# EnricoMiccoli/nodal

Hardware: AMD Instinct MI355X
Metric: circuits_per_sec (higher is better)
Workload: dtype f64; 1 GPU; cfg3: grid(1000) 1e6 nodes, sparse CSR path; n=999999, nnz=4995995, parallelism=one GPU

## Files before the change

include/nodal_hip.h:

```cpp
#ifndef NODAL_HIP_H
#define NODAL_HIP_H

#include <stddef.h>
#include <stdint.h>

#ifdef __cplusplus
extern "C" {
#endif

typedef struct nodal_ctx *nodal_handle;

typedef enum {
    NODAL_OK = 0,
    NODAL_E_INVALID = 1,
    NODAL_E_HIP = 2,
    NODAL_E_ZERO_RESISTANCE = 3,
    NODAL_E_STAMP_COLLISION = 4,
    NODAL_E_SINGULAR = 5,
    NODAL_E_NOMEM = 6,
    NODAL_E_UNSUPPORTED = 7
} nodal_status;

enum { NODAL_T_R = 0, NODAL_T_A = 1, NODAL_T_E = 2, NODAL_T_VCVS = 3,
       NODAL_T_CCVS = 4, NODAL_T_CCCS = 5,
// ... 11 lines not shown
const char *nodal_version(void);

int nodal_upload_components(nodal_handle h, int64_t ncomp,
                            const uint8_t *type, const double *value,
                            const int32_t *a, const int32_t *b,
                            const int32_t *c, const int32_t *d,
                            const int32_t *drv, const int32_t *k,
                            int32_t K, int32_t B);
int nodal_host_alloc(size_t bytes, void **out);
int nodal_host_free(void *p);

int nodal_upload_values(nodal_handle h, int32_t batch, const double *values);

int nodal_assemble_symbolic(nodal_handle h);
int nodal_assemble_numeric(nodal_handle h, int32_t member, int64_t *bad_component);

int nodal_get_sizes(nodal_handle h, int64_t *n, int64_t *nnz, int64_t *ncontrib);

int nodal_export_csr(nodal_handle h, int32_t *indptr, int32_t *indices,
                     double *data, double *rhs);
int nodal_export_dense(nodal_handle h, double *G, double *rhs);

int nodal_solve_dense(nodal_handle h, double *x, int32_t *info);
int nodal_solve_sparse(nodal_handle h, int32_t method, double *x, int32_t *info,
                       int32_t *iters, double *resid);
int nodal_download_x(nodal_handle h, double *x);

int nodal_solve_pairs(nodal_handle h, int32_t dense, int32_t npairs, const int32_t *ia,
                      const int32_t *ib, double *resistance, int32_t *info);

int nodal_solve_sources(nodal_handle h, int32_t dense, int32_t count, int32_t nsrc, const int64_t *rows,
                        const double *values, double *x_out, double *resid_out, int32_t *info_out);

int nodal_branches(nodal_handle h, double *voltage, double *current, double *power, double *totals2);

int nodal_solve_sources_branches(nodal_handle h, int32_t dense, int32_t count, int32_t nsrc, const int64_t *rows,
                                 const double *values, double *x_out, double *resid_out, int32_t *info_out,
                                 double *current_absmax, int32_t *current_member, double *potential_min,
                                 int32_t *potential_min_member, double *potential_max, int32_t *potential_max_member,
                                 double *power_out);

int nodal_sensitivities(nodal_handle h, int32_t dense, int32_t count, const int32_t *kind, const int32_t *p,
                        const int32_t *q2, double *sens_out, double *value_out, double *adjoint_out,
                        double *resid_out, int32_t *info_out);

int nodal_gradient(nodal_handle h, int32_t dense, int32_t count, const double *x, const double *cotangent, int32_t nsrc,
                   const int64_t *rows, double *grad_out, double *grad_sources_out, double *adjoint_out,
                   double *resid_out, int32_t *info_out);

int nodal_transient(nodal_handle h, int32_t dense, int32_t steps, int32_t method, int64_t ncap, const int64_t *cap_rows,
                    int32_t nsrc, const int64_t *src_rows, const double *src_values, const double *x0, int32_t nprobe,
                    const int32_t *probe_a, const int32_t *probe_b, double *wave_out, int32_t keep_every, double *x_out,
                    double *pot_min, int32_t *pot_min_step, double *pot_max, int32_t *pot_max_step, double *resid_out,
                    int32_t *info_out, int32_t *iters_out);

int nodal_transient_rlc(nodal_handle h, int32_t dense, int32_t steps, int32_t method, int64_t ncap, const int64_t *cap_rows,
                        int32_t nsrc, const int64_t *src_rows, const double *src_values, const double *x0, int32_t nprobe,
                        const int32_t *probe_a, const int32_t *probe_b, double *wave_out, int32_t keep_every, double *x_out,
                        double *pot_min, int32_t *pot_min_step, double *pot_max, int32_t *pot_max_step, double *resid_out,
                        int32_t *info_out, int32_t *iters_out, int64_t nind, const int64_t *ind_rows, const double *i0,
                        int32_t ncur, const int32_t *cur_index, double *cur_out, double *i_final_out);

int nodal_transient_gradient(nodal_handle h, int32_t dense, int32_t nprobe, const int32_t *probe_a, const int32_t *probe_b,
                             const double *wave_cot ,
                             double *grad_out ,
                             double *grad_sources_out ,
                             double *grad_x0_out ,
                             double *adjoint_out ,
                             double *resid_out , int32_t *info_out );

int nodal_ac_sweep(nodal_handle h, int32_t dense, int32_t nfreq, const double *omega ,
                   int64_t nreact, const uint8_t *kind , const double *value ,
                   const int32_t *lead_a, const int32_t *lead_b ,
                   int32_t nsrc, const int64_t *src_rows, const double *src_re, const double *src_im,
                   int32_t nprobe, const int32_t *probe_a, const int32_t *probe_b, double *wave_out ,
                   int32_t ncur, const int32_t *cur_index , double *cur_out ,
                   int32_t keep_every, double *x_out ,
                   double *peak_out , int32_t *peak_freq_out ,
                   double *resid_out , int32_t *info_out );

int nodal_ac_noise(nodal_handle h, int32_t dense, int32_t nfreq, const double *omega ,
                   int64_t nreact, const uint8_t *kind , const double *value ,
                   const int32_t *lead_a, const int32_t *lead_b ,
                   double temperature ,
                   int32_t nout, const int32_t *out_a, const int32_t *out_b ,
                   int64_t input_row , const double *weight ,
                   double *density_out , double *gain_out ,
                   double *contrib_out , double *resid_out ,
                   int32_t *info_out );

int nodal_ac_ports(nodal_handle h, int32_t dense, int32_t nfreq, const double *omega ,
                   int64_t nreact, const uint8_t *kind , const double *value ,
                   const int32_t *lead_a, const int32_t *lead_b ,
                   int32_t nports, const int32_t *ia, const int32_t *ib ,
                   double *z_out ,
                   double *node_peak_out , int32_t *node_peak_port_out ,
                   int32_t *node_peak_freq_out ,
                   double *resid_out , int32_t *info_out ,
                   int64_t *work_out );

int nodal_ac_gradient(nodal_handle h, int32_t dense, int32_t nfreq, const double *omega ,
                      int64_t nreact, const uint8_t *kind , const double *value ,
                      const int32_t *lead_a, const int32_t *lead_b ,
                      int32_t nsrc, const int64_t *src_rows, const double *src_re, const double *src_im,
                      int32_t nprobe, const int32_t *probe_a, const int32_t *probe_b ,
                      const double *wave_cot , double *wave_out ,
                      double *grad_out , double *grad_react_out ,
                      double *grad_sources_out , int32_t keep_every,
                      double *adjoint_out ,
                      double *resid_out , int32_t *info_out ,
                      int64_t *work_out );

int nodal_port_matrix(nodal_handle h, int32_t dense, int32_t nports, const int32_t *ia, const int32_t *ib,
                      double *z_out , double *voc_out ,
                      double *resid_out , int32_t *info_out );

int nodal_residual(nodal_handle h, double *scaled_residual);

int nodal_run(nodal_handle h, int32_t dense, int32_t member, int32_t reuse_symbolic,
              int32_t *info);

int nodal_run_batch(nodal_handle h, int32_t first, int32_t count, int32_t reuse_symbolic,
                    double *x_out, int32_t *info_out);
int nodal_batch_x_device(nodal_handle h, void *device_dst, int64_t capacity_bytes);
int nodal_x_device(nodal_handle h, void *device_dst, int64_t capacity_bytes);

int nodal_last_timings(nodal_handle h, double *ms3);
int nodal_last_kernel_stats(nodal_handle h, double *ms_total, int64_t *launches,
                            double *alg_bytes_or_flops);

int nodal_last_solve_info(nodal_handle h, int32_t *iterations, int32_t *amg_levels,
                          double *relative_residual);

int nodal_synchronize(nodal_handle h);

enum {
    NODAL_OPT_FORCE_PIVOTING = 1, NODAL_OPT_GEPP_PANEL = 2, NODAL_OPT_EXTRA_STREAMS = 3, NODAL_OPT_BORROW_TABLE = 4,
    NODAL_OPT_TRANSIENT_TAPE = 5
};
int nodal_set_option(nodal_handle h, int32_t option, int32_t value);

int nodal_debug_gemm(nodal_handle h, int32_t M, int32_t N, int32_t K, const double *A,
                     const double *B, double *C);
int nodal_debug_sources_rhs(nodal_handle h, int32_t count, int32_t nsrc, const int64_t *rows,
                            const double *values, double *rhs_out);
int nodal_debug_residual(nodal_handle h, int32_t transposed, int32_t cols, int32_t layout, const double *x,
                         const double *b, double *scaled_out, double *norms_out);
int nodal_debug_direct_apply(nodal_handle h, int32_t transposed, int32_t cols, const double *r, double *z,
                             int64_t *perturbed_out, int32_t *info_out);
enum {
    NODAL_HA_ACOL = 0, NODAL_HA_AVAL = 1, NODAL_HA_AVALF = 2, NODAL_HA_ALEN = 3, NODAL_HA_DINV = 4, NODAL_HA_ADCOL = 5,
    NODAL_HA_AGG = 6, NODAL_HA_PCOL = 7, NODAL_HA_PVAL = 8, NODAL_HA_PVALF = 9, NODAL_HA_RCOL = 10, NODAL_HA_RVAL = 11,
    NODAL_HA_RVALF = 12, NODAL_HA_RLEN = 13, NODAL_HA_WCOL = 14, NODAL_HA_WVAL = 15, NODAL_HA_WLEN = 16,
    NODAL_HA_P2COL = 17, NODAL_HA_P2VAL = 18, NODAL_HA_P2LEN = 19, NODAL_HA_D2 = 20
};
int nodal_debug_hierarchy_info(nodal_handle h, int32_t *nlev, int64_t *ints , double *reals );
int nodal_debug_hierarchy_array(nodal_handle h, int32_t level, int32_t which, void *dst, int64_t capacity_bytes,
                                int64_t *bytes_out);

#ifdef __cplusplus
}
#endif
#endif
```

nodal_amd/_ffi.py:

```python

import atexit
import ctypes as C
import os
import weakref

import numpy as np

_HERE = os.path.dirname(os.path.abspath(__file__))
LIB_PATH = os.path.join(_HERE, "libnodal_hip.so")

OK, E_INVALID, E_HIP, E_ZERO_RESISTANCE, E_STAMP_COLLISION, E_SINGULAR, E_NOMEM, \
    E_UNSUPPORTED = range(8)
SPARSE_AUTO, SPARSE_PCG, SPARSE_DENSIFY, SPARSE_LU, SPARSE_DIRECT = range(5)
OPT_FORCE_PIVOTING = 1
OPT_GEPP_PANEL = 2
OPT_EXTRA_STREAMS = 3
OPT_BORROW_TABLE = 4
OPT_TRANSIENT_TAPE = 5

_p = C.POINTER
_i32p, _i64p, _f64p, _u8p = _p(C.c_int32), _p(C.c_int64), _p(C.c_double), _p(C.c_uint8)

SIGNATURES = {
    "nodal_version": (C.c_char_p, []),
    "nodal_create": (C.c_int, [C.c_int, _p(C.c_void_p)]),
    "nodal_destroy": (C.c_int, [C.c_void_p]),
    "nodal_last_error": (C.c_char_p, [C.c_void_p]),
    "nodal_upload_components": (C.c_int, [C.c_void_p, C.c_int64, _u8p, _f64p, _i32p, _i32p,
                                          _i32p, _i32p, _i32p, _i32p, C.c_int32, C.c_int32]),
    "nodal_host_alloc": (C.c_int, [C.c_size_t, _p(C.c_void_p)]),
    "nodal_host_free": (C.c_int, [C.c_void_p]),
    "nodal_upload_values": (C.c_int, [C.c_void_p, C.c_int32, _f64p]),
    "nodal_assemble_symbolic": (C.c_int, [C.c_void_p]),
    "nodal_assemble_numeric": (C.c_int, [C.c_void_p, C.c_int32, _i64p]),
    "nodal_get_sizes": (C.c_int, [C.c_void_p, _i64p, _i64p, _i64p]),
    "nodal_export_csr": (C.c_int, [C.c_void_p, _i32p, _i32p, _f64p, _f64p]),
    "nodal_export_dense": (C.c_int, [C.c_void_p, _f64p, _f64p]),
    "nodal_solve_dense": (C.c_int, [C.c_void_p, _f64p, _i32p]),
    "nodal_solve_sparse": (C.c_int, [C.c_void_p, C.c_int32, _f64p, _i32p, _i32p, _f64p]),
    "nodal_download_x": (C.c_int, [C.c_void_p, _f64p]),
    "nodal_solve_pairs": (C.c_int, [C.c_void_p, C.c_int32, C.c_int32, _i32p, _i32p, _f64p, _i32p]),
    "nodal_solve_sources": (C.c_int, [C.c_void_p, C.c_int32, C.c_int32, C.c_int32, _i64p, _f64p, _f64p, _f64p,
                                      _i32p]),
    "nodal_branches": (C.c_int, [C.c_void_p, _f64p, _f64p, _f64p, _f64p]),
    "nodal_solve_sources_branches": (C.c_int, [C.c_void_p, C.c_int32, C.c_int32, C.c_int32, _i64p, _f64p, _f64p, _f64p,
                                               _i32p, _f64p, _i32p, _f64p, _i32p, _f64p, _i32p, _f64p]),
    "nodal_sensitivities": (C.c_int, [C.c_void_p, C.c_int32, C.c_int32, _i32p, _i32p, _i32p, _f64p, _f64p, _f64p, _f64p,
                                      _i32p]),
    "nodal_gradient": (C.c_int, [C.c_void_p, C.c_int32, C.c_int32, _f64p, _f64p, C.c_int32, _i64p, _f64p, _f64p, _f64p,
                                 _f64p, _i32p]),
    "nodal_transient": (C.c_int, [C.c_void_p, C.c_int32, C.c_int32, C.c_int32, C.c_int64, _i64p, C.c_int32, _i64p, _f64p,
                                  _f64p, C.c_int32, _i32p, _i32p, _f64p, C.c_int32, _f64p, _f64p, _i32p, _f64p, _i32p,
                                  _f64p, _i32p, _i32p]),
    "nodal_transient_rlc": (C.c_int, [C.c_void_p, C.c_int32, C.c_int32, C.c_int32, C.c_int64, _i64p, C.c_int32, _i64p, _f64p,
                                      _f64p, C.c_int32, _i32p, _i32p, _f64p, C.c_int32, _f64p, _f64p, _i32p, _f64p, _i32p,
                                      _f64p, _i32p, _i32p, C.c_int64, _i64p, _f64p, C.c_int32, _i32p, _f64p, _f64p]),
    "nodal_transient_gradient": (C.c_int, [C.c_void_p, C.c_int32, C.c_int32, _i32p, _i32p, _f64p, _f64p, _f64p, _f64p, _f64p,
                                           _f64p, _i32p]),
    "nodal_ac_sweep": (C.c_int, [C.c_void_p, C.c_int32, C.c_int32, _f64p, C.c_int64, _u8p, _f64p, _i32p, _i32p, C.c_int32,
                                 _i64p, _f64p, _f64p, C.c_int32, _i32p, _i32p, _f64p, C.c_int32, _i32p, _f64p, C.c_int32,
                                 _f64p, _f64p, _i32p, _f64p, _i32p]),
    "nodal_ac_noise": (C.c_int, [C.c_void_p, C.c_int32, C.c_int32, _f64p, C.c_int64, _u8p, _f64p, _i32p, _i32p, C.c_double,
                                 C.c_int32, _i32p, _i32p, C.c_int64, _f64p, _f64p, _f64p, _f64p, _f64p, _i32p]),
    "nodal_ac_ports": (C.c_int, [C.c_void_p, C.c_int32, C.c_int32, _f64p, C.c_int64, _u8p, _f64p, _i32p, _i32p, C.c_int32,
                                 _i32p, _i32p, _f64p, _f64p, _i32p, _i32p, _f64p, _i32p, _i64p]),
    "nodal_ac_gradient": (C.c_int, [C.c_void_p, C.c_int32, C.c_int32, _f64p, C.c_int64, _u8p, _f64p, _i32p, _i32p, C.c_int32,
                                    _i64p, _f64p, _f64p, C.c_int32, _i32p, _i32p, _f64p, _f64p, _f64p, _f64p, _f64p,
                                    C.c_int32, _f64p, _f64p, _i32p, _i64p]),
    "nodal_port_matrix": (C.c_int, [C.c_void_p, C.c_int32, C.c_int32, _i32p, _i32p, _f64p, _f64p, _f64p, _i32p]),
    "nodal_residual": (C.c_int, [C.c_void_p, _f64p]),
    "nodal_run": (C.c_int, [C.c_void_p, C.c_int32, C.c_int32, C.c_int32, _i32p]),
    "nodal_run_batch": (C.c_int, [C.c_void_p, C.c_int32, C.c_int32, C.c_int32, _f64p, _i32p]),
    "nodal_batch_x_device": (C.c_int, [C.c_void_p, C.c_void_p, C.c_int64]),
    "nodal_x_device": (C.c_int, [C.c_void_p, C.c_void_p, C.c_int64]),
    "nodal_last_timings": (C.c_int, [C.c_void_p, _f64p]),
    "nodal_last_kernel_stats": (C.c_int, [C.c_void_p, _f64p, _i64p, _f64p]),
    "nodal_last_solve_info": (C.c_int, [C.c_void_p, _i32p, _i32p, _f64p]),
    "nodal_synchronize": (C.c_int, [C.c_void_p]),
    "nodal_set_option": (C.c_int, [C.c_void_p, C.c_int32, C.c_int32]),
    "nodal_debug_gemm": (C.c_int, [C.c_void_p, C.c_int32, C.c_int32, C.c_int32, _f64p, _f64p, _f64p]),
    "nodal_debug_sources_rhs": (C.c_int, [C.c_void_p, C.c_int32, C.c_int32, _i64p, _f64p, _f64p]),
    "nodal_debug_residual": (C.c_int, [C.c_void_p, C.c_int32, C.c_int32, C.c_int32, _f64p, _f64p, _f64p, _f64p]),
    "nodal_debug_direct_apply": (C.c_int, [C.c_void_p, C.c_int32, C.c_int32, _f64p, _f64p, _i64p, _i32p]),
    "nodal_debug_hierarchy_info": (C.c_int, [C.c_void_p, _i32p, _i64p, _f64p]),
    "nodal_debug_hierarchy_array": (C.c_int, [C.c_void_p, C.c_int32, C.c_int32, C.c_void_p, C.c_int64, _i64p]),
}

HIERARCHY_ARRAYS = (("acol", np.int32), ("aval", np.float64), ("avalf", np.float32), ("alen", np.int32),
                    ("dinv", np.float64), ("adcol", np.int16), ("agg", np.int32), ("pcol", np.int32),
                    ("pval", np.float64), ("pvalf", np.float32), ("rcol", np.int32), ("rval", np.float64),
                    ("rvalf", np.float32), ("rlen", np.int32), ("wcol", np.int32), ("wval", np.float32),
                    ("wlen", np.int32), ("p2col", np.int32), ("p2val", np.float32), ("p2len", np.int32),
                    ("d2", np.float32))
HIERARCHY_INFO = ("n", "ld", "nc", "width", "maxlen", "wfix", "nnz", "rld", "rcap", "wslots", "fold_want", "fold", "d16",
                  "in_tail", "refreshed", "dense_coarsest")

_lib = None
_live = weakref.WeakSet()


@atexit.register
def _close_all():
    _closing[0] = True
    for h in list(_live):
        h.close()


class NodalHipError(RuntimeError):
    def __init__(self, status, message):
        super().__init__(f"libnodal_hip status {status}: {message}")
        self.status = status


def load():
    global _lib
    if _lib is None:
        if not os.path.exists(LIB_PATH):
            raise OSError(
                f"{LIB_PATH} not found: build it with `make` (or "
                "`python -c 'import __graft_entry__ as g; g.build()'`) -- "
                "nodal_amd has no CPU fallback")
        lib = C.CDLL(LIB_PATH)
        for name, (res, args) in SIGNATURES.items():
            fn = getattr(lib, name)
            fn.restype, fn.argtypes = res, args
        _lib = lib
    return _lib


def _ptr(arr, ctype):
    return arr.ctypes.data_as(_p(ctype))


PINNED_MIN_BYTES = 1 << 20
_PINNED_POOL = {}
_PINNED_POOL_BYTES = [0]
_PINNED_POOL_MAX = 1 << 30
_pinned_ok = [None]
_closing = [False]


def _pinned_release(addr, nbytes):
    if _lib is None or _closing[0]:
        return
    if _PINNED_POOL_BYTES[0] + nbytes <= _PINNED_POOL_MAX:
        _PINNED_POOL.setdefault(nbytes, []).append(addr)
        _PINNED_POOL_BYTES[0] += nbytes
    else:
        _lib.nodal_host_free(C.c_void_p(addr))


def host_empty(count, dtype):
    dtype = np.dtype(dtype)
    nbytes = int(count) * dtype.itemsize
    if nbytes < PINNED_MIN_BYTES or _pinned_ok[0] is False:
        return np.empty(count, dtype=dtype)
    try:
        lib = load()
    except OSError:
        _pinned_ok[0] = False
        return np.empty(count, dtype=dtype)
    size = (nbytes + 4095) & ~4095
    free = _PINNED_POOL.get(size)
    if free:
        addr = free.pop()
        _PINNED_POOL_BYTES[0] -= size
    else:
        out = C.c_void_p()
        if lib.nodal_host_alloc(size, C.byref(out)) != OK or not out.value:
            _pinned_ok[0] = False
            return np.empty(count, dtype=dtype)
        _pinned_ok[0] = True
        addr = out.value
    buf = (C.c_char * size).from_address(addr)
    weakref.finalize(buf, _pinned_release, addr, size)
    return np.frombuffer(buf, dtype=dtype, count=count)


class Handle:

    def __init__(self, device=0):
        self.lib = load()
        self._h = C.c_void_p()
        status = self.lib.nodal_create(device, C.byref(self._h))
        if status != OK:
            raise NodalHipError(
                status, f"nodal_create(device={device}) failed: no usable MI355X "
                "(HIP device) is visible; nodal_amd has no CPU fallback")
        self.n = self.nnz = self.ncontrib = 0
        self._ncomp = self._K = 0
        self.lib.nodal_set_option(self._h, OPT_BORROW_TABLE, 1)
        _live.add(self)

    def close(self):
        if getattr(self, "_h", None):
            self.lib.nodal_destroy(self._h)
            self._h = None

    __del__ = close

    @property
    def closed(self):
        return not getattr(self, "_h", None)

    def _check(self, status, allow=()):
        if status != OK and status not in allow:
            raise NodalHipError(status, self.lib.nodal_last_error(self._h).decode())
        return status

    def upload(self, table):
        names = ("type", "value", "a", "b") if table.B == 0 else ("type", "value", "a", "b", "c", "d", "drv", "k")
        cols = [np.ascontiguousarray(getattr(table, n)) for n in names]
        self._keep = cols
        t, v, a, b = cols[:4]
        rest = [_ptr(x, C.c_int32) for x in cols[4:]] or [None] * 4
        self.n_members = table.K + table.B
        self._ncomp, self._K = int(table.ncomp), int(table.K)
        self._check(self.lib.nodal_upload_components(
            self._h, table.ncomp, _ptr(t, C.c_uint8), _ptr(v, C.c_double),
            _ptr(a, C.c_int32), _ptr(b, C.c_int32), *rest, table.K, table.B))

    def upload_values(self, values):
        values = np.ascontiguousarray(values, dtype=np.float64)
        assert values.ndim == 2
        self._check(self.lib.nodal_upload_values(self._h, values.shape[0], _ptr(values, C.c_double)))

    def assemble_symbolic(self):
        self._check(self.lib.nodal_assemble_symbolic(self._h))
        self._refresh_sizes()

    def _refresh_sizes(self):
        n, nnz, nc = C.c_int64(), C.c_int64(), C.c_int64()
        self._check(self.lib.nodal_get_sizes(self._h, C.byref(n), C.byref(nnz), C.byref(nc)))
        self.n, self.nnz, self.ncontrib = n.value, nnz.value, nc.value

    def assemble_numeric(self, member=0):
        bad = C.c_int64(-1)
        status = self._check(self.lib.nodal_assemble_numeric(self._h, member, C.byref(bad)),
                             allow=(E_ZERO_RESISTANCE, E_STAMP_COLLISION))
        return status, bad.value

    def export_csr(self, values=True):
        indptr = np.empty(self.n + 1, dtype=np.int32)
        indices = np.empty(self.nnz, dtype=np.int32)
        data = np.empty(self.nnz, dtype=np.float64) if values else None
        rhs = np.empty(self.n, dtype=np.float64) if values else None
# ... 445 lines not shown
```

nodal_amd/csrc/knobs.h:

```cpp
#pragma once
#include <stdint.h>
#include <stdlib.h>

#include <optional>

namespace knob {

struct Present {
    const char *name;
    bool now() const { return getenv(name) != nullptr; }
};
struct OnUnless0 {
    const char *name;
    bool now() const { const char *e = getenv(name); return !(e && atoi(e) == 0); }
};
struct OffUnlessNon0 {
    const char *name;
    bool now() const { const char *e = getenv(name); return e && atoi(e) != 0; }
};
struct OnIfSet0 {
    const char *name;
    bool now() const { const char *e = getenv(name); return e != nullptr && atoi(e) == 0; }
};
struct Level {
    const char *name;
    int now() const {
        const char *e = getenv(name);
        if (!e) return 0;
        const int v = atoi(e);
        return v > 1 ? v : 1;
    }
};
struct Int {
    const char *name;
    int dflt;
    int now() const { const char *e = getenv(name); return e ? atoi(e) : dflt; }
};
struct Int64 {
    const char *name;
    int64_t dflt;
    int64_t now() const { const char *e = getenv(name); return e ? atoll(e) : dflt; }
};
struct Double {
    const char *name;
    double dflt;
    double now() const { const char *e = getenv(name); return e ? atof(e) : dflt; }
};
struct IntIfSet {
    const char *name;
    std::optional<int> now() const { const char *e = getenv(name); return e ? std::optional<int>(atoi(e)) : std::nullopt; }
};
struct Int64IfSet {
    const char *name;
    std::optional<int64_t> now() const { const char *e = getenv(name); return e ? std::optional<int64_t>(atoll(e)) : std::nullopt; }
};
struct DoubleIfSet {
    const char *name;
    std::optional<double> now() const { const char *e = getenv(name); return e ? std::optional<double>(atof(e)) : std::nullopt; }
};
struct Text {
    const char *name;
    const char *now() const { return getenv(name); }
};

inline constexpr Present TRACE{"NODAL_TRACE"};
inline constexpr Level POISON{"NODAL_POISON"};
inline constexpr Present NOFILL{"NODAL_NOFILL"};
inline constexpr Present NANCHECK{"NODAL_NANCHECK"};
inline constexpr Double WAIT_TIMEOUT_S{"NODAL_WAIT_TIMEOUT_S", 60.0};
inline constexpr Text STREAM_PRIORITY{"NODAL_STREAM_PRIORITY"};
inline constexpr IntIfSet EXTRA_STREAMS{"NODAL_EXTRA_STREAMS"};
inline constexpr IntIfSet HOST_THREADS{"NODAL_HOST_THREADS"};
inline constexpr IntIfSet CSV_CHUNKS{"NODAL_CSV_CHUNKS"};
inline constexpr OnUnless0 FOLD_STREAM{"NODAL_FOLD_STREAM"};
inline constexpr OffUnlessNon0 COUNT_LDS{"NODAL_COUNT_LDS"};
inline constexpr IntIfSet DENSE_BLOCKINV{"NODAL_DENSE_BLOCKINV"};
inline constexpr IntIfSet GJ_SCALAR{"NODAL_GJ_SCALAR"};
inline constexpr OnUnless0 GJ_DPP{"NODAL_GJ_DPP"};
inline constexpr OnUnless0 BI_SYM{"NODAL_BI_SYM"};
inline constexpr OnIfSet0 BI_MASKED{"NODAL_BI_MASKED"};
inline constexpr Int PANEL_CUS{"NODAL_PANEL_CUS", 32};
inline constexpr Int64 BI_UNMASK_ROWS{"NODAL_BI_UNMASK_ROWS", 0};
inline constexpr OnUnless0 BI_EARLY_COPY{"NODAL_BI_EARLY_COPY"};
inline constexpr Int BI_FIRST_BLOCKS{"NODAL_BI_FIRST_BLOCKS", 2};
inline constexpr Text BI_SWITCH{"NODAL_BI_SWITCH"};
inline constexpr Text BI_SWITCH2{"NODAL_BI_SWITCH2"};
inline constexpr Text BI_WIDTH{"NODAL_BI_WIDTH"};
inline constexpr IntIfSet GEPP_PANEL{"NODAL_GEPP_PANEL"};
inline constexpr Int GEPP_MAX{"NODAL_GEPP_MAX", 1280};
inline constexpr Present GEPP_PROBE{"NODAL_GEPP_PROBE"};
inline constexpr Int64IfSet FCG_MAXIT{"NODAL_FCG_MAXIT"};
inline constexpr OnUnless0 FCG_HOST_SUM{"NODAL_FCG_HOST_SUM"};
inline constexpr Double FCG_LOOK{"NODAL_FCG_LOOK", 0.75};
inline constexpr OnUnless0 LOWDEG{"NODAL_LOWDEG"};
inline constexpr IntIfSet LOWDEG_SHARE{"NODAL_LOWDEG_SHARE"};
inline constexpr Int64 LOWDEG_MIN{"NODAL_LOWDEG_MIN", 32};
inline constexpr Present SPARSE_FORCE_DIRECT{"NODAL_SPARSE_FORCE_DIRECT"};
inline constexpr Present SPARSE_CHILD_DIRECT{"NODAL_SPARSE_CHILD_DIRECT"};
inline constexpr OnUnless0 SAGG{"NODAL_SAGG"};
inline constexpr OnUnless0 SA_REUSE{"NODAL_SA_REUSE"};
inline constexpr OnUnless0 SA_FORK{"NODAL_SA_FORK"};
inline constexpr Double SA_SPREAD{"NODAL_SA_SPREAD", 16.0};
inline constexpr Double SA_SHARE{"NODAL_SA_SHARE", 0.9};
inline constexpr IntIfSet SA_MIS{"NODAL_SA_MIS"};
inline constexpr Text SA_OMEGA_P{"NODAL_SA_OMEGA_P"};
inline constexpr Double SA_PADSLACK{"NODAL_SA_PADSLACK", 1.3};
inline constexpr OnUnless0 SA_D16{"NODAL_SA_D16"};
inline constexpr Int SA_GG{"NODAL_SA_GG", 40};
inline constexpr Int64 SA_GCAP{"NODAL_SA_GCAP", 16384};
inline constexpr Int SA_GSEG{"NODAL_SA_GSEG", 4};
inline constexpr Text SA_NU{"NODAL_SA_NU"};
inline constexpr Int SA_KCYCLE{"NODAL_SA_KCYCLE", 1};
inline constexpr Int SA_KLEVELS{"NODAL_SA_KLEVELS", 1};
inline constexpr OnUnless0 SA_KFREEZE{"NODAL_SA_KFREEZE"};
inline constexpr OnUnless0 SA_FUSE_DIR{"NODAL_SA_FUSE_DIR"};
inline constexpr OffUnlessNon0 SA_GRAPH{"NODAL_SA_GRAPH"};
inline constexpr Text SA_FOLD_POST{"NODAL_SA_FOLD_POST"};
inline constexpr OffUnlessNon0 SA_FOLD_CHECK{"NODAL_SA_FOLD_CHECK"};
inline constexpr OnUnless0 SA_FOLD_VISIT{"NODAL_SA_FOLD_VISIT"};
inline constexpr Int64 SA_VISIT_CAP{"NODAL_SA_VISIT_CAP", 16777216};
inline constexpr OffUnlessNon0 SA_VISIT_CHECK{"NODAL_SA_VISIT_CHECK"};
inline constexpr OnUnless0 SA_TAIL_DENSE{"NODAL_SA_TAIL_DENSE"};
inline constexpr OffUnlessNon0 SA_TAIL_CHECK{"NODAL_SA_TAIL_CHECK"};
inline constexpr Int SA_TAIL_NU{"NODAL_SA_TAIL_NU", 3};
inline constexpr Present TAIL_PROBE{"NODAL_TAIL_PROBE"};
inline constexpr IntIfSet AMG_PASSES0{"NODAL_AMG_PASSES0"};
inline constexpr IntIfSet AMG_PASSES1{"NODAL_AMG_PASSES1"};
inline constexpr IntIfSet AMG_SWEEPS0{"NODAL_AMG_SWEEPS0"};
inline constexpr IntIfSet AMG_BLOCK{"NODAL_AMG_BLOCK"};
inline constexpr DoubleIfSet AMG_THETA{"NODAL_AMG_THETA"};
inline constexpr Present AMG_KEEP_DENSE{"NODAL_AMG_KEEP_DENSE"};
inline constexpr Present AMG_NOTAIL{"NODAL_AMG_NOTAIL"};
inline constexpr IntIfSet AMG_KMAX{"NODAL_AMG_KMAX"};
inline constexpr OnUnless0 PAIRS_BLOCK{"NODAL_PAIRS_BLOCK"};
inline constexpr OnUnless0 PAIRS_FUNCTIONAL{"NODAL_PAIRS_FUNCTIONAL"};
inline constexpr Int PAIRS_DIRECT{"NODAL_PAIRS_DIRECT", -1};
inline constexpr Int64 PAIRS_DIRECT_MIN{"NODAL_PAIRS_DIRECT_MIN", 256};
inline constexpr Double MULTI_BAR{"NODAL_MULTI_BAR", 1e-14};
inline constexpr IntIfSet PRESOLVE{"NODAL_PRESOLVE"};
inline constexpr OnUnless0 PRESOLVE_KEEP{"NODAL_PRESOLVE_KEEP"};
inline constexpr IntIfSet FGMRES_WINDOW{"NODAL_FGMRES_WINDOW"};
inline constexpr Text DIRECT_NB{"NODAL_DIRECT_NB"};
inline constexpr Int DIRECT_LANES{"NODAL_DIRECT_LANES", 4};
inline constexpr DoubleIfSet DIRECT_MAX_GB{"NODAL_DIRECT_MAX_GB"};
inline constexpr IntIfSet DIRECT_BIG_DIM{"NODAL_DIRECT_BIG_DIM"};
inline constexpr OnUnless0 DIRECT_FRONT_LDS{"NODAL_DIRECT_FRONT_LDS"};
inline constexpr Int DIRECT_LDS_BS{"NODAL_DIRECT_LDS_BS", 64};
inline constexpr OnUnless0 DIRECT_PANEL_REGS{"NODAL_DIRECT_PANEL_REGS"};
inline constexpr OnUnless0 DIRECT_BATCHED{"NODAL_DIRECT_BATCHED"};
inline constexpr OnUnless0 DIRECT_WAVE{"NODAL_DIRECT_WAVE"};
inline constexpr Present DIRECT_LEVELS{"NODAL_DIRECT_LEVELS"};
inline constexpr OnUnless0 DIRECT_SUPER{"NODAL_DIRECT_SUPER"};
inline constexpr OnUnless0 DIRECT_APPLY_STEPPED{"NODAL_DIRECT_APPLY_STEPPED"};
inline constexpr OnUnless0 DIRECT_PEEL{"NODAL_DIRECT_PEEL"};
inline constexpr Int ND_DEPTH{"NODAL_ND_DEPTH", 4};
inline constexpr Int64 ND_PAR{"NODAL_ND_PAR", 20000};
inline constexpr Present SLU_DEBUG{"SLU_DEBUG"};

}
```

nodal_amd/csrc/sagg.hip:

```cpp
#include <hip/hip_ext.h>

#include <atomic>
#include <type_traits>

#include "group.h"

int grounded_flags(nodal_ctx *h, uint8_t *flags_dev);

namespace {

using grp::TB;
constexpr int PW = 4;
constexpr int ACAP = 64;
constexpr int RCAP = 96;
constexpr int RCAP_SMALL = 512;
constexpr int RCAP_SMALL_ROWS = 16384;
inline int rcap_for(int64_t nc) { return nc <= RCAP_SMALL_ROWS ? RCAP_SMALL : RCAP; }
constexpr int W0_MAX = 32;
constexpr int COARSEST = 64;
constexpr int MAX_LEVELS = 12;
constexpr int MIS_ROUNDS = 6;
constexpr int TAIL_MAX_N = 1024;
constexpr int TAIL_LEVELS = 6;
constexpr int TAIL_LDS_BUDGET = 150 * 1024;
constexpr int APAD = 32;
constexpr int DOT_BLOCKS = 1024;
#ifndef NODAL_SA_OMEGA
#define NODAL_SA_OMEGA 0.85
#endif
constexpr double OMEGA = NODAL_SA_OMEGA;
constexpr double OMEGA_P = 0.70;
constexpr double OMEGA_P_COARSE = 0.85;
using cyc_t = nodal_cyc_t;

inline unsigned grid_for(int64_t n, unsigned cap = 8192) {
    int64_t g = (n + TB - 1) / TB;
    if (g < 1) g = 1;
    if (g >= 64) g = (g + 7) & ~(int64_t)7;
    return (unsigned)(g > cap ? cap : g);
}
inline int64_t pad64(int64_t n) { return (n + 63) & ~(int64_t)63; }
inline size_t align256(size_t x) { return (x + 255) & ~(size_t)255; }

__device__ __forceinline__ unsigned xcd_block() {
    const unsigned g = gridDim.x, b = blockIdx.x;
    return (g & 7u) ? b : (b & 7u) * (g >> 3) + (b >> 3);
}


struct Ell {
    int64_t n = 0, ld = 0;
    int32_t width = 0;
    const int32_t *col = nullptr;
    const int16_t *dcol = nullptr;
    const double *val = nullptr;
    const float *valf = nullptr;
    const int32_t *len = nullptr;
};

enum { ST_MAXLEN = 0, ST_GRADED = 1, ST_BADDIAG = 2, ST_OVERFLOW = 3, ST_NNZ = 4, ST_UNASSIGNED = 5,
       ST_MAXR = 6, ST_NC = 7 ,
       ST_FARCOL = 8 ,
       ST_FOLDMISS = 9 ,
       ST_VISITMISS = 10 ,
       ST_COUNT = 11 };

struct SLevel {
    int64_t n = 0, ld = 0, nc = 0;
    int32_t width = 0;
    int32_t maxlen = 0;
    int32_t wfix = 0;
    int64_t nnz = 0;
    DevBuf acol, aval, alen, dinv;
    DevBuf adcol;
    bool d16 = false;
    DevBuf agg, pcol, pval;
    DevBuf rcol, rval, rlen;
    int64_t rld = 0;
    DevBuf vec, part, gflag;
    DevBuf avalf, pvalf, rvalf;
    DevBuf wcol, wval, wlen;
    int32_t wslots = 0;
    bool fold_want = false, fold = false;
    DevBuf p2col, p2val, p2len, d2;
    bool visit_want = false, visit = false;
    Ell A() const {
        Ell e;
        e.n = n; e.ld = ld; e.width = width;
        e.col = acol.as<int32_t>(); e.val = aval.as<double>(); e.len = alen.as<int32_t>();
        e.valf = avalf.as<float>();
        e.dcol = d16 ? adcol.as<int16_t>() : nullptr;
        return e;
    }
    template <typename T = double> T *v(int which) const { return reinterpret_cast<T *>(vec.as<double>() + (int64_t)which * ld); }
};
enum { V_X = 0, V_R = 1, V_XP = 2, V_RC = 3, V_C1 = 4, V_C2 = 5, V_V1 = 6, V_V2 = 7, V_R2 = 8, V_X1 = 9, V_T = 10,
       V_COUNT = 11 };

struct TailLevelDesc {
    int n, nc, ld, rld, width, nq, lpr;
    const int32_t *acol, *pcol, *rcol, *rlen, *alen;
    const double *aval, *dinv, *pval, *rval;
    int o_aval, o_acol, o_dinv, o_pval, o_pcol, o_rval, o_rcol, o_B, o_X, o_Y, o_R;
};
struct TailDesc {
    int nlev;
    TailLevelDesc lv[TAIL_LEVELS];
    const double *inv;
    int nu;
    int image_bytes;
    int lds_bytes;
    int skip;
    int slots;
    long long *stamps;
};

struct SHierarchy {
    std::vector<SLevel *> pool;
    int nlev = 0;
    int tail = -1;
    bool ready = false;
    bool kcycle = true;
    bool kfrozen = false;
    int kslot = -1, kcount = 0, ksamples = 0;
    int klevels = 1;
    int nu[3] = {2, 1, 2};
    bool dense_coarsest = true;
    DevBuf tail_stamps, tail_image, apcol, apval, aplen, bstat;
    DevBuf tail_op;
    bool tail_dense = false;
    DevBuf mvec;
    hipEvent_t ev_copy = nullptr;
    hipStream_t aux = nullptr;
    hipEvent_t ev_fork = nullptr, ev_join = nullptr, ev_flags = nullptr;
    bool aux_pending = false;
    bool aux_tried = false;
    bool want_flags = false;
    int flags_levels = 0;
    DevBuf stats, coarse_inv, mis_t, mis_m, mis_flag, mis_id, agg1, keys, rstart, cursor, lists;
    TailDesc td;
    uint64_t *host_stats = nullptr;
    bool sym_valid = false;
    uint64_t sym_epoch = 0;
    int64_t sym_n = 0, sym_nnz = 0;
    bool sym_general = false, sym_check = false;
    int32_t sym_floating = 0;
    hipGraph_t it_graph = nullptr;
    hipGraphExec_t it_exec = nullptr;
    uint64_t it_key = 0;
    bool refreshed = false;
    int last_iters = 0;
    int hint_iters = 0;
    int64_t hint_n = 0, hint_nnz = 0;
    int mblock_iters = 0;
    int64_t mblock_n = 0;
    unsigned long long sym_stats[MAX_LEVELS * ST_COUNT] = {0};
    SLevel *level(int l) {
        while ((int)pool.size() <= l) pool.push_back(new SLevel());
        return pool[l];
    }
    void drop_graph() {
        if (it_exec) (void)hipGraphExecDestroy(it_exec);
        if (it_graph) (void)hipGraphDestroy(it_graph);
        it_exec = nullptr;
        it_graph = nullptr;
        it_key = 0;
    }
    ~SHierarchy() {
        drop_graph();
        if (ev_copy) (void)hipEventDestroy(ev_copy);
        if (ev_fork) (void)hipEventDestroy(ev_fork);
        if (ev_join) (void)hipEventDestroy(ev_join);
        if (ev_flags) (void)hipEventDestroy(ev_flags);
        if (aux) (void)hipStreamDestroy(aux);
        for (SLevel *l : pool) {
            DevBuf *b[] = {&l->acol, &l->aval, &l->alen, &l->dinv, &l->agg, &l->pcol, &l->pval, &l->rcol,
                           &l->rval, &l->rlen, &l->vec, &l->part, &l->gflag, &l->avalf, &l->pvalf, &l->rvalf, &l->adcol,
                           &l->wcol, &l->wval, &l->wlen, &l->p2col, &l->p2val, &l->p2len, &l->d2};
            for (DevBuf *x : b) x->release();
            delete l;
        }
        tail_image.release();
        tail_op.release();
        mvec.release();
        tail_stamps.release();
        bstat.release();
        apcol.release();
        apval.release();
        aplen.release();
        DevBuf *b[] = {&stats, &coarse_inv, &mis_t, &mis_m, &mis_flag, &mis_id, &agg1, &keys, &rstart, &cursor, &lists};
        for (DevBuf *x : b) x->release();
        if (host_stats) (void)hipHostFree(host_stats);
    }
};


constexpr int BSTAT_MAX = 65536;
__global__ __launch_bounds__(1024) void reduce_bstat(int nblocks, const uint32_t *__restrict__ bstat,
                                                     unsigned long long *__restrict__ stats, int slot_max,
                                                     int slot_sum) {
    __shared__ unsigned int s_max;
    __shared__ unsigned long long s_sum;
    if (threadIdx.x == 0) { s_max = 0; s_sum = 0; }
    __syncthreads();
    unsigned int m = 0;
    unsigned long long t = 0;
    for (int i = threadIdx.x; i < nblocks; i += 1024) {
        m = max(m, bstat[i]);
        t += bstat[BSTAT_MAX + i];
    }
    atomicMax(&s_max, m);
    atomicAdd(&s_sum, t);
    __syncthreads();
    if (threadIdx.x == 0) {
        if (slot_max >= 0) stats[slot_max] = s_max;
        if (slot_sum >= 0) stats[slot_sum] = s_sum;
    }
}

__global__ __launch_bounds__(TB) void row_stats(int64_t n, const int32_t *__restrict__ indptr,
                                                const int32_t *__restrict__ indices,
                                                const double *__restrict__ data, double share, double spread,
                                                bool general, unsigned long long *__restrict__ stats,
                                                uint32_t *__restrict__ bstat) {
    int32_t mlen = 0;
    uint32_t graded = 0, bad = 0, far = 0;
    for (int64_t i = (int64_t)xcd_block() * TB + threadIdx.x; i < n; i += (int64_t)gridDim.x * TB) {
        const int32_t e0 = indptr[i], e1 = indptr[i + 1];
        mlen = max(mlen, e1 - e0);
        double d = 0.0, mx = 0.0, mn = 1e300;
        for (int32_t e = e0; e < e1; ++e) {
            const double v = data[e];
            const int64_t dc = (int64_t)indices[e] - i;
            if (dc > 32767 || dc < -32767) far = 1;
            if (indices[e] == (int32_t)i) d = v;
            else if (v != 0.0) {
                mx = fmax(mx, fabs(v));
                mn = fmin(mn, fabs(v));
                if (v > 0.0 && !general) bad = 1;
            }
        }
        if (!(d > 0.0)) bad = 1;
        graded += (d > 0.0 && (mx > share * d || mx > spread * mn)) ? 1u : 0u;
    }
    __shared__ unsigned int s_len, s_graded, s_bad;
    if (threadIdx.x == 0) s_len = s_graded = s_bad = 0;
    __syncthreads();
    atomicMax(&s_len, (unsigned)mlen);
    if (graded) atomicAdd(&s_graded, graded);
    if (bad) atomicOr(&s_bad, 1u);
    if (far) atomicOr(&s_bad, 2u);
    __syncthreads();
    if (threadIdx.x == 0) {
        bstat[blockIdx.x] = s_len;
        bstat[BSTAT_MAX + blockIdx.x] = s_graded;
        if (s_bad & 1u) atomicOr(&stats[ST_BADDIAG], 1ull);
        if (s_bad & 2u) stats[ST_FARCOL] = 1ull;
    }
}

__global__ __launch_bounds__(TB) void csr_to_ell(int64_t n, int64_t ld, const int32_t *__restrict__ indptr,
                                                 const int32_t *__restrict__ indices,
                                                 const double *__restrict__ data, int32_t *__restrict__ col,
                                                 double *__restrict__ val, float *__restrict__ valf,
                                                 int32_t *__restrict__ len, double *__restrict__ dinv, int32_t wpad,
                                                 int16_t *__restrict__ dcol) {
    for (int64_t i = (int64_t)xcd_block() * TB + threadIdx.x; i < n; i += (int64_t)gridDim.x * TB) {
        const int32_t e0 = indptr[i], e1 = indptr[i + 1];
        double d = 1.0;
        for (int32_t e = e0; e < e1; ++e) {
            const int32_t c = indices[e];
            const double v = data[e];
            col[(int64_t)(e - e0) * ld + i] = c;
            if (dcol) dcol[(int64_t)(e - e0) * ld + i] = (int16_t)(c - (int32_t)i);
            val[(int64_t)(e - e0) * ld + i] = v;
            valf[(int64_t)(e - e0) * ld + i] = (float)v;
            if (c == (int32_t)i) d = v;
        }
        for (int32_t s = e1 - e0; s < wpad; ++s) {
            col[(int64_t)s * ld + i] = (int32_t)i;
            if (dcol) dcol[(int64_t)s * ld + i] = 0;
            val[(int64_t)s * ld + i] = 0.0;
            valf[(int64_t)s * ld + i] = 0.0f;
        }
        len[i] = e1 - e0;
        dinv[i] = 1.0 / d;
    }
}


__device__ __forceinline__ uint32_t hash30(uint32_t x) {
    x ^= x >> 16;
    x *= 0x7feb352du;
    x ^= x >> 15;
    x *= 0x846ca68bu;
    x ^= x >> 16;
    return x & 0x3fffffffu;
}

__global__ __launch_bounds__(TB) void mis_init(int64_t n, uint32_t *__restrict__ T) {
    for (int64_t i = (int64_t)xcd_block() * TB + threadIdx.x; i < n; i += (int64_t)gridDim.x * TB)
        T[i] = (1u << 30) | hash30((uint32_t)i);
}

template <int NB>
__device__ __forceinline__ uint32_t nbr_max_batch(const Ell &A, const uint32_t *__restrict__ v, int64_t i, int32_t l, int32_t s0,
                                                  uint32_t best) {
    int32_t c[NB];
#pragma unroll
    for (int u = 0; u < NB; ++u) c[u] = A.col[(int64_t)(s0 + u < l ? s0 + u : 0) * A.ld + i];
    uint32_t t[NB];
#pragma unroll
    for (int u = 0; u < NB; ++u) t[u] = v[c[u]];
#pragma unroll
    for (int u = 0; u < NB; ++u) best = t[u] > best ? t[u] : best;
    return best;
}
__device__ __forceinline__ uint32_t nbr_max(const Ell &A, const uint32_t *__restrict__ v, int64_t i, int32_t l, uint32_t best) {
    if (l <= 5) return nbr_max_batch<5>(A, v, i, l, 0, best);
    for (int32_t s0 = 0; s0 < l; s0 += 8) best = nbr_max_batch<8>(A, v, i, l, s0, best);
    return best;
}

__global__ __launch_bounds__(TB) void mis_max(Ell A, const uint32_t *__restrict__ v, uint32_t *__restrict__ m) {
    for (int64_t i = (int64_t)xcd_block() * TB + threadIdx.x; i < A.n; i += (int64_t)gridDim.x * TB)
        m[i] = nbr_max(A, v, i, A.len[i], v[i]);
}

__global__ __launch_bounds__(TB) void mis_update(Ell A, uint32_t *__restrict__ T, const uint32_t *__restrict__ m1) {
    for (int64_t i = (int64_t)xcd_block() * TB + threadIdx.x; i < A.n; i += (int64_t)gridDim.x * TB) {
        const uint32_t own = T[i];
        if ((own >> 30) != 1) continue;
        const uint32_t best = nbr_max(A, m1, i, A.len[i], m1[i]);
        if (best == own) T[i] = own | (2u << 30);
        else if ((best >> 30) == 3) T[i] = 0;
    }
}

__global__ __launch_bounds__(TB) void mis_count(int64_t n, const uint32_t *__restrict__ T,
                                                unsigned long long *__restrict__ out) {
    uint32_t left = 0;
    for (int64_t i = (int64_t)xcd_block() * TB + threadIdx.x; i < n; i += (int64_t)gridDim.x * TB)
        left += (T[i] >> 30) == 1 ? 1u : 0u;
// ... 22 lines not shown

constexpr int64_t MIS_SMALL_MAX = 1024;
__global__ __launch_bounds__(1024) void mis_small(Ell A, uint32_t *__restrict__ T, uint32_t *__restrict__ M,
                                                  uint32_t *__restrict__ flag, int rounds) {
    const int64_t n = A.n;
    for (int64_t i = threadIdx.x; i < n; i += 1024) T[i] = (1u << 30) | hash30((uint32_t)i);
    __syncthreads();
    for (int r = 0; r < rounds; ++r) {
        for (int64_t i = threadIdx.x; i < n; i += 1024) {
            uint32_t best = T[i];
            const int32_t l = A.len[i];
            for (int32_t s = 0; s < l; ++s) {
                const uint32_t t = T[A.col[(int64_t)s * A.ld + i]];
                best = t > best ? t : best;
            }
            M[i] = best;
        }
        __syncthreads();
        for (int64_t i = threadIdx.x; i < n; i += 1024) {
            const uint32_t own = T[i];
            if ((own >> 30) != 1) continue;
            uint32_t best = M[i];
            const int32_t l = A.len[i];
            for (int32_t s = 0; s < l; ++s) {
                const uint32_t t = M[A.col[(int64_t)s * A.ld + i]];
                best = t > best ? t : best;
            }
            if (best == own) T[i] = own | (2u << 30);
            else if ((best >> 30) == 3) T[i] = 0;
        }
        __syncthreads();
    }
    for (int64_t i = threadIdx.x; i <= n; i += 1024) {
        uint32_t f = 0;
        if (i < n) {
            const uint32_t own = T[i];
            if ((own >> 30) == 3) f = 1;
            else if ((own >> 30) == 1) {
                bool near = false;
                const int32_t l = A.len[i];
                for (int32_t s = 0; s < l; ++s) near = near || (T[A.col[(int64_t)s * A.ld + i]] >> 30) == 3;
                f = near ? 0u : 1u;
            }
        }
        flag[i] = f;
    }
}

__global__ __launch_bounds__(TB) void assign_near(Ell A, const uint32_t *__restrict__ T,
                                                  const uint32_t *__restrict__ flag,
                                                  const uint32_t *__restrict__ id, int32_t *__restrict__ agg1) {
    for (int64_t i = (int64_t)xcd_block() * TB + threadIdx.x; i < A.n; i += (int64_t)gridDim.x * TB) {
        int32_t a = -1;
        if (flag[i]) a = (int32_t)id[i];
        else {
            uint32_t best = 0;
            const int32_t l = A.len[i];
            auto batch = [&](auto NBc, int32_t s0) {
                constexpr int NB = decltype(NBc)::value;
                int32_t c[NB];
#pragma unroll
                for (int u = 0; u < NB; ++u) c[u] = A.col[(int64_t)(s0 + u < l ? s0 + u : 0) * A.ld + i];
                uint32_t fl[NB], tt[NB], idd[NB];
#pragma unroll
                for (int u = 0; u < NB; ++u) {
                    fl[u] = flag[c[u]];
                    tt[u] = T[c[u]];
                    idd[u] = id[c[u]];
                }
#pragma unroll
                for (int u = 0; u < NB; ++u) {
                    if (s0 + u >= l || c[u] == (int32_t)i || !fl[u]) continue;
                    const uint32_t t = tt[u] | (3u << 30);
                    if (t > best) { best = t; a = (int32_t)idd[u]; }
                }
            };
            if (l <= 5) batch(std::integral_constant<int, 5>{}, 0);
            else for (int32_t s0 = 0; s0 < l; s0 += 8) batch(std::integral_constant<int, 8>{}, s0);
        }
        agg1[i] = a;
    }
}

__global__ __launch_bounds__(TB) void assign_far(Ell A, const int32_t *__restrict__ agg1, int32_t *__restrict__ agg,
                                                 unsigned long long *__restrict__ stats) {
    for (int64_t i = (int64_t)xcd_block() * TB + threadIdx.x; i < A.n; i += (int64_t)gridDim.x * TB) {
        int32_t a = agg1[i];
        if (a < 0) {
            double bw = -1.0;
            const int32_t l = A.len[i];
            auto batch = [&](auto NBc, int32_t s0) {
                constexpr int NB = decltype(NBc)::value;
                int32_t c[NB];
                double w[NB];
#pragma unroll
                for (int u = 0; u < NB; ++u) {
                    const int64_t at = (int64_t)(s0 + u < l ? s0 + u : 0) * A.ld + i;
                    c[u] = A.col[at];
                    w[u] = fabs(A.val[at]);
                }
                int32_t aj[NB];
#pragma unroll
                for (int u = 0; u < NB; ++u) aj[u] = agg1[c[u]];
#pragma unroll
                for (int u = 0; u < NB; ++u) {
                    if (s0 + u >= l || c[u] == (int32_t)i || aj[u] < 0) continue;
                    if (w[u] > bw) { bw = w[u]; a = aj[u]; }
                }
            };
            if (l <= 5) batch(std::integral_constant<int, 5>{}, 0);
            else for (int32_t s0 = 0; s0 < l; s0 += 8) batch(std::integral_constant<int, 8>{}, s0);
            if (a < 0) stats[ST_UNASSIGNED] = 1;
        }
        agg[i] = a;
    }
}

__global__ __launch_bounds__(TB) void build_P(Ell A, const double *__restrict__ dinv,
                                              const int32_t *__restrict__ agg, int32_t *__restrict__ pcol,
                                              double *__restrict__ pval, float *__restrict__ pvalf, double omega_p) {
    for (int64_t i = (int64_t)xcd_block() * TB + threadIdx.x; i < A.n; i += (int64_t)gridDim.x * TB) {
        int32_t c[PW];
        double v[PW];
#pragma unroll
        for (int k = 0; k < PW; ++k) { c[k] = -1; v[k] = 0.0; }
        const int32_t own = agg[i];
        c[0] = own;
        v[0] = 1.0;
        const double wd = omega_p * dinv[i];
        const int32_t l = A.len[i];
        for (int32_t s = 0; s < l; ++s) {
            const int32_t J = agg[A.col[(int64_t)s * A.ld + i]];
            const double t = -wd * A.val[(int64_t)s * A.ld + i];
            bool placed = false;
#pragma unroll
            for (int k = 0; k < PW; ++k) {
                if (!placed && c[k] == J) { v[k] += t; placed = true; }
            }
#pragma unroll
            for (int k = 1; k < PW; ++k) {
                if (!placed && c[k] < 0) { c[k] = J; v[k] = t; placed = true; }
            }
            if (!placed) v[0] += t;
        }
#pragma unroll
        for (int k = 0; k < PW; ++k) {
            pcol[(int64_t)k * A.ld + i] = c[k];
            pval[(int64_t)k * A.ld + i] = v[k];
            pvalf[(int64_t)k * A.ld + i] = (float)v[k];
        }
    }
}

__global__ __launch_bounds__(TB) void r_count(int64_t n, int64_t ld, const int32_t *__restrict__ pcol,
                                              uint32_t *__restrict__ cnt, uint32_t *__restrict__ place) {
    for (int64_t i = (int64_t)xcd_block() * TB + threadIdx.x; i < n; i += (int64_t)gridDim.x * TB) {
#pragma unroll
        for (int k = 0; k < PW; ++k) {
            const int32_t J = pcol[(int64_t)k * ld + i];
            if (J >= 0) place[(int64_t)k * ld + i] = atomicAdd(&cnt[J], 1u);
        }
    }
}
__global__ __launch_bounds__(TB) void r_fill(int64_t n, int64_t ld, const int32_t *__restrict__ pcol,
                                             const uint32_t *__restrict__ rstart, const uint32_t *__restrict__ place,
                                             uint64_t *__restrict__ keys) {
    for (int64_t i = (int64_t)xcd_block() * TB + threadIdx.x; i < n; i += (int64_t)gridDim.x * TB) {
#pragma unroll
        for (int k = 0; k < PW; ++k) {
            const int32_t J = pcol[(int64_t)k * ld + i];
            if (J >= 0) keys[rstart[J] + place[(int64_t)k * ld + i]] = ((uint64_t)i << 2) | (uint64_t)k;
        }
    }
}
__global__ __launch_bounds__(TB) void r_to_ell(int64_t nc, int64_t rld, const uint32_t *__restrict__ rstart,
                                               const uint64_t *__restrict__ keys, int64_t ld,
                                               const double *__restrict__ pval, int32_t *__restrict__ rcol,
                                               double *__restrict__ rval, float *__restrict__ rvalf,
                                               int32_t *__restrict__ rlen,
                                               unsigned long long *__restrict__ stats, uint32_t *__restrict__ bstat,
                                               uint32_t rcap) {
    uint32_t mlen = 0;
    const int sub = threadIdx.x & 7;
    const int64_t rows_per_pass = (int64_t)gridDim.x * (TB / 8);
    for (int64_t I = (int64_t)xcd_block() * (TB / 8) + threadIdx.x / 8; I < nc; I += rows_per_pass) {
        const uint32_t s0 = rstart[I];
        uint32_t l = rstart[I + 1] - s0;
        mlen = l > mlen ? l : mlen;
        if (l > rcap) l = rcap;
        const uint32_t upto = nc <= 4096 ? rcap : ((l + 7u) & ~7u);
        for (uint32_t t = sub; t < upto; t += 8) {
            const int64_t at = ((int64_t)(t >> 3) * rld + I) * 8 + (t & 7);
            if (t < l) {
                const uint64_t key = keys[s0 + t];
                const int64_t i = (int64_t)(key >> 2);
                const double v = pval[(int64_t)(key & 3) * ld + i];
                rcol[at] = (int32_t)i;
                rval[at] = v;
                rvalf[at] = (float)v;
            } else {
                rcol[at] = 0;
                rval[at] = 0.0;
                rvalf[at] = 0.0f;
            }
        }
        if (sub == 0) rlen[I] = (int32_t)l;
    }
    if (mlen > rcap) atomicOr(&stats[ST_OVERFLOW], 2ull);
    __shared__ unsigned int s_max;
    if (threadIdx.x == 0) s_max = 0;
    __syncthreads();
#pragma unroll
    for (int off = 32; off > 0; off >>= 1) {
        const uint32_t o = __shfl_down(mlen, off, 64);
        mlen = o > mlen ? o : mlen;
    }
    if ((threadIdx.x & 63) == 0) atomicMax(&s_max, mlen);
    __syncthreads();
    if (threadIdx.x == 0) {
        bstat[blockIdx.x] = s_max;
        bstat[BSTAT_MAX + blockIdx.x] = 0;
    }
}

__global__ __launch_bounds__(TB) void r_refresh(int64_t nc, int64_t rld, const int32_t *__restrict__ rlen,
                                                const int32_t *__restrict__ rcol, int64_t ld,
                                                const int32_t *__restrict__ pcol, const double *__restrict__ pval,
                                                double *__restrict__ rval, float *__restrict__ rvalf) {
    const int sub = threadIdx.x & 7;
    const int64_t rows_per_pass = (int64_t)gridDim.x * (TB / 8);
    for (int64_t I = (int64_t)xcd_block() * (TB / 8) + threadIdx.x / 8; I < nc; I += rows_per_pass) {
        const int32_t l = rlen[I];
        for (int32_t t = sub; t < l; t += 8) {
            const int64_t at = ((int64_t)(t >> 3) * rld + I) * 8 + (t & 7);
            const int64_t i = rcol[at];
            double v = 0.0;
#pragma unroll
            for (int k = 0; k < PW; ++k) {
                const double pv = pval[(int64_t)k * ld + i];
                v = pcol[(int64_t)k * ld + i] == (int32_t)I ? pv : v;
            }
            rval[at] = v;
            rvalf[at] = (float)v;
        }
    }
}

__global__ __launch_bounds__(TB) void r_sort_short(const uint32_t *__restrict__ rstart, uint64_t *__restrict__ keys,
                                                   int64_t nc) {
    for (int64_t I = (int64_t)xcd_block() * TB + threadIdx.x; I < nc; I += (int64_t)gridDim.x * TB) {
        const uint32_t s0 = rstart[I];
        const int len = (int)(rstart[I + 1] - s0);
        if (len < 2) continue;
        if (len <= 4) grp::sort_short_row<4>(keys + s0, len);
        else if (len <= 8) grp::sort_short_row<8>(keys + s0, len);
        else if (len <= 16) grp::sort_short_row<16>(keys + s0, len);
        else if (len <= 32) grp::sort_short_row<32>(keys + s0, len);
    }
}
__global__ __launch_bounds__(64) void r_sort_medium(const uint32_t *__restrict__ rstart, uint64_t *__restrict__ keys,
                                                    int64_t nc) {
    __shared__ uint64_t buf[RCAP_SMALL];
    const int lane = threadIdx.x;
    for (int64_t I = blockIdx.x; I < nc; I += gridDim.x) {
        const uint32_t s0 = rstart[I];
        const int len = (int)(rstart[I + 1] - s0);
        if (len <= 32 || len > RCAP_SMALL) continue;
        const int P = len <= 64 ? 64 : (len <= 128 ? 128 : (len <= 256 ? 256 : 512));
        for (int e = lane; e < P; e += 64) buf[e] = e < len ? keys[s0 + e] : ~0ull;
        __syncthreads();
        for (int size = 2; size <= P; size <<= 1)
            for (int stride = size >> 1; stride > 0; stride >>= 1) {
                for (int p = lane; p < P / 2; p += 64) {
                    const int i = ((p & ~(stride - 1)) << 1) | (p & (stride - 1));
                    const int j = i | stride;
                    const bool up = (i & size) == 0;
                    const uint64_t a = buf[i], b = buf[j];
                    if ((a > b) == up) { buf[i] = b; buf[j] = a; }
                }
                __syncthreads();
            }
        for (int e = lane; e < len; e += 64) keys[s0 + e] = buf[e];
        __syncthreads();
    }
}

__device__ __forceinline__ int wave_excl_scan(int v, int *total) {
    const int lane = threadIdx.x & 63;
    int incl = v;
#pragma unroll
    for (int off = 1; off < 64; off <<= 1) {
        const int t = __shfl_up(incl, off, 64);
        if (lane >= off) incl += t;
    }
    *total = __shfl(incl, 63, 64);
    return incl - v;
}

template <int APW, bool EMIT>
__global__ __launch_bounds__(TB) void ap_rows(Ell A, const int32_t *__restrict__ pcol, const double *__restrict__ pval,
                                              int32_t *__restrict__ apcol, double *__restrict__ apval,
                                              int32_t *__restrict__ aplen, unsigned long long *__restrict__ stats,
                                              const double *__restrict__ dinv, int32_t *__restrict__ wcol,
                                              float *__restrict__ wval, int32_t *__restrict__ wlen) {
    bool overflow = false, miss = false;
    for (int64_t i = (int64_t)xcd_block() * TB + threadIdx.x; i < A.n; i += (int64_t)gridDim.x * TB) {
        int32_t c[APW];
        double v[APW];
        [[maybe_unused]] int32_t Jo[PW];
        [[maybe_unused]] double po[PW], wd = 0.0;
        if constexpr (EMIT) {
#pragma unroll
            for (int sp = 0; sp < PW; ++sp) {
                Jo[sp] = pcol[(int64_t)sp * A.ld + i];
                po[sp] = pval[(int64_t)sp * A.ld + i];
            }
            wd = OMEGA * dinv[i];
        }
#pragma unroll
        for (int q = 0; q < APW; ++q) { c[q] = -1; v[q] = 0.0; }
        int cnt = 0;
        const int32_t l = A.len[i];
        for (int32_t s = 0; s < l; ++s) {
            const int32_t k = A.col[(int64_t)s * A.ld + i];
            const double a = A.val[(int64_t)s * A.ld + i];
            int32_t J[PW];
            double pp[PW];
#pragma unroll
            for (int sp = 0; sp < PW; ++sp) {
                J[sp] = pcol[(int64_t)sp * A.ld + k];
                pp[sp] = pval[(int64_t)sp * A.ld + k];
            }
#pragma unroll
            for (int sp = 0; sp < PW; ++sp) {
                if (J[sp] < 0) continue;
                const double t = a * pp[sp];
                bool placed = false;
#pragma unroll
                for (int q = 0; q < APW; ++q)
                    if (!placed && c[q] == J[sp]) { v[q] += t; placed = true; }
#pragma unroll
                for (int q = 0; q < APW; ++q)
                    if (!placed && c[q] < 0) { c[q] = J[sp]; v[q] = t; placed = true; cnt = q + 1; }
                if (!placed) overflow = true;
            }
        }
#pragma unroll
        for (int q = 0; q < APW; ++q)
            if (q < cnt) {
                apcol[(int64_t)q * A.ld + i] = c[q];
                apval[(int64_t)q * A.ld + i] = v[q];
            }
        aplen[i] = cnt;
        if constexpr (EMIT) {
            int have = 0, found = 0;
#pragma unroll
            for (int sp = 0; sp < PW; ++sp) have += Jo[sp] >= 0 ? 1 : 0;
#pragma unroll
            for (int q = 0; q < APW; ++q)
                if (q < cnt) {
                    double pv = 0.0;
#pragma unroll
                    for (int sp = 0; sp < PW; ++sp)
                        if (Jo[sp] == c[q]) { pv += po[sp]; ++found; }
                    wcol[(int64_t)q * A.ld + i] = c[q];
                    wval[(int64_t)q * A.ld + i] = (float)(pv - wd * v[q]);
                }
            wlen[i] = cnt;
            if (found != have) miss = true;
        }
    }
    if (overflow) atomicOr(&stats[ST_OVERFLOW], 4ull);
    if (miss) stats[ST_FOLDMISS] = 1ull;
}

template <int APW, bool EMIT>
__global__ __launch_bounds__(64) void ap_rows_lds(Ell A, const int32_t *__restrict__ pcol,
                                                  const double *__restrict__ pval, int32_t *__restrict__ apcol,
                                                  double *__restrict__ apval, int32_t *__restrict__ aplen,
                                                  unsigned long long *__restrict__ stats,
                                                  const double *__restrict__ dinv, int32_t *__restrict__ wcol,
                                                  float *__restrict__ wval, int32_t *__restrict__ wlen) {
    __shared__ int32_t tc[APW * 64];
    __shared__ double tv[APW * 64];
    const int lane = threadIdx.x;
    bool overflow = false, miss = false;
    for (int64_t i0 = (int64_t)xcd_block() * 64; i0 < A.n; i0 += (int64_t)gridDim.x * 64) {
        const int64_t i = i0 + lane;
#pragma unroll 8
        for (int q = 0; q < APW; ++q) tc[q * 64 + lane] = -1;
        int cnt = 0;
        if (i < A.n) {
            const int32_t l = A.len[i];
            [[maybe_unused]] int32_t Jo[PW];
            [[maybe_unused]] double po[PW], wd = 0.0;
            if constexpr (EMIT) {
#pragma unroll
                for (int sp = 0; sp < PW; ++sp) {
                    Jo[sp] = pcol[(int64_t)sp * A.ld + i];
                    po[sp] = pval[(int64_t)sp * A.ld + i];
                }
                wd = OMEGA * dinv[i];
            }
            constexpr int AB = 4;
            for (int32_t s0 = 0; s0 < l; s0 += AB) {
                int32_t kk[AB];
                double aa[AB];
#pragma unroll
                for (int u = 0; u < AB; ++u) {
                    const int32_t su = s0 + u < l ? s0 + u : 0;
                    kk[u] = A.col[(int64_t)su * A.ld + i];
                    aa[u] = A.val[(int64_t)su * A.ld + i];
                }
                int32_t J[AB][PW];
                double pp[AB][PW];
#pragma unroll
                for (int u = 0; u < AB; ++u)
#pragma unroll
                    for (int sp = 0; sp < PW; ++sp) {
                        J[u][sp] = pcol[(int64_t)sp * A.ld + kk[u]];
                        pp[u][sp] = pval[(int64_t)sp * A.ld + kk[u]];
                    }
#pragma unroll
                for (int u = 0; u < AB; ++u) {
                    if (s0 + u >= l) continue;
#pragma unroll
                    for (int sp = 0; sp < PW; ++sp) {
                        if (J[u][sp] < 0) continue;
                        const double t = aa[u] * pp[u][sp];
                        uint32_t slot = ((uint32_t)J[u][sp] * 2654435761u) >> 16 & (APW - 1);
                        bool placed = false;
                        for (int probe = 0; probe < APW && !placed; ++probe) {
                            const int32_t c = tc[slot * 64 + lane];
                            if (c == J[u][sp]) {
                                tv[slot * 64 + lane] += t;
                                placed = true;
                            } else if (c < 0) {
// ... 282 lines not shown
}

__global__ __launch_bounds__(TB) void any_unflagged(int64_t n, const uint8_t *__restrict__ grounded,
                                                    uint32_t *__restrict__ floating) {
    for (int64_t i = (int64_t)xcd_block() * TB + threadIdx.x; i < n; i += (int64_t)gridDim.x * TB)
        if (!grounded[i]) *floating = 1;
}

}

#include "sagg_cycle.h"

namespace {

constexpr int SAGG_DECLINED = -3;

int width_class(int maxlen) {
    static const int classes[] = {4, 5, 6, 8, 12, 16, 20, 24, 32};
    for (int c : classes)
        if (maxlen <= c) return c;
    return 0;
}
int choose_wfix(int maxlen, int64_t n, int64_t nnz, int pad_limit) {
    const int c = width_class(maxlen);
    if (c == 0 || c > pad_limit) return 0;
    static const double slack = knob::SA_PADSLACK.now();
    if ((double)c * (double)n <= slack * (double)nnz || n <= 32768) return c;
    return 0;
}

SHierarchy *hierarchy_of(nodal_ctx *h) {
    if (!h->sagg) h->sagg = new SHierarchy();
    return static_cast<SHierarchy *>(h->sagg);
}

struct SolveBufs {
    double *r, *p, *p2, *Ap, *part_rz, *part_zap, *part_rr, *part_pap, *sc;
    cyc_t *z, *x0;
    int g0;
};

template <bool NUMERIC>
int galerkin_product(nodal_ctx *h, SHierarchy *H, int l, hipEvent_t r_ready = nullptr, int phase = 0) {
    hipStream_t st = h->stream;
    SLevel *L = H->level(l), *C = H->level(l + 1);
    const int64_t n = L->n, ld = L->ld, nc = C->n;
    Ell A = L->A();
    A.width = L->maxlen;
    unsigned long long *dstats = H->stats.as<unsigned long long>();
    const int apw = A.width <= 6 ? 16 : 64;
    NODAL_HIP_TRY(h, H->apcol.reserve((size_t)apw * ld * 4 + 64));
    NODAL_HIP_TRY(h, H->apval.reserve((size_t)apw * ld * 8 + 64));
    NODAL_HIP_TRY(h, H->aplen.reserve((size_t)ld * 4 + 64));
    int32_t *apcol = H->apcol.as<int32_t>(), *aplen = H->aplen.as<int32_t>();
    double *apval = H->apval.as<double>();
    unsigned long long *lst = dstats + (size_t)l * ST_COUNT;
    const unsigned g = grid_for(n);
    if (phase != 2) {
        const bool w = L->fold_want && L->wslots == apw;
        int32_t *wcol = w ? L->wcol.as<int32_t>() : nullptr, *wlen = w ? L->wlen.as<int32_t>() : nullptr;
        float *wval = w ? L->wval.as<float>() : nullptr;
        const double *dinv = L->dinv.as<double>();
        const int32_t *pc = L->pcol.as<int32_t>();
        const double *pv = L->pval.as<double>();
        const unsigned gl = (unsigned)((n + 63) / 64 < 4096 ? (n + 63) / 64 : 4096);
        if (apw == 16 && w) ap_rows<16, true><<<g, TB, 0, st>>>(A, pc, pv, apcol, apval, aplen, lst, dinv, wcol, wval, wlen);
        else if (apw == 16) ap_rows<16, false><<<g, TB, 0, st>>>(A, pc, pv, apcol, apval, aplen, lst, dinv, wcol, wval, wlen);
        else if (w) ap_rows_lds<64, true><<<gl, 64, 0, st>>>(A, pc, pv, apcol, apval, aplen, lst, dinv, wcol, wval, wlen);
        else ap_rows_lds<64, false><<<gl, 64, 0, st>>>(A, pc, pv, apcol, apval, aplen, lst, dinv, wcol, wval, wlen);
        NODAL_HIP_TRY(h, hipGetLastError());
    }
    if (phase == 1) return NODAL_OK;
    int G = 1024 / apw;
    G = (G < 8 ? 8 : (G > 64 ? 64 : G));
    static const int g_env = knob::SA_GG.now();
    if (g_env >= 8 && g_env <= 64 && apw == 16) G = g_env & ~7;
    const int pcap = G * apw + 72;
    const size_t lds = 1024 + (size_t)pcap * 12;
    static const int64_t gcap = knob::SA_GCAP.now();
    static const int maxseg = knob::SA_GSEG.now();
    const unsigned gg = (unsigned)(nc < gcap ? nc : (gcap < BSTAT_MAX ? gcap : BSTAT_MAX));
    if (r_ready) NODAL_HIP_TRY(h, hipStreamWaitEvent(st, r_ready, 0));
    galerkin<NUMERIC><<<gg, 64, lds, st>>>(
        ld, apcol, apval, aplen, nc, L->rld, L->rcol.as<int32_t>(), L->rval.as<double>(), L->rlen.as<int32_t>(),
        C->ld, C->acol.as<int32_t>(), C->aval.as<double>(), C->avalf.as<float>(), C->alen.as<int32_t>(),
        C->dinv.as<double>(), dstats + (size_t)(l + 1) * ST_COUNT, H->bstat.as<uint32_t>(), G, pcap, maxseg);
    if (!NUMERIC)
        reduce_bstat<<<1, 1024, 0, st>>>((int)gg, H->bstat.as<uint32_t>(), dstats + (size_t)(l + 1) * ST_COUNT,
                                         ST_MAXLEN, ST_NNZ);
    NODAL_HIP_TRY(h, hipGetLastError());
    return NODAL_OK;
}

double omega_p(int level) {
    static double w[2] = {-1.0, -1.0};
    if (w[0] < 0.0) {
        double a = OMEGA_P, b = OMEGA_P_COARSE;
        if (const char *e = knob::SA_OMEGA_P.now()) {
            a = atof(e);
            const char *c = strchr(e, ',');
            b = c ? atof(c + 1) : a;
        }
        w[1] = b > 0.0 && b < 1.2 ? b : OMEGA_P_COARSE;
        w[0] = a > 0.0 && a < 1.0 ? a : OMEGA_P;
    }
    return w[level > 0 ? 1 : 0];
}

constexpr int64_t FOLD_MAX_ROWS = 1 << 19;
struct FoldSetting { int mode = 0; unsigned mask = 0; };
const FoldSetting &fold_setting() {
    static const FoldSetting s = [] {
        FoldSetting f;
        const char *e = knob::SA_FOLD_POST.now();
        if (!e || !*e) return f;
        if (strchr(e, 'l')) {
            f.mode = 3;
            for (const char *q = e; (q = strchr(q, 'l')) != nullptr; ++q) {
                const int k = atoi(q + 1);
                if (q[1] >= '0' && q[1] <= '9' && k < MAX_LEVELS) f.mask |= 1u << k;
            }
        } else {
            f.mode = atoi(e) == 0 ? 1 : 2;
        }
        return f;
    }();
    return s;
}
bool fold_wanted(int level, int64_t n) {
    if (level > 0 && n <= TAIL_MAX_N) return false;
    const FoldSetting &f = fold_setting();
    switch (f.mode) {
    case 1: return false;
    case 2: return true;
    case 3: return (f.mask >> level & 1u) != 0;
    default: return n <= FOLD_MAX_ROWS;
    }
}
void decide_folds(SHierarchy *H, const unsigned long long *hs, bool trace) {
    for (int k = 0; k < H->nlev; ++k) {
        SLevel *L = H->pool[k];
        const bool runs_cycle = k + 1 < H->nlev && (H->tail < 0 || k < H->tail);
        const bool miss = hs[(size_t)k * ST_COUNT + ST_FOLDMISS] != 0;
        L->fold = L->fold_want && runs_cycle && !miss;
        if (trace && L->fold_want && runs_cycle)
            fprintf(stderr, "[sagg] level %d (%lld rows): first post-smoothing sweep %s\n", k, (long long)L->n,
                    miss ? "NOT folded: a row of A P lacks a column of its P row (no stored diagonal)"
                         : "folded into the prolongation");
        const bool wide = hs[(size_t)k * ST_COUNT + ST_VISITMISS] != 0;
        L->visit = L->visit_want && L->fold && !wide;
        if (trace && L->visit_want)
            fprintf(stderr, "[sagg] level %d (%lld rows): visit %s\n", k, (long long)L->n,
                    L->visit ? "in three launches" : "NOT in three launches: W missing, or a row of P2 beyond its slots");
    }
}

int build_level(nodal_ctx *h, SHierarchy *H, int l, unsigned long long *hs, bool *declined, bool *stop) {
    hipStream_t st = h->stream;
    SLevel *L = H->level(l);
    const int64_t n = L->n, ld = L->ld;
    Ell A = L->A();
    A.width = L->maxlen;
    unsigned long long *dstats = H->stats.as<unsigned long long>();

    NODAL_HIP_TRY(h, H->mis_t.reserve((size_t)n * 8 + 64));
    NODAL_HIP_TRY(h, H->mis_m.reserve((size_t)n * 8 + 64));
    NODAL_HIP_TRY(h, H->mis_flag.reserve((size_t)(n + 1) * 4 + 64));
    NODAL_HIP_TRY(h, H->mis_id.reserve((size_t)(n + 1) * 4 + 64 + scan_tmp_bytes(n + 1)));
    NODAL_HIP_TRY(h, H->agg1.reserve((size_t)n * 4 + 64));
    NODAL_HIP_TRY(h, L->agg.reserve((size_t)n * 4 + 64));
    NODAL_HIP_TRY(h, H->cursor.reserve((MIS_ROUNDS + 2) * 8 + 64));
    uint32_t *T = H->mis_t.as<uint32_t>(), *M = H->mis_m.as<uint32_t>();
    uint32_t *flag = H->mis_flag.as<uint32_t>(), *id = H->mis_id.as<uint32_t>();
    unsigned long long *cnt = H->cursor.as<unsigned long long>();
    void *scan_tmp = H->mis_id.as<char>() + (((size_t)(n + 1) * 4 + 63) & ~(size_t)63);

    const unsigned g = grid_for(n);
    static const bool trace_mis = knob::TRACE.now();
    if (trace_mis) NODAL_HIP_TRY(h, hipMemsetAsync(cnt, 0, (MIS_ROUNDS + 2) * 8, st));
    static const int mis_rounds = std::min(MIS_ROUNDS, std::max(1, knob::SA_MIS.now().value_or(MIS_ROUNDS)));
    if (n <= MIS_SMALL_MAX && !trace_mis) {
        mis_small<<<1, 1024, 0, st>>>(A, T, M, flag, mis_rounds);
    } else {
        mis_init<<<g, TB, 0, st>>>(n, T);
        for (int r = 0; r < mis_rounds; ++r) {
            mis_max<<<g, TB, 0, st>>>(A, T, M);
            mis_update<<<g, TB, 0, st>>>(A, T, M);
            if (trace_mis) mis_count<<<g, TB, 0, st>>>(n, T, cnt + r + 1);
        }
        mis_flag_roots<<<grid_for(n + 1), TB, 0, st>>>(A, T, flag);
    }
    NODAL_HIP_TRY(h, hipGetLastError());
    NODAL_TRY(scan_exclusive_u32(h, flag, id, n + 1, reinterpret_cast<uint32_t *>(dstats + (size_t)l * ST_COUNT + ST_NC),
                                 scan_tmp));
    NODAL_HIP_TRY(h, hipMemcpyAsync(hs, dstats, (size_t)MAX_LEVELS * ST_COUNT * 8, hipMemcpyDeviceToHost, st));
    unsigned long long hcnt[MIS_ROUNDS + 1] = {0};
    if (trace_mis) NODAL_HIP_TRY(h, hipMemcpyAsync(hcnt, cnt, sizeof hcnt, hipMemcpyDeviceToHost, st));
    if (!H->ev_copy) NODAL_HIP_TRY(h, hipEventCreateWithFlags(&H->ev_copy, hipEventDisableTiming));
    NODAL_HIP_TRY(h, hipEventRecord(H->ev_copy, st));
    NODAL_HIP_TRY(h, L->pcol.reserve((size_t)PW * ld * 4 + 64));
    NODAL_HIP_TRY(h, L->pval.reserve((size_t)PW * ld * 8 + 64));
    NODAL_HIP_TRY(h, L->pvalf.reserve((size_t)PW * ld * 4 + 64));
    assign_near<<<g, TB, 0, st>>>(A, T, flag, id, H->agg1.as<int32_t>());
    assign_far<<<g, TB, 0, st>>>(A, H->agg1.as<int32_t>(), L->agg.as<int32_t>(), dstats + (size_t)l * ST_COUNT);
    build_P<<<g, TB, 0, st>>>(A, L->dinv.as<double>(), L->agg.as<int32_t>(), L->pcol.as<int32_t>(),
                             L->pval.as<double>(), L->pvalf.as<float>(), omega_p(l));
    NODAL_HIP_TRY(h, hipGetLastError());
    NODAL_WAIT_EVENT(h, H->ev_copy, st);
    if (trace_mis) {
        fprintf(stderr, "[sagg] level %d: undecided after each MIS round:", l);
        for (int r = 1; r <= MIS_ROUNDS; ++r) fprintf(stderr, " %llu", hcnt[r]);
        fprintf(stderr, "\n");
    }
    const int64_t nc = (int64_t)(hs[(size_t)l * ST_COUNT + ST_NC] & 0xffffffffull);
    if (l > 0) {
        const unsigned long long *s = hs + (size_t)l * ST_COUNT;
        L->maxlen = (int32_t)s[ST_MAXLEN];
        L->nnz = (int64_t)s[ST_NNZ];
        A.width = L->maxlen;
        if (s[ST_OVERFLOW] || s[ST_BADDIAG] || hs[(size_t)(l - 1) * ST_COUNT + ST_OVERFLOW] ||
            hs[(size_t)(l - 1) * ST_COUNT + ST_UNASSIGNED]) {
            *declined = true;
            return NODAL_OK;
        }
    }
    if (nc >= n || L->maxlen <= 1) {
        *stop = true;
        return NODAL_OK;
    }
    if ((nc * 2 > n && n > 4096) || nc < 1) {
        *declined = true;
        return NODAL_OK;
    }
    L->nc = nc;

    static const bool fork_allowed = knob::SA_FORK.now();
    if (H->aux && !nodal_extra_streams_ok(h) && nodal_calls_in_flight() <= 1) {
        NODAL_WAIT_STREAM(h, H->aux);
        (void)hipStreamDestroy(H->aux);
        H->aux = nullptr;
        H->aux_tried = false;
    }
    if (fork_allowed && !H->aux_tried && nodal_extra_streams_ok(h)) {
        H->aux_tried = true;
        if (hipStreamCreateWithFlags(&H->aux, hipStreamNonBlocking) != hipSuccess) H->aux = nullptr;
        if (H->aux && ((!H->ev_fork && hipEventCreateWithFlags(&H->ev_fork, hipEventDisableTiming) != hipSuccess) ||
                       (!H->ev_join && hipEventCreateWithFlags(&H->ev_join, hipEventDisableTiming) != hipSuccess) ||
                       (!H->ev_flags && hipEventCreateWithFlags(&H->ev_flags, hipEventDisableTiming) != hipSuccess))) {
            (void)hipStreamDestroy(H->aux);
            H->aux = nullptr;
        }
        (void)hipGetLastError();
    }
    const bool forked = fork_allowed && H->aux != nullptr && nodal_extra_streams_ok(h);
    const size_t a4 = (((size_t)(nc + 1) * 4) + 255) & ~(size_t)255;
    const size_t scan2 = (scan_tmp_bytes(nc + 1) + 255) & ~(size_t)255;
    NODAL_HIP_TRY(h, H->rstart.reserve(a4 + 256 + scan2 + (size_t)PW * ld * 4 + 64));
    NODAL_HIP_TRY(h, H->keys.reserve((size_t)PW * n * 8 + 64));
    SLevel *C = H->level(l + 1);
    C->n = nc;
    C->ld = pad64(nc);
    C->width = ACAP;
    C->nc = 0;
    L->rld = C->ld;
    const int rcap = rcap_for(nc);
    NODAL_HIP_TRY(h, L->rcol.reserve((size_t)rcap * C->ld * 4 + 64));
    NODAL_HIP_TRY(h, L->rval.reserve((size_t)rcap * C->ld * 8 + 64));
    NODAL_HIP_TRY(h, L->rvalf.reserve((size_t)rcap * C->ld * 4 + 64));
    NODAL_HIP_TRY(h, L->rlen.reserve((size_t)C->ld * 4 + 64));
    NODAL_HIP_TRY(h, C->acol.reserve((size_t)ACAP * C->ld * 4 + 64));
    NODAL_HIP_TRY(h, C->aval.reserve((size_t)ACAP * C->ld * 8 + 64));
    NODAL_HIP_TRY(h, C->avalf.reserve((size_t)ACAP * C->ld * 4 + 64));
    NODAL_HIP_TRY(h, C->alen.reserve((size_t)C->ld * 4 + 64));
    NODAL_HIP_TRY(h, C->dinv.reserve((size_t)C->ld * 8 + 64));
    if (forked && H->want_flags) {
        if (l == 0) NODAL_HIP_TRY(h, L->gflag.reserve((size_t)n + 64));
        NODAL_HIP_TRY(h, C->gflag.reserve((size_t)C->n + 64));
    }
    {
        const int apw = L->maxlen <= 6 ? 16 : 64;
        NODAL_HIP_TRY(h, H->apcol.reserve((size_t)apw * ld * 4 + 64));
        NODAL_HIP_TRY(h, H->apval.reserve((size_t)apw * ld * 8 + 64));
        NODAL_HIP_TRY(h, H->aplen.reserve((size_t)ld * 4 + 64));
        L->fold = false;
        L->fold_want = fold_wanted(l, n);
        L->wslots = apw;
        if (L->fold_want) {
            NODAL_HIP_TRY(h, L->wcol.reserve((size_t)apw * ld * 4 + 64));
            NODAL_HIP_TRY(h, L->wval.reserve((size_t)apw * ld * 4 + 64));
            NODAL_HIP_TRY(h, L->wlen.reserve((size_t)ld * 4 + 64));
        }
    }
    hipStream_t main_st = h->stream;
    struct StreamGuard {
        nodal_ctx *h;
        hipStream_t keep;
        ~StreamGuard() { h->stream = keep; }
    } guard{h, main_st};
    if (forked) {
        NODAL_HIP_TRY(h, hipEventRecord(H->ev_fork, main_st));
        NODAL_HIP_TRY(h, hipStreamWaitEvent(H->aux, H->ev_fork, 0));
        H->aux_pending = true;
        NODAL_TRY(galerkin_product<false>(h, H, l, nullptr, 1));
        h->stream = H->aux;
        st = H->aux;
    }
    char *rs = H->rstart.as<char>();
    uint32_t *rstart = reinterpret_cast<uint32_t *>(rs);
    void *scan_tmp2 = rs + a4 + 256;
    uint32_t *place = reinterpret_cast<uint32_t *>(rs + a4 + 256 + scan2);
    NODAL_HIP_TRY(h, hipMemsetAsync(rs, 0, a4 + 256, st));
    r_count<<<g, TB, 0, st>>>(n, ld, L->pcol.as<int32_t>(), rstart, place);
    NODAL_HIP_TRY(h, hipGetLastError());
    NODAL_TRY(scan_exclusive_u32(h, rstart, rstart, nc + 1, nullptr, scan_tmp2));
    uint64_t *keys = H->keys.as<uint64_t>();
    r_fill<<<g, TB, 0, st>>>(n, ld, L->pcol.as<int32_t>(), rstart, place, keys);
    r_sort_short<<<grid_for(nc), TB, 0, st>>>(rstart, keys, nc);
    r_sort_medium<<<(unsigned)(nc < 8192 ? nc : 8192), 64, 0, st>>>(rstart, keys, nc);
    NODAL_HIP_TRY(h, hipGetLastError());

    {
        const unsigned gr = grid_for(nc * 8);
        r_to_ell<<<gr, TB, 0, st>>>(nc, L->rld, rstart, keys, ld, L->pval.as<double>(), L->rcol.as<int32_t>(),
                                   L->rval.as<double>(), L->rvalf.as<float>(), L->rlen.as<int32_t>(),
                                   dstats + (size_t)l * ST_COUNT, H->bstat.as<uint32_t>(), (uint32_t)rcap);
        reduce_bstat<<<1, 1024, 0, st>>>((int)gr, H->bstat.as<uint32_t>(), dstats + (size_t)l * ST_COUNT, ST_MAXR, -1);
    }
    if (forked) {
        NODAL_HIP_TRY(h, hipGetLastError());
        NODAL_HIP_TRY(h, hipEventRecord(H->ev_join, H->aux));
        if (H->want_flags && H->flags_levels == l) {
            if (l == 0) NODAL_TRY(grounded_flags(h, L->gflag.as<uint8_t>()));
            NODAL_HIP_TRY(h, hipMemsetAsync(C->gflag.p, 0, ((size_t)C->n + 63) & ~(size_t)63, st));
            flags_up<<<grid_for(n), TB, 0, st>>>(n, L->agg.as<int32_t>(), L->gflag.as<uint8_t>(), C->gflag.as<uint8_t>());
            NODAL_HIP_TRY(h, hipGetLastError());
            NODAL_HIP_TRY(h, hipEventRecord(H->ev_flags, H->aux));
            H->flags_levels = l + 1;
        }
        h->stream = main_st;
        st = main_st;
    }
    NODAL_TRY(galerkin_product<false>(h, H, l, forked ? H->ev_join : nullptr, forked ? 2 : 0));
    if (forked && H->flags_levels != l + 1) H->aux_pending = false;
    return NODAL_OK;
}

const void *tail_kernel(int slots) {
    return slots <= 8 ? reinterpret_cast<const void *>(k_tail<8>)
                      : slots <= 16 ? reinterpret_cast<const void *>(k_tail<16>)
                                    : reinterpret_cast<const void *>(k_tail<32>);
}

const void *tail_op_kernel(int slots) {
    return slots <= 8 ? reinterpret_cast<const void *>(k_tail_pack_op<8>)
                      : slots <= 16 ? reinterpret_cast<const void *>(k_tail_pack_op<16>)
                                    : reinterpret_cast<const void *>(k_tail_pack_op<32>);
}

int tail_walk(nodal_ctx *h, SHierarchy *H, const double *b, double *out, int nv) {
    const TailDesc &d = H->td;
    const char *img = H->tail_image.as<char>();
    if (d.slots <= 8) k_tail<8><<<nv, 1024, (size_t)d.lds_bytes, h->stream>>>(d, img, b, out, nv);
    else if (d.slots <= 16) k_tail<16><<<nv, 1024, (size_t)d.lds_bytes, h->stream>>>(d, img, b, out, nv);
    else k_tail<32><<<nv, 1024, (size_t)d.lds_bytes, h->stream>>>(d, img, b, out, nv);
    NODAL_HIP_TRY(h, hipGetLastError());
    return NODAL_OK;
}

template <int NV>
int tail_apply(nodal_ctx *h, SHierarchy *H, const double *b, double *out) {
    const int n = H->td.lv[0].n;
    const double *T = H->tail_op.as<double>();
    const unsigned gr = (unsigned)((n + 3) / 4);
    if (n <= 256) k_tail_apply<4, NV><<<gr, 256, 0, h->stream>>>(n, T, b, out);
    else if (n <= 512) k_tail_apply<8, NV><<<gr, 256, 0, h->stream>>>(n, T, b, out);
    else k_tail_apply<16, NV><<<gr, 256, 0, h->stream>>>(n, T, b, out);
    NODAL_HIP_TRY(h, hipGetLastError());
    return NODAL_OK;
}

int tail_self_check(nodal_ctx *h, SHierarchy *H) {
    const int n = H->td.lv[0].n;
    std::vector<double> b((size_t)n), yc((size_t)n), yd((size_t)n), T((size_t)n * n);
    uint64_t seed = 0x9e3779b97f4a7c15ull;
    for (int i = 0; i < n; ++i) {
        uint64_t z = (seed += 0x9e3779b97f4a7c15ull);
        z = (z ^ (z >> 30)) * 0xbf58476d1ce4e5b9ull;
        z = (z ^ (z >> 27)) * 0x94d049bb133111ebull;
        z ^= z >> 31;
        b[i] = (double)(z >> 11) * (1.0 / 4503599627370496.0) - 1.0;
    }
    DevBuf v;
    hipError_t e = v.reserve((size_t)3 * n * 8);
    double *db = v.as<double>(), *dc = db + n, *dd = dc + n;
    int rc = NODAL_OK;
    if (e == hipSuccess) e = hipMemcpyAsync(db, b.data(), (size_t)n * 8, hipMemcpyHostToDevice, h->stream);
    if (e == hipSuccess) rc = tail_walk(h, H, db, dc, 1);
    if (e == hipSuccess && rc == NODAL_OK) rc = tail_apply<1>(h, H, db, dd);
    if (e == hipSuccess && rc == NODAL_OK) e = hipStreamSynchronize(h->stream);
    if (e == hipSuccess) e = hipMemcpy(yc.data(), dc, (size_t)n * 8, hipMemcpyDeviceToHost);
    if (e == hipSuccess) e = hipMemcpy(yd.data(), dd, (size_t)n * 8, hipMemcpyDeviceToHost);
    if (e == hipSuccess) e = hipMemcpy(T.data(), H->tail_op.p, (size_t)n * n * 8, hipMemcpyDeviceToHost);
    v.release();
    if (rc != NODAL_OK) return rc;
    NODAL_HIP_TRY(h, e);
    double d = 0.0, dp = 0.0;
    for (int i = 0; i < n; ++i) {
        long double y = 0.0L, a = 0.0L;
        for (int j = 0; j < n; ++j) {
            y += (long double)T[(size_t)i * n + j] * b[j];
            a += fabsl((long double)T[(size_t)i * n + j] * b[j]);
        }
        const double den = (double)a;
        const double q = fabs(yd[i] - yc[i]) / den, qp = (double)(fabsl((long double)yd[i] - y) / a);
        d = !(q <= d) ? q : d;
        dp = !(qp <= dp) ? qp : dp;
    }
    fprintf(stderr, "[sagg] tail check: n_t %d, dense operator against the cycle d = %.3e (product alone %.3e)\n", n, d, dp);
    return NODAL_OK;
}

int form_tail_op(nodal_ctx *h, SHierarchy *H) {
    static const bool on = knob::SA_TAIL_DENSE.now();
    H->tail_dense = false;
    if (!on || H->tail < 0) return NODAL_OK;
    const TailDesc &d = H->td;
    const int n = d.lv[0].n;
    static std::atomic<int> cus[64];
    const int dev = h->device >= 0 && h->device < 64 ? h->device : 0;
    int ncu = cus[dev].load(std::memory_order_acquire);
    if (ncu == 0) {
        NODAL_HIP_TRY(h, hipDeviceGetAttribute(&ncu, hipDeviceAttributeMultiprocessorCount, h->device >= 0 ? h->device : 0));
        if (ncu < 1) ncu = 1;
        cus[dev].store(ncu, std::memory_order_release);
    }
    NODAL_HIP_TRY(h, H->tail_op.reserve((size_t)n * n * 8 + 64));
    const unsigned gr = (unsigned)(n < ncu ? n : ncu);
    double *T = H->tail_op.as<double>();
    const char *img = H->tail_image.as<char>();
    if (d.slots <= 8) k_tail_pack_op<8><<<gr, 1024, (size_t)d.lds_bytes, h->stream>>>(d, img, T);
    else if (d.slots <= 16) k_tail_pack_op<16><<<gr, 1024, (size_t)d.lds_bytes, h->stream>>>(d, img, T);
    else k_tail_pack_op<32><<<gr, 1024, (size_t)d.lds_bytes, h->stream>>>(d, img, T);
    NODAL_HIP_TRY(h, hipGetLastError());
    H->tail_dense = true;
    static const bool check = knob::TRACE.now() && knob::SA_TAIL_CHECK.now();
    if (check) NODAL_TRY(tail_self_check(h, H));
    return NODAL_OK;
}

constexpr int P2LIST = 1024;
__global__ __launch_bounds__(64) void p2_rows_wave(Ell A, const double *__restrict__ dinv, const int32_t *__restrict__ wcol,
                                                   const float *__restrict__ wval, const int32_t *__restrict__ wlen,
                                                   int32_t *__restrict__ p2col, float *__restrict__ p2val,
                                                   int32_t *__restrict__ p2len, unsigned long long *__restrict__ stats) {
    __shared__ int32_t lJ[P2LIST];
    __shared__ double lV[P2LIST];
    __shared__ uint32_t mask[TAIL_MAX_N / 32];
    __shared__ int32_t cols[P2CAP];
    static_assert(TAIL_MAX_N / 32 <= 64, "one lane per word of the column mask");
    const int lane = threadIdx.x;
    bool overflow = false;
    for (int64_t i = blockIdx.x; i < A.n; i += gridDim.x) {
        if (lane < TAIL_MAX_N / 32) mask[lane] = 0u;
        const int32_t total = A.len[i] + 1;
        const double wd = -OMEGA * dinv[i];
        int np = 0;
        bool fits = true;
        for (int32_t g0 = 0; g0 < total; g0 += 64) {
            const int32_t src = g0 + lane;
            const bool has = src < total;
            const int32_t su = has && src >= 1 ? src - 1 : 0;
            const int32_t ka = A.col[(int64_t)su * A.ld + i];
            const double a = A.val[(int64_t)su * A.ld + i];
            const int32_t k = src == 0 ? (int32_t)i : ka;
            const double cf = src == 0 ? 1.0 : wd * a;
            const int32_t lk = wlen[k];
            const int32_t len = has ? lk : 0;
            int tot = 0;
            int o = np + wave_excl_scan(len, &tot);
            if (np + tot > P2LIST) {
                fits = false;
                break;
            }
            constexpr int SQ = 8;
            for (int32_t s0 = 0; s0 < len; s0 += SQ) {
                int32_t cj[SQ];
                float cv[SQ];
#pragma unroll
                for (int q = 0; q < SQ; ++q) {
                    const int32_t s = s0 + q < len ? s0 + q : s0;
                    cj[q] = wcol[(int64_t)s * A.ld + k];
                    cv[q] = wval[(int64_t)s * A.ld + k];
                }
#pragma unroll
                for (int q = 0; q < SQ; ++q)
                    if (s0 + q < len) {
// ... 3 lines not shown
                    }
            }
            np += tot;
        }
        __syncthreads();
        if (fits)
            for (int p = lane; p < np; p += 64) atomicOr(&mask[lJ[p] >> 5], 1u << (lJ[p] & 31));
        __syncthreads();
        uint32_t m = lane < TAIL_MAX_N / 32 ? mask[lane] : 0u;
        int distinct = 0;
        int at = wave_excl_scan(__popc(m), &distinct);
        if (!fits || distinct > P2CAP) {
            overflow = true;
            if (lane == 0) p2len[i] = 0;
            __syncthreads();
            continue;
        }
        while (m) {
            cols[at++] = lane * 32 + (__ffs(m) - 1);
            m &= m - 1u;
        }
        __syncthreads();
        if (lane < distinct) {
            const int32_t c = cols[lane];
            double acc = 0.0;
#pragma unroll 8
            for (int p = 0; p < np; ++p) {
                const int32_t j = lJ[p];
                const double v = lV[p];
                if (j == c) acc += v;
            }
            p2col[(int64_t)lane * A.ld + i] = c;
            p2val[(int64_t)lane * A.ld + i] = (float)acc;
        }
        if (lane == 0) p2len[i] = distinct;
        __syncthreads();
    }
    if (overflow) stats[ST_VISITMISS] = 1ull;
}

__global__ __launch_bounds__(TB) void d2_zero(float4 *__restrict__ d, int64_t pieces) {
    for (int64_t e = (int64_t)blockIdx.x * TB + threadIdx.x; e < pieces; e += (int64_t)gridDim.x * TB)
        d[e] = make_float4(0.0f, 0.0f, 0.0f, 0.0f);
}

__global__ __launch_bounds__(TB) void d2_scatter(int64_t n, int64_t ld, const int32_t *__restrict__ p2col,
                                                 const float *__restrict__ p2val, const int32_t *__restrict__ p2len,
                                                 float *__restrict__ d2) {
    for (int64_t e = (int64_t)blockIdx.x * TB + threadIdx.x; e < (int64_t)P2CAP * ld; e += (int64_t)gridDim.x * TB) {
        const int64_t s = e / ld, i = e - s * ld;
        if (i >= n || s >= p2len[i]) continue;
        d2[(int64_t)p2col[e] * ld + i] = p2val[e];
    }
}

void apply_nu_knob(SHierarchy *H) {
    if (const char *e = knob::SA_NU.now()) {
        for (int k = 0; k < 3 && e[k] >= '1' && e[k] <= '3'; ++k) H->nu[k] = e[k] - '0';
    }
}

int build_visit(nodal_ctx *h, SHierarchy *H, bool general) {
    static const bool on = knob::SA_FOLD_VISIT.now();
    static const int64_t cap = knob::SA_VISIT_CAP.now();
    for (int k = 0; k < H->nlev; ++k) H->pool[k]->visit_want = H->pool[k]->visit = false;
    if (!on || general || H->tail < 2 || !H->tail_dense) return NODAL_OK;
    const int l = H->tail - 1;
    SLevel *L = H->pool[l];
    apply_nu_knob(H);
    const int64_t nt = H->pool[H->tail]->n;
    if (H->nu[l < 2 ? l : 2] != 2 || !L->fold_want || nt > TAIL_MAX_N || nt * L->ld * 4 > cap) return NODAL_OK;
    hipStream_t st = h->stream;
    NODAL_HIP_TRY(h, L->p2col.reserve((size_t)P2CAP * L->ld * 4 + 64));
    NODAL_HIP_TRY(h, L->p2val.reserve((size_t)P2CAP * L->ld * 4 + 64));
    NODAL_HIP_TRY(h, L->p2len.reserve((size_t)L->ld * 4 + 64));
    NODAL_HIP_TRY(h, L->d2.reserve((size_t)nt * L->ld * 4 + 64));
    Ell A = L->A();
    const unsigned gl = (unsigned)(L->n < 8192 ? L->n : 8192);
    p2_rows_wave<<<gl, 64, 0, st>>>(A, L->dinv.as<double>(), L->wcol.as<int32_t>(), L->wval.as<float>(), L->wlen.as<int32_t>(),
                                  L->p2col.as<int32_t>(), L->p2val.as<float>(), L->p2len.as<int32_t>(),
                                  H->stats.as<unsigned long long>() + (size_t)l * ST_COUNT);
    NODAL_HIP_TRY(h, hipGetLastError());
    d2_zero<<<grid_for(nt * L->ld / 4), TB, 0, st>>>(L->d2.as<float4>(), nt * L->ld / 4);
    d2_scatter<<<grid_for((int64_t)P2CAP * L->ld), TB, 0, st>>>(L->n, L->ld, L->p2col.as<int32_t>(), L->p2val.as<float>(),
                                                                 L->p2len.as<int32_t>(), L->d2.as<float>());
    NODAL_HIP_TRY(h, hipGetLastError());
    L->visit_want = true;
    return NODAL_OK;
}

template <typename TC>
int fold_check_level(nodal_ctx *h, SHierarchy *H, int l, bool two) {
    hipStream_t st = h->stream;
    const SLevel *L = H->pool[l];
    const int64_t n = L->n, nc = H->pool[l + 1]->n;
    const Ell A = L->A();
    uint64_t seed = 0x9e3779b97f4a7c15ull + (uint64_t)l;
    auto unit = [&]() {
        uint64_t z = (seed += 0x9e3779b97f4a7c15ull);
        z = (z ^ (z >> 30)) * 0xbf58476d1ce4e5b9ull;
        z = (z ^ (z >> 27)) * 0x94d049bb133111ebull;
        z ^= z >> 31;
        return (double)(z >> 11) * (1.0 / 4503599627370496.0) - 1.0;
    };
    std::vector<cyc_t> hx((size_t)n), hb((size_t)n);
    std::vector<TC> he((size_t)2 * nc);
    for (auto &v : hx) v = (cyc_t)unit();
    for (auto &v : hb) v = (cyc_t)unit();
    for (auto &v : he) v = (TC)unit();
    const double hcoef[2] = {0.9, 0.4};
    const size_t vb = align256((size_t)n * sizeof(cyc_t)), eb = align256((size_t)nc * sizeof(TC)), db = align256((size_t)n * 8);
    DevBuf buf;
    hipError_t e = buf.reserve(6 * vb + 2 * eb + 2 * db + 256);
    char *p = buf.as<char>();
    cyc_t *x = reinterpret_cast<cyc_t *>(p), *b = reinterpret_cast<cyc_t *>(p + vb), *r = reinterpret_cast<cyc_t *>(p + 2 * vb),
          *xp = reinterpret_cast<cyc_t *>(p + 3 * vb), *mt = reinterpret_cast<cyc_t *>(p + 4 * vb),
          *mf = reinterpret_cast<cyc_t *>(p + 5 * vb);
    TC *c1 = reinterpret_cast<TC *>(p + 6 * vb), *c2 = reinterpret_cast<TC *>(p + 6 * vb + eb);
    double *d = reinterpret_cast<double *>(p + 6 * vb + 2 * eb), *q = reinterpret_cast<double *>(p + 6 * vb + 2 * eb + db);
    double *coef = reinterpret_cast<double *>(p + 6 * vb + 2 * eb + 2 * db);
    std::vector<double> hd((size_t)n), hq((size_t)n);
    if (e == hipSuccess) e = hipMemcpyAsync(x, hx.data(), (size_t)n * sizeof(cyc_t), hipMemcpyHostToDevice, st);
    if (e == hipSuccess) e = hipMemcpyAsync(b, hb.data(), (size_t)n * sizeof(cyc_t), hipMemcpyHostToDevice, st);
    if (e == hipSuccess) e = hipMemcpyAsync(c1, he.data(), (size_t)nc * sizeof(TC), hipMemcpyHostToDevice, st);
    if (e == hipSuccess) e = hipMemcpyAsync(c2, he.data() + nc, (size_t)nc * sizeof(TC), hipMemcpyHostToDevice, st);
    if (e == hipSuccess) e = hipMemcpyAsync(coef, hcoef, sizeof hcoef, hipMemcpyHostToDevice, st);
    if (e == hipSuccess) {
        const unsigned g = grid_for(n), tb = L->wfix ? TB : TB * LPR_RAGGED;
        const double *dinv = L->dinv.as<double>(), *cf = two ? coef : nullptr;
        const int32_t *wcol = L->wcol.as<int32_t>(), *wlen = L->wlen.as<int32_t>();
        const float *wval = L->wval.as<float>();
        SAGG_DISPATCH_W(L->wfix, (k_smooth_residual<W, cyc_t><<<g, tb, 0, st>>>(A, b, x, r)));
        k_prolong<TC><<<g, TB, 0, st>>>(n, L->ld, L->pcol.as<int32_t>(), L->pvalf.as<float>(), x, c1, two ? c2 : nullptr, cf, xp);
        SAGG_DISPATCH_W(L->wfix, (k_post<W, false, cyc_t, cyc_t><<<g, tb, 0, st>>>(A, dinv, b, xp, mt, nullptr, nullptr, nullptr)));
        k_prolong_post<TC, cyc_t><<<g, TB, 0, st>>>(n, L->ld, wcol, wval, wlen, x, r, dinv, c1, two ? c2 : nullptr, cf, mf);
        k_fold_check<TC><<<g, TB, 0, st>>>(A, dinv, b, x, xp, wcol, wval, wlen, c1, two ? c2 : nullptr, cf, mt, mf, d, q);
        e = hipGetLastError();
    }
    if (e == hipSuccess) e = hipStreamSynchronize(st);
    if (e == hipSuccess) e = hipMemcpy(hd.data(), d, (size_t)n * 8, hipMemcpyDeviceToHost);
    if (e == hipSuccess) e = hipMemcpy(hq.data(), q, (size_t)n * 8, hipMemcpyDeviceToHost);
    buf.release();
    NODAL_HIP_TRY(h, e);
    double dm = 0.0, qm = 0.0;
    for (int64_t i = 0; i < n; ++i) {
        dm = !(hd[i] <= dm) ? hd[i] : dm;
        qm = !(hq[i] <= qm) ? hq[i] : qm;
    }
    fprintf(stderr, "[sagg] fold check: level %d, rows %lld, slots %d, width %d, fused launch against the two d = %.3e "
                    "(worst row against its own bound: %.3e)\n", l, (long long)n, (int)L->wslots, (int)L->maxlen, dm, qm);
    return NODAL_OK;
}
int visit_self_check(nodal_ctx *h, SHierarchy *H);
int fold_self_check(nodal_ctx *h, SHierarchy *H) {
    static const bool check = knob::TRACE.now() && knob::SA_FOLD_CHECK.now();
    if (!check) return NODAL_OK;
    for (int l = 0; l + 1 < H->nlev; ++l) {
        if (!H->pool[l]->fold) continue;
        const bool last = l + 1 == H->tail || l + 1 == H->nlev - 1;
        if (last) NODAL_TRY(fold_check_level<double>(h, H, l, false));
        else NODAL_TRY(fold_check_level<cyc_t>(h, H, l, true));
    }
    return NODAL_OK;
}

int build_tail(nodal_ctx *h, SHierarchy *H, const unsigned long long *hs) {
    H->tail = -1;
    H->tail_dense = false;
    const int last = H->nlev - 1;
    auto up16 = [](int x) { return (x + 15) & ~15; };
    for (int t = 1; t <= last; ++t) {
        if (H->pool[t]->n > TAIL_MAX_N || last - t + 1 > TAIL_LEVELS) continue;
        TailDesc d;
        memset(&d, 0, sizeof d);
        d.nlev = last - t + 1;
        d.nu = knob::SA_TAIL_NU.now();
        if (d.nu < 1) d.nu = 1;
        int off = 0;
        for (int k = 0; k < d.nlev; ++k) {
            const SLevel *L = H->pool[t + k];
            TailLevelDesc &q = d.lv[k];
            q.n = (int)L->n; q.nc = (int)L->nc; q.ld = (int)L->ld; q.rld = (int)L->rld; q.width = L->maxlen;
            q.acol = L->acol.as<int32_t>(); q.aval = L->aval.as<double>();
            q.dinv = L->dinv.as<double>(); q.alen = L->alen.as<int32_t>();
            q.pcol = L->pcol.as<int32_t>(); q.pval = L->pval.as<double>();
            q.rcol = L->rcol.as<int32_t>(); q.rval = L->rval.as<double>(); q.rlen = L->rlen.as<int32_t>();
            if (k == d.nlev - 1) {
                q.o_aval = off; off = up16(off + (H->dense_coarsest ? q.n * q.n : q.n) * 8);
                continue;
            }
            const int maxr = (int)hs[(size_t)(t + k) * ST_COUNT + ST_MAXR];
            q.nq = (maxr + 7) / 8;
            q.lpr = 1;
            while (q.lpr < 8 && q.n * q.lpr * 2 <= 1024) q.lpr *= 2;
            q.o_aval = off; off = up16(off + q.n * q.width * 8);
            q.o_acol = off; off = up16(off + q.n * q.width * 2);
            q.o_dinv = off; off = up16(off + q.n * 8);
            q.o_pval = off; off = up16(off + q.n * PW * 8);
            q.o_pcol = off; off = up16(off + q.n * PW * 2);
            q.o_rval = off; off = up16(off + q.nq * q.nc * 8 * 8);
            q.o_rcol = off; off = up16(off + q.nq * q.nc * 8 * 2);
        }
        d.image_bytes = off;
        for (int k = 0; k < d.nlev; ++k) {
            TailLevelDesc &q = d.lv[k];
            q.o_B = off; off = up16(off + q.n * 8);
            q.o_X = off; off = up16(off + q.n * 8);
            if (k == d.nlev - 1) continue;
            q.o_Y = off; off = up16(off + q.n * 8);
            q.o_R = off; off = up16(off + q.n * 8);
        }
        d.inv = H->dense_coarsest ? H->coarse_inv.as<double>() : nullptr;
        d.skip = d.nlev > 1 ? d.lv[0].o_dinv : 0;
        d.lds_bytes = off - d.skip;
        if (knob::TAIL_PROBE.now()) {
            NODAL_HIP_TRY(h, H->tail_stamps.reserve(64 * sizeof(long long)));
            d.stamps = H->tail_stamps.as<long long>();
        }
        if (d.lds_bytes > TAIL_LDS_BUDGET) continue;
        d.slots = d.nlev > 1 ? (d.lv[0].width + d.lv[0].lpr - 1) / d.lv[0].lpr : 1;
        if (d.slots > 32) continue;
        {
            static std::atomic<bool> lds_allowed[64][3];
            const int dev = h->device >= 0 && h->device < 64 ? h->device : 0;
            const int which = d.slots <= 8 ? 0 : (d.slots <= 16 ? 1 : 2);
            if (!lds_allowed[dev][which].load(std::memory_order_acquire)) {
                NODAL_HIP_TRY(h, hipFuncSetAttribute(tail_kernel(d.slots), hipFuncAttributeMaxDynamicSharedMemorySize,
                                                     TAIL_LDS_BUDGET));
                NODAL_HIP_TRY(h, hipFuncSetAttribute(tail_op_kernel(d.slots), hipFuncAttributeMaxDynamicSharedMemorySize,
                                                     TAIL_LDS_BUDGET));
                lds_allowed[dev][which].store(true, std::memory_order_release);
            }
        }
        NODAL_HIP_TRY(h, H->tail_image.reserve((size_t)d.image_bytes + 256));
        k_tail_pack<<<1, 1024, 0, h->stream>>>(d, H->tail_image.as<char>());
        NODAL_HIP_TRY(h, hipGetLastError());
        H->td = d;
        H->tail = t;
        NODAL_TRY(form_tail_op(h, H));
        break;
    }
    return NODAL_OK;
}

int sagg_refresh(nodal_ctx *h, SHierarchy *H, const int32_t *indptr0, const int32_t *indices0, const double *data0,
                 bool general, bool *ok) {
    *ok = false;
    hipStream_t st = h->stream;
    unsigned long long *dstats = H->stats.as<unsigned long long>();
    unsigned long long *hs = reinterpret_cast<unsigned long long *>(H->host_stats);
    NODAL_HIP_TRY(h, hipMemsetAsync(dstats, 0, (size_t)MAX_LEVELS * ST_COUNT * 8, st));
    SLevel *L0 = H->pool[0];
    const int64_t n0 = L0->n;
    {
        const unsigned gr = grid_for(n0);
        static const double spread = knob::SA_SPREAD.now();
        static const double share = knob::SA_SHARE.now();
        row_stats<<<gr, TB, 0, st>>>(n0, indptr0, indices0, data0, share, spread, general, dstats, H->bstat.as<uint32_t>());
        reduce_bstat<<<1, 1024, 0, st>>>((int)gr, H->bstat.as<uint32_t>(), dstats, ST_MAXLEN, ST_GRADED);
    }
    csr_to_ell<<<grid_for(n0), TB, 0, st>>>(n0, L0->ld, indptr0, indices0, data0, L0->acol.as<int32_t>(),
                                           L0->aval.as<double>(), L0->avalf.as<float>(),
                                           L0->alen.as<int32_t>(), L0->dinv.as<double>(), L0->wfix,
                                           L0->d16 ? L0->adcol.as<int16_t>() : nullptr);
    NODAL_HIP_TRY(h, hipGetLastError());
    for (int l = 0; l + 1 < H->nlev; ++l) {
        SLevel *L = H->pool[l], *C = H->pool[l + 1];
        Ell A = L->A();
        A.width = L->maxlen;
        build_P<<<grid_for(L->n), TB, 0, st>>>(A, L->dinv.as<double>(), L->agg.as<int32_t>(), L->pcol.as<int32_t>(),
                                              L->pval.as<double>(), L->pvalf.as<float>(), omega_p(l));
        const bool forked = H->aux != nullptr && nodal_extra_streams_ok(h) &&
                            knob::SA_FORK.now();
        hipStream_t rst = st;
        if (forked) {
            NODAL_HIP_TRY(h, hipEventRecord(H->ev_fork, st));
            NODAL_HIP_TRY(h, hipStreamWaitEvent(H->aux, H->ev_fork, 0));
            H->aux_pending = true;
            NODAL_TRY(galerkin_product<true>(h, H, l, nullptr, 1));
            rst = H->aux;
        }
        r_refresh<<<grid_for(C->n * 8), TB, 0, rst>>>(C->n, L->rld, L->rlen.as<int32_t>(), L->rcol.as<int32_t>(), L->ld,
                                                     L->pcol.as<int32_t>(), L->pval.as<double>(), L->rval.as<double>(),
                                                     L->rvalf.as<float>());
        NODAL_HIP_TRY(h, hipGetLastError());
        if (forked) NODAL_HIP_TRY(h, hipEventRecord(H->ev_join, H->aux));
        NODAL_TRY(galerkin_product<true>(h, H, l, forked ? H->ev_join : nullptr, forked ? 2 : 0));
        if (forked) H->aux_pending = false;
    }
    const int last = H->nlev - 1;
    if (H->dense_coarsest)
        coarsest_inverse<<<1, 256, 0, st>>>(H->pool[last]->A(), H->coarse_inv.as<double>(), dstats + (size_t)last * ST_COUNT);
    if (H->tail >= 0) k_tail_pack<<<1, 1024, 0, st>>>(H->td, H->tail_image.as<char>());
    NODAL_HIP_TRY(h, hipGetLastError());
    NODAL_TRY(form_tail_op(h, H));
    NODAL_TRY(build_visit(h, H, general));
    NODAL_HIP_TRY(h, hipMemcpyAsync(hs, dstats, (size_t)MAX_LEVELS * ST_COUNT * 8, hipMemcpyDeviceToHost, st));
    NODAL_WAIT_STREAM(h, st);
    const int64_t bar = n0 / 100 < 32 ? (n0 / 100 > 0 ? n0 / 100 : 1) : 32;
    if (hs[ST_BADDIAG] || (int64_t)hs[ST_GRADED] >= bar) return NODAL_OK;
    for (int k = 1; k < H->nlev; ++k)
        if (hs[(size_t)k * ST_COUNT + ST_BADDIAG] || hs[(size_t)k * ST_COUNT + ST_OVERFLOW]) return NODAL_OK;
    decide_folds(H, hs, false);
    NODAL_TRY(fold_self_check(h, H));
    NODAL_TRY(visit_self_check(h, H));
    *ok = true;
    return NODAL_OK;
}

}

void sagg_destroy(nodal_ctx *h) {
    delete static_cast<SHierarchy *>(h->sagg);
    h->sagg = nullptr;
}

static int sagg_setup_csr_body(nodal_ctx *h, int64_t n0, int64_t nnz0, const int32_t *indptr0, const int32_t *indices0,
                               const double *data0, bool general, bool check_floating, bool *accepted, int32_t *floating);

int sagg_setup_csr(nodal_ctx *h, int64_t n0, int64_t nnz0, const int32_t *indptr0, const int32_t *indices0,
                   const double *data0, bool general, bool check_floating, bool *accepted, int32_t *floating) {
    const int s = sagg_setup_csr_body(h, n0, nnz0, indptr0, indices0, data0, general, check_floating, accepted, floating);
    SHierarchy *H = static_cast<SHierarchy *>(h->sagg);
    if (H && H->aux && H->aux_pending && H->ev_flags) {
        if (hipEventRecord(H->ev_flags, H->aux) == hipSuccess) (void)hipStreamWaitEvent(h->stream, H->ev_flags, 0);
        H->aux_pending = false;
        (void)hipGetLastError();
    }
    return s;
}

static int sagg_setup_csr_body(nodal_ctx *h, int64_t n0, int64_t nnz0, const int32_t *indptr0, const int32_t *indices0,
                               const double *data0, bool general, bool check_floating, bool *accepted, int32_t *floating) {
    *accepted = false;
    *floating = 0;
    static const bool enabled = knob::SAGG.now();
    static const bool trace = knob::TRACE.now();
    if (!enabled) return NODAL_OK;
    SHierarchy *H = hierarchy_of(h);
    H->ready = false;
    hipStream_t st = h->stream;
    if (n0 >= (1ll << 30)) return NODAL_OK;
    static const bool reuse = knob::SA_REUSE.now();
    if (reuse && H->sym_valid && H->sym_epoch == h->struct_epoch && H->sym_n == n0 && H->sym_nnz == nnz0 &&
        H->sym_general == general && H->sym_check == check_floating) {
        bool ok = false;
        NODAL_TRY(sagg_refresh(h, H, indptr0, indices0, data0, general, &ok));
        if (ok) {
            *floating = H->sym_floating;
            H->refreshed = true;
            H->ready = true;
            *accepted = true;
            if (trace) fprintf(stderr, "[sagg] symbolic setup kept (struct epoch %llu): values refreshed\n",
                               (unsigned long long)h->struct_epoch);
            return NODAL_OK;
        }
        if (trace) fprintf(stderr, "[sagg] the kept hierarchy does not take the new values: full setup\n");
    }
    H->sym_valid = false;
    H->refreshed = false;
    H->want_flags = check_floating;
    H->flags_levels = 0;
    H->last_iters = 0;
    H->drop_graph();
    NODAL_HIP_TRY(h, H->stats.reserve((size_t)MAX_LEVELS * ST_COUNT * 8 + 64));
    if (!H->host_stats)
        NODAL_HIP_TRY(h, hipHostMalloc(reinterpret_cast<void **>(&H->host_stats), (size_t)MAX_LEVELS * ST_COUNT * 8 + 64));
    unsigned long long *dstats = H->stats.as<unsigned long long>();
    unsigned long long *hs = reinterpret_cast<unsigned long long *>(H->host_stats);
    NODAL_HIP_TRY(h, hipMemsetAsync(dstats, 0, (size_t)MAX_LEVELS * ST_COUNT * 8, st));
    NODAL_HIP_TRY(h, H->bstat.reserve((size_t)2 * BSTAT_MAX * 4 + 64));
    {
        const unsigned gr = grid_for(n0);
        static const double spread = knob::SA_SPREAD.now();
        static const double share = knob::SA_SHARE.now();
        row_stats<<<gr, TB, 0, st>>>(n0, indptr0, indices0, data0, share, spread, general, dstats, H->bstat.as<uint32_t>());
        reduce_bstat<<<1, 1024, 0, st>>>((int)gr, H->bstat.as<uint32_t>(), dstats, ST_MAXLEN, ST_GRADED);
    }
    NODAL_HIP_TRY(h, hipGetLastError());
    NODAL_HIP_TRY(h, hipMemcpyAsync(hs, dstats, ST_COUNT * 8, hipMemcpyDeviceToHost, st));
    NODAL_WAIT_STREAM(h, st);
    const int64_t bar = n0 / 100 < 32 ? (n0 / 100 > 0 ? n0 / 100 : 1) : 32;
    if (hs[ST_MAXLEN] > (unsigned long long)W0_MAX || hs[ST_MAXLEN] == 0 || hs[ST_BADDIAG] ||
        (int64_t)hs[ST_GRADED] >= bar) {
        if (trace)
            fprintf(stderr, "[sagg] declined: longest row %llu, graded nodes %llu (bar %lld), M-matrix %s\n",
                    hs[ST_MAXLEN], hs[ST_GRADED], (long long)bar, hs[ST_BADDIAG] ? "no" : "yes");
        return NODAL_OK;
    }
    SLevel *L0 = H->level(0);
    L0->n = n0;
    L0->ld = pad64(n0);
    L0->maxlen = (int32_t)hs[ST_MAXLEN];
    L0->nnz = nnz0;
    L0->wfix = choose_wfix(L0->maxlen, n0, nnz0, 8);
    L0->width = L0->wfix ? L0->wfix : L0->maxlen;
    NODAL_HIP_TRY(h, L0->acol.reserve((size_t)L0->width * L0->ld * 4 + 64));
    NODAL_HIP_TRY(h, L0->aval.reserve((size_t)L0->width * L0->ld * 8 + 64));
    NODAL_HIP_TRY(h, L0->avalf.reserve((size_t)L0->width * L0->ld * 4 + 64));
    NODAL_HIP_TRY(h, L0->alen.reserve((size_t)L0->ld * 4 + 64));
    NODAL_HIP_TRY(h, L0->dinv.reserve((size_t)L0->ld * 8 + 64));
    static const bool d16_env = knob::SA_D16.now();
    L0->d16 = d16_env && hs[ST_FARCOL] == 0;
    if (L0->d16) NODAL_HIP_TRY(h, L0->adcol.reserve((size_t)L0->width * L0->ld * 2 + 64));
    csr_to_ell<<<grid_for(n0), TB, 0, st>>>(n0, L0->ld, indptr0, indices0, data0, L0->acol.as<int32_t>(),
                                           L0->aval.as<double>(), L0->avalf.as<float>(),
                                           L0->alen.as<int32_t>(), L0->dinv.as<double>(), L0->wfix,
                                           L0->d16 ? L0->adcol.as<int16_t>() : nullptr);
    NODAL_HIP_TRY(h, hipGetLastError());

    int l = 0;
    bool diag_last = false;
    for (;; ++l) {
        SLevel *L = H->level(l);
        if (L->n <= COARSEST && l > 0) break;
        if (l + 1 >= MAX_LEVELS) {
            if (trace) fprintf(stderr, "[sagg] declined: more than %d levels\n", MAX_LEVELS);
            return NODAL_OK;
        }
        bool declined = false, stop = false;
        NODAL_TRY(build_level(h, H, l, hs, &declined, &stop));
        if (declined) {
            if (trace)
                fprintf(stderr, "[sagg] declined at level %d (%lld rows): does not coarsen / over a cap / not positive "
                                "(this level: overflow %llx baddiag %llx; level above: overflow %llx unassigned %llu maxr %llu)\n",
                        l, (long long)L->n, hs[(size_t)l * ST_COUNT + ST_OVERFLOW], hs[(size_t)l * ST_COUNT + ST_BADDIAG],
                        l > 0 ? hs[(size_t)(l - 1) * ST_COUNT + ST_OVERFLOW] : 0ull,
                        l > 0 ? hs[(size_t)(l - 1) * ST_COUNT + ST_UNASSIGNED] : 0ull,
                        l > 0 ? hs[(size_t)(l - 1) * ST_COUNT + ST_MAXR] : 0ull);
            return NODAL_OK;
        }
        if (stop) {
            diag_last = true;
            break;
        }
    }
    H->nlev = l + 1;
    SLevel *last = H->level(l);
    last->fold_want = last->fold = false;
    if (H->nlev < 2) return NODAL_OK;
    NODAL_HIP_TRY(h, hipMemcpyAsync(hs, dstats, (size_t)MAX_LEVELS * ST_COUNT * 8, hipMemcpyDeviceToHost, st));
    if (!H->ev_copy) NODAL_HIP_TRY(h, hipEventCreateWithFlags(&H->ev_copy, hipEventDisableTiming));
    NODAL_HIP_TRY(h, hipEventRecord(H->ev_copy, st));
    if (check_floating) {
        if (H->flags_levels == 0) {
            NODAL_HIP_TRY(h, H->level(0)->gflag.reserve((size_t)n0 + 64));
            NODAL_TRY(grounded_flags(h, H->level(0)->gflag.as<uint8_t>()));
        } else {
            NODAL_HIP_TRY(h, hipStreamWaitEvent(st, H->ev_flags, 0));
            H->aux_pending = false;
        }
        for (int k = H->flags_levels; k + 1 < H->nlev; ++k) {
            SLevel *L = H->pool[k], *C = H->pool[k + 1];
            NODAL_HIP_TRY(h, C->gflag.reserve((size_t)C->n + 64));
            NODAL_HIP_TRY(h, hipMemsetAsync(C->gflag.p, 0, ((size_t)C->n + 63) & ~(size_t)63, st));
            flags_up<<<grid_for(L->n), TB, 0, st>>>(L->n, L->agg.as<int32_t>(), L->gflag.as<uint8_t>(),
                                                   C->gflag.as<uint8_t>());
        }
        NODAL_HIP_TRY(h, hipGetLastError());
    }
    NODAL_WAIT_EVENT(h, H->ev_copy, st);
    for (int k = 0; k < H->nlev; ++k) {
        const unsigned long long *s = hs + (size_t)k * ST_COUNT;
        if (k > 0) {
            H->pool[k]->maxlen = (int32_t)s[ST_MAXLEN];
            H->pool[k]->nnz = (int64_t)s[ST_NNZ];
            H->pool[k]->wfix = choose_wfix(H->pool[k]->maxlen, H->pool[k]->n, H->pool[k]->nnz, APAD);
        }
        if (s[ST_OVERFLOW] || (k > 0 && s[ST_BADDIAG]) || s[ST_UNASSIGNED]) {
            if (trace) fprintf(stderr, "[sagg] declined: level %d over a cap / not positive\n", k);
            return NODAL_OK;
        }
    }
    diag_last = last->maxlen <= 1;
    H->dense_coarsest = !diag_last;
    if (H->dense_coarsest) {
        if (last->n > COARSEST) return NODAL_OK;
        NODAL_HIP_TRY(h, H->coarse_inv.reserve((size_t)last->n * last->n * 8 + 64));
        coarsest_inverse<<<1, 256, 0, st>>>(last->A(), H->coarse_inv.as<double>(),
                                            dstats + (size_t)l * ST_COUNT);
        NODAL_HIP_TRY(h, hipGetLastError());
    }
    for (int k = 0; k < H->nlev; ++k) {
        SLevel *L = H->pool[k];
        NODAL_HIP_TRY(h, L->vec.reserve((size_t)V_COUNT * L->ld * 8 + 256));
        NODAL_HIP_TRY(h, L->part.reserve(5 * DOT_BLOCKS * 8 + 512));
    }
    NODAL_TRY(build_tail(h, H, hs));
    NODAL_TRY(build_visit(h, H, general));

    if (!check_floating) {
        NODAL_HIP_TRY(h, hipMemcpyAsync(hs, dstats, (size_t)MAX_LEVELS * ST_COUNT * 8, hipMemcpyDeviceToHost, st));
        NODAL_WAIT_STREAM(h, st);
        if (hs[(size_t)l * ST_COUNT + ST_BADDIAG] & 2ull) return NODAL_OK;
    } else {
        uint32_t *fl = reinterpret_cast<uint32_t *>(dstats + (size_t)(MAX_LEVELS - 1) * ST_COUNT + ST_COUNT - 1);
        if (H->dense_coarsest) last_level_floating<<<1, 64, 0, st>>>(last->A(), last->gflag.as<uint8_t>(), fl);
        else any_unflagged<<<grid_for(last->n), TB, 0, st>>>(last->n, last->gflag.as<uint8_t>(), fl);
        NODAL_HIP_TRY(h, hipGetLastError());
        NODAL_HIP_TRY(h, hipMemcpyAsync(hs, dstats, (size_t)MAX_LEVELS * ST_COUNT * 8, hipMemcpyDeviceToHost, st));
        NODAL_WAIT_STREAM(h, st);
        if (hs[(size_t)l * ST_COUNT + ST_BADDIAG] & 2ull) {
            if (trace) fprintf(stderr, "[sagg] declined: coarsest matrix not positive definite\n");
            return NODAL_OK;
        }
        *floating = hs[(size_t)(MAX_LEVELS - 1) * ST_COUNT + ST_COUNT - 1] != 0 ? 1 : 0;
    }
    if (trace) {
        fprintf(stderr, "[sagg] levels (rows/entries/longest row/padded width):");
        for (int k = 0; k < H->nlev; ++k)
            fprintf(stderr, " %lld/%lld/%d/%d", (long long)H->pool[k]->n, (long long)H->pool[k]->nnz,
                    H->pool[k]->maxlen, H->pool[k]->wfix);
        fprintf(stderr, "  tail %d (%d register slots)  coarsest %s\n", H->tail, H->tail >= 0 ? H->td.slots : 0,
                H->dense_coarsest ? "dense" : "diagonal");
    }
    decide_folds(H, hs, trace);
    NODAL_TRY(fold_self_check(h, H));
    NODAL_TRY(visit_self_check(h, H));
    H->ready = true;
    *accepted = true;
    H->sym_valid = true;
    H->sym_epoch = h->struct_epoch;
    H->sym_n = n0;
    H->sym_nnz = nnz0;
    H->sym_general = general;
    H->sym_check = check_floating;
    H->sym_floating = *floating;
    memcpy(H->sym_stats, hs, sizeof H->sym_stats);
    return NODAL_OK;
}

int sagg_setup(nodal_ctx *h, bool *accepted, int32_t *floating) {
    return sagg_setup_csr(h, h->n, h->nnz, h->indptr.as<int32_t>(), h->indices.as<int32_t>(), h->data.as<double>(),
                          false, true, accepted, floating);
}

namespace {

int last_level(nodal_ctx *h, SHierarchy *H, int l, const double *b, double *out) {
    hipStream_t st = h->stream;
    SLevel *L = H->pool[l];
    const int64_t n = L->n;
    if (l == H->tail) return H->tail_dense ? tail_apply<1>(h, H, b, out) : tail_walk(h, H, b, out, 1);
    k_coarsest<<<grid_for(n), TB, 0, st>>>(n, H->dense_coarsest ? H->coarse_inv.as<double>() : nullptr,
                                           L->dinv.as<double>(), b, out);
    NODAL_HIP_TRY(h, hipGetLastError());
    return NODAL_OK;
}

void kcycle_schedule(SHierarchy *H, int it) {
    static const bool on = knob::SA_KFREEZE.now();
    H->kfrozen = false;
    H->kslot = -1;
    if (!on || it < 0) return;
    if (it == 0) H->ksamples = 0;
    const bool adaptive = it < 4 || (it & 3) == 0;
    if (!adaptive && H->ksamples > 0) {
        H->kfrozen = true;
    } else if (it >= 2) {
        H->kslot = H->ksamples % 3;
        ++H->ksamples;
        H->kcount = H->ksamples < 3 ? H->ksamples : 3;
    }
}

int visit_three(nodal_ctx *h, SHierarchy *H, int l, const cyc_t *b, const cyc_t *x0, cyc_t *out) {
    hipStream_t st = h->stream;
    SLevel *L = H->pool[l], *C = H->pool[l + 1];
    const Ell A = L->A();
    const double *dinv = L->dinv.as<double>();
    cyc_t *x1 = L->v<cyc_t>(V_X1), *x2 = L->v<cyc_t>(V_T);
    double *rc = C->v<double>(V_RC), *c1 = C->v<double>(V_C1);
    const int nt = (int)C->n;
    const unsigned g = grid_for(L->n);
    SAGG_DISPATCH_W(L->wfix, (k_visit_first<W><<<g + (unsigned)nt, TB, 0, st>>>(A, dinv, b, x0, x1, g, L->d2.as<float>(), rc)));
    SAGG_DISPATCH_W(L->wfix, (k_visit_second<W><<<g + (unsigned)((nt + 3) / 4), TB, 0, st>>>(A, dinv, b, x1, x2, g, nt,
                                                                                             H->tail_op.as<double>(), rc, c1)));
    SAGG_DISPATCH_W(L->wfix, (k_visit_last<W><<<grid_for(L->n * VL), TB, 0, st>>>(A, dinv, b, x2, out, L->p2col.as<int32_t>(), L->p2val.as<float>(),
                                                                L->p2len.as<int32_t>(), c1)));
    NODAL_HIP_TRY(h, hipGetLastError());
    return NODAL_OK;
}

template <typename TBV, typename TOUT>
int cycle(nodal_ctx *h, SHierarchy *H, int l, const TBV *b, const cyc_t *x0, TOUT *out, const SolveBufs *sb) {
    hipStream_t st = h->stream;
    SLevel *L = H->pool[l];
    const int64_t n = L->n;
    SLevel *C = H->pool[l + 1];
    const int64_t nc = C->n;
    const Ell A = L->A();
    const double *dinv = L->dinv.as<double>();
    const cyc_t *x = x0;
    cyc_t *r = L->v<cyc_t>(V_R), *xp = L->v<cyc_t>(V_XP);
    const unsigned g = sb ? (unsigned)sb->g0 : grid_for(n);
    const unsigned tb = L->wfix ? TB : TB * LPR_RAGGED;
    const int nu = H->nu[l < 2 ? l : 2];
    const bool fold = L->fold && !(sb && nu == 1);
    if constexpr (std::is_same_v<TBV, cyc_t> && std::is_same_v<TOUT, cyc_t>) {
        if (L->visit && !sb && nu == 2 && l + 1 == H->tail && H->tail_dense) return visit_three(h, H, l, b, x0, out);
    }
    auto hand_up =[&](const auto *c1, const auto *c2, const double *cf) {
        using TC = std::remove_cv_t<std::remove_pointer_t<decltype(c1)>>;
        if (!fold)
            k_prolong<TC><<<grid_for(n), TB, 0, st>>>(n, L->ld, L->pcol.as<int32_t>(), L->pvalf.as<float>(), x, c1, c2, cf, xp);
        else if (nu == 1)
            k_prolong_post<TC, TOUT><<<grid_for(n), TB, 0, st>>>(n, L->ld, L->wcol.as<int32_t>(), L->wval.as<float>(),
                                                               L->wlen.as<int32_t>(), x, r, dinv, c1, c2, cf, out);
        else
            k_prolong_post<TC, cyc_t><<<grid_for(n), TB, 0, st>>>(n, L->ld, L->wcol.as<int32_t>(), L->wval.as<float>(),
                                                                L->wlen.as<int32_t>(), x, r, dinv, c1, c2, cf, xp);
    };
    if (nu >= 2) {
        cyc_t *x1 = L->v<cyc_t>(V_X1);
        SAGG_DISPATCH_W(L->wfix, (k_post<W, false, TBV, cyc_t><<<g, tb, 0, st>>>(A, dinv, b, x0, x1, nullptr, nullptr, nullptr)));
        x = x1;
    }
    if (nu >= 3) {
        cyc_t *x2 = L->v<cyc_t>(V_T);
        SAGG_DISPATCH_W(L->wfix, (k_post<W, false, TBV, cyc_t><<<g, tb, 0, st>>>(A, dinv, b, x, x2, nullptr, nullptr, nullptr)));
        x = x2;
    }
    SAGG_DISPATCH_W(L->wfix, (k_smooth_residual<W, TBV><<<g, tb, 0, st>>>(A, b, x, r)));
    const bool last = l + 1 == H->tail || l + 1 == H->nlev - 1;
    const double *coef = nullptr;
    if (last) {
        double *rc = C->v<double>(V_RC), *c1 = C->v<double>(V_C1);
        k_restrict<double><<<grid_for(nc * RL), TB, 0, st>>>(nc, L->rld, L->rcol.as<int32_t>(), L->rvalf.as<float>(),
                                                            L->rlen.as<int32_t>(), r, rc, C->dinv.as<double>(), nullptr);
        NODAL_HIP_TRY(h, hipGetLastError());
        NODAL_TRY(last_level(h, H, l + 1, rc, c1));
        hand_up((const double *)c1, (const double *)nullptr, nullptr);
    } else {
        cyc_t *rc = C->v<cyc_t>(V_RC), *c1 = C->v<cyc_t>(V_C1), *c2 = C->v<cyc_t>(V_C2), *x0c = C->v<cyc_t>(V_X);
        k_restrict<cyc_t><<<grid_for(nc * RL), TB, 0, st>>>(nc, L->rld, L->rcol.as<int32_t>(), L->rvalf.as<float>(),
                                                           L->rlen.as<int32_t>(), r, rc, C->dinv.as<double>(), x0c);
        NODAL_HIP_TRY(h, hipGetLastError());
        int nparts = 0;
        const bool kcycle = l < H->klevels && H->kcycle;
        if (kcycle) {
            cyc_t *v1 = C->v<cyc_t>(V_V1), *v2 = C->v<cyc_t>(V_V2), *r2 = C->v<cyc_t>(V_R2);
            double *part = C->part.as<double>();
            const Ell Ac = C->A();
            const unsigned gd = grid_for(nc, DOT_BLOCKS);
            const unsigned tbc = C->wfix ? TB : TB * LPR_RAGGED;
            nparts = (int)gd;
            double *cf = part + 5 * DOT_BLOCKS;
            if (H->kfrozen && l == 0) {
                NODAL_TRY((cycle<cyc_t, cyc_t>(h, H, l + 1, rc, x0c, c1, nullptr)));
                SAGG_DISPATCH_W(C->wfix, (k_spmv_resid<W><<<gd, tbc, 0, st>>>(Ac, c1, rc, cf + 3, r2, C->dinv.as<double>(), x0c)));
                NODAL_HIP_TRY(h, hipGetLastError());
                NODAL_TRY((cycle<cyc_t, cyc_t>(h, H, l + 1, r2, x0c, c2, nullptr)));
                coef = cf + 3;
                nparts = 0;
            } else {
                NODAL_TRY((cycle<cyc_t, cyc_t>(h, H, l + 1, rc, x0c, c1, nullptr)));
                SAGG_DISPATCH_W(C->wfix, (k_spmv_dots<W><<<gd, tbc, 0, st>>>(Ac, c1, v1, rc, nullptr, part + 0 * DOT_BLOCKS,
                                                                            part + 1 * DOT_BLOCKS, nullptr)));
                k_second_residual<<<grid_for(nc), TB, 0, st>>>(nc, rc, v1, part, nparts, r2, C->dinv.as<double>(), x0c);
                NODAL_HIP_TRY(h, hipGetLastError());
                NODAL_TRY((cycle<cyc_t, cyc_t>(h, H, l + 1, r2, x0c, c2, nullptr)));
                SAGG_DISPATCH_W(C->wfix, (k_spmv_dots<W><<<gd, tbc, 0, st>>>(Ac, c2, v2, v1, r2, part + 3 * DOT_BLOCKS,
                                                                            part + 2 * DOT_BLOCKS, part + 4 * DOT_BLOCKS)));
                NODAL_HIP_TRY(h, hipGetLastError());
            }
        } else {
            NODAL_TRY((cycle<cyc_t, cyc_t>(h, H, l + 1, rc, x0c, c1, nullptr)));
        }
        if (nparts) {
            double *cf = C->part.as<double>() + 5 * DOT_BLOCKS;
            const bool sample = l == 0 && H->kslot >= 0;
            k_kcoef<<<1, 320, 0, st>>>(C->part.as<double>(), nparts, cf, sample ? H->kslot : -1, sample ? H->kcount : 0);
            coef = cf;
        }
        hand_up((const cyc_t *)c1, (const cyc_t *)c2, coef);
    }
    const cyc_t *cur = xp;
    const int left = fold ? nu - 1 : nu;
    if (left == 0) {
        NODAL_HIP_TRY(h, hipGetLastError());
        return NODAL_OK;
    }
    if (left >= 2) {
        cyc_t *mid = L->v<cyc_t>(V_T);
        SAGG_DISPATCH_W(L->wfix, (k_post<W, false, TBV, cyc_t><<<g, tb, 0, st>>>(A, dinv, b, cur, mid, nullptr, nullptr, nullptr)));
        cur = mid;
    }
    if (left >= 3) {
        cyc_t *mid2 = L->v<cyc_t>(V_X1);
        SAGG_DISPATCH_W(L->wfix, (k_post<W, false, TBV, cyc_t><<<g, tb, 0, st>>>(A, dinv, b, cur, mid2, nullptr, nullptr, nullptr)));
        cur = mid2;
    }
    if (sb) {
        SAGG_DISPATCH_W(L->wfix, (k_post<W, true, TBV, TOUT><<<g, tb, 0, st>>>(A, dinv, b, cur, out, sb->Ap, sb->part_rz,
                                                                              sb->part_zap)));
    } else {
        SAGG_DISPATCH_W(L->wfix, (k_post<W, false, TBV, TOUT><<<g, tb, 0, st>>>(A, dinv, b, cur, out, nullptr, nullptr, nullptr)));
    }
    NODAL_HIP_TRY(h, hipGetLastError());
    return NODAL_OK;
}

__global__ void f_set_scalars(double *__restrict__ sc, double tol2) {
    for (int k = 0; k < F_COUNT; ++k) sc[k] = 0.0;
    sc[F_TOL2] = tol2;
}

size_t align_up(size_t x) { return (x + 255) & ~(size_t)255; }

int visit_check_level(nodal_ctx *h, SHierarchy *H, int l) {
    hipStream_t st = h->stream;
    SLevel *L = H->pool[l], *C = H->pool[l + 1];
    const int64_t n = L->n, ld = L->ld, nt = C->n;
    uint64_t seed = 0x9e3779b97f4a7c15ull + 977ull * (uint64_t)l;
    auto unit = [&]() {
        uint64_t z = (seed += 0x9e3779b97f4a7c15ull);
        z = (z ^ (z >> 30)) * 0xbf58476d1ce4e5b9ull;
        z = (z ^ (z >> 27)) * 0x94d049bb133111ebull;
        z ^= z >> 31;
        return (double)(z >> 11) * (1.0 / 4503599627370496.0) - 1.0;
    };
    std::vector<double> dinv((size_t)n), T((size_t)nt * nt), c6((size_t)nt), c3((size_t)nt);
    std::vector<cyc_t> hb((size_t)n), hx0((size_t)n), x1((size_t)n), x2((size_t)n), r((size_t)n), xp((size_t)n),
        o6((size_t)n), o3((size_t)n);
    std::vector<int32_t> acol((size_t)L->width * ld), alen((size_t)n), pcol((size_t)PW * ld), wcol((size_t)L->wslots * ld),
        wlen((size_t)n), p2col((size_t)P2CAP * ld), p2len((size_t)n);
    std::vector<float> aval((size_t)L->width * ld), pval((size_t)PW * ld), wval((size_t)L->wslots * ld),
        p2val((size_t)P2CAP * ld);
    auto down = [&](void *dst, const void *src, size_t bytes) { return hipMemcpy(dst, src, bytes, hipMemcpyDeviceToHost); };
    hipError_t e = hipStreamSynchronize(st);
    if (e == hipSuccess) e = down(dinv.data(), L->dinv.p, (size_t)n * 8);
    for (int64_t i = 0; i < n; ++i) {
        hb[i] = (cyc_t)unit();
        hx0[i] = (cyc_t)(OMEGA * dinv[i] * (double)hb[i]);
    }
    const size_t vb = align256((size_t)n * sizeof(cyc_t));
    DevBuf buf;
    if (e == hipSuccess) e = buf.reserve(4 * vb);
    char *p = buf.as<char>();
    cyc_t *b = reinterpret_cast<cyc_t *>(p), *x0 = reinterpret_cast<cyc_t *>(p + vb), *out6 = reinterpret_cast<cyc_t *>(p + 2 * vb),
          *out3 = reinterpret_cast<cyc_t *>(p + 3 * vb);
    if (e == hipSuccess) e = hipMemcpyAsync(b, hb.data(), (size_t)n * sizeof(cyc_t), hipMemcpyHostToDevice, st);
    if (e == hipSuccess) e = hipMemcpyAsync(x0, hx0.data(), (size_t)n * sizeof(cyc_t), hipMemcpyHostToDevice, st);
    int rc = NODAL_OK;
    if (e == hipSuccess) {
        L->visit = false;
        rc = cycle<cyc_t, cyc_t>(h, H, l, b, x0, out6, nullptr);
        L->visit = true;
    }
    if (e == hipSuccess && rc == NODAL_OK) e = hipStreamSynchronize(st);
    if (e == hipSuccess) e = down(r.data(), L->v<cyc_t>(V_R), (size_t)n * sizeof(cyc_t));
    if (e == hipSuccess) e = down(xp.data(), L->v<cyc_t>(V_XP), (size_t)n * sizeof(cyc_t));
    if (e == hipSuccess) e = down(c6.data(), C->v<double>(V_C1), (size_t)nt * 8);
    if (e == hipSuccess && rc == NODAL_OK) rc = cycle<cyc_t, cyc_t>(h, H, l, b, x0, out3, nullptr);
    if (e == hipSuccess && rc == NODAL_OK) e = hipStreamSynchronize(st);
    if (e == hipSuccess) e = down(x1.data(), L->v<cyc_t>(V_X1), (size_t)n * sizeof(cyc_t));
    if (e == hipSuccess) e = down(x2.data(), L->v<cyc_t>(V_T), (size_t)n * sizeof(cyc_t));
    if (e == hipSuccess) e = down(c3.data(), C->v<double>(V_C1), (size_t)nt * 8);
    if (e == hipSuccess) e = down(o6.data(), out6, (size_t)n * sizeof(cyc_t));
    if (e == hipSuccess) e = down(o3.data(), out3, (size_t)n * sizeof(cyc_t));
    if (e == hipSuccess) e = down(acol.data(), L->acol.p, acol.size() * 4);
    if (e == hipSuccess) e = down(aval.data(), L->avalf.p, aval.size() * 4);
    if (e == hipSuccess) e = down(alen.data(), L->alen.p, (size_t)n * 4);
    if (e == hipSuccess) e = down(pcol.data(), L->pcol.p, pcol.size() * 4);
    if (e == hipSuccess) e = down(pval.data(), L->pvalf.p, pval.size() * 4);
    if (e == hipSuccess) e = down(wcol.data(), L->wcol.p, wcol.size() * 4);
    if (e == hipSuccess) e = down(wval.data(), L->wval.p, wval.size() * 4);
    if (e == hipSuccess) e = down(wlen.data(), L->wlen.p, (size_t)n * 4);
    if (e == hipSuccess) e = down(p2col.data(), L->p2col.p, p2col.size() * 4);
    if (e == hipSuccess) e = down(p2val.data(), L->p2val.p, p2val.size() * 4);
    if (e == hipSuccess) e = down(p2len.data(), L->p2len.p, (size_t)n * 4);
    if (e == hipSuccess) e = down(T.data(), H->tail_op.p, (size_t)nt * nt * 8);
    buf.release();
    if (rc != NODAL_OK) return rc;
    NODAL_HIP_TRY(h, e);
    using Vec = std::vector<double>;
    auto absv = [](const auto &v) { Vec y(v.size()); for (size_t i = 0; i < v.size(); ++i) y[i] = fabs((double)v[i]); return y; };
    auto add = [](Vec a, const Vec &b2) { for (size_t i = 0; i < a.size(); ++i) a[i] += b2[i]; return a; };
    auto wd = [&](Vec v) { for (int64_t i = 0; i < n; ++i) v[i] *= OMEGA * dinv[i]; return v; };
    auto absA = [&](const Vec &v) {
        Vec y((size_t)n, 0.0);
        for (int64_t i = 0; i < n; ++i)
            for (int32_t s = 0; s < alen[i]; ++s) y[i] += fabs((double)aval[(size_t)s * ld + i]) * v[acol[(size_t)s * ld + i]];
        return y;
    };
    auto absG = [&](const Vec &v) { return add(v, wd(absA(v))); };
    auto absGT = [&](const Vec &v) { return add(v, absA(wd(v))); };
    auto ell = [&](int slots, const std::vector<int32_t> &col, const std::vector<float> &val, const std::vector<int32_t> *len,
                   const Vec &v, bool transposed) {
        Vec y((size_t)(transposed ? nt : n), 0.0);
        for (int64_t i = 0; i < n; ++i) {
            const int32_t m = len ? (*len)[i] : slots;
            for (int32_t s = 0; s < m; ++s) {
                const int32_t J = col[(size_t)s * ld + i];
                if (J < 0) continue;
                const double a = fabs((double)val[(size_t)s * ld + i]);
                if (transposed) y[J] += a * v[i];
                else y[i] += a * v[J];
            }
        }
        return y;
    };
    auto absT = [&](const Vec &v) {
        Vec y((size_t)nt, 0.0);
        for (int64_t i = 0; i < nt; ++i)
            for (int64_t j = 0; j < nt; ++j) y[i] += fabs(T[(size_t)i * nt + j]) * v[j];
        return y;
    };
    auto Pt = [&](const Vec &v) { return ell(PW, pcol, pval, nullptr, v, true); };
    auto Wm = [&](const Vec &v) { return ell(L->wslots, wcol, wval, &wlen, v, false); };
    auto Wt = [&](const Vec &v) { return ell(L->wslots, wcol, wval, &wlen, v, true); };
    auto P2m = [&](const Vec &v) { return ell(P2CAP, p2col, p2val, &p2len, v, false); };
    auto P2t = [&](const Vec &v) { return ell(P2CAP, p2col, p2val, &p2len, v, true); };
    const Vec ax1 = absA(absv(x1));
    const Vec e_r = add(absv(r), ax1);
    const Vec e_c6 = absT(Pt(add(absv(r), e_r)));
    const Vec e_xp = add(add(absv(xp), wd(e_r)), add(Wm(absv(c6)), Wm(e_c6)));
    const Vec dev6 = add(add(absv(o6), absG(e_xp)), wd(absA(absv(xp))));
    const Vec e_x2 = add(absv(x2), wd(ax1));
    const Vec e_c3 = absT(add(P2t(absv(hb)), Wt(absGT(absv(hb)))));
    const Vec ac3 = absv(c3);
    const Vec dev3 = add(add(add(absv(o3), absG(e_x2)), wd(absA(absv(x2)))), add(add(P2m(ac3), absG(Wm(ac3))), P2m(e_c3)));
    double dm = 0.0;
    int maxp2 = 0;
    for (int64_t i = 0; i < n; ++i) {
        const double di = fabs((double)o3[i] - (double)o6[i]) / (dev6[i] + dev3[i]);
        dm = !(di <= dm) ? di : dm;
        maxp2 = p2len[i] > maxp2 ? p2len[i] : maxp2;
    }
    fprintf(stderr, "[sagg] visit check: level %d, rows %lld, n_t %lld, longest P2 row %d, three launches against the six "
                    "d = %.3e (against the bound 2^-23: %.3e)\n", l, (long long)n, (long long)nt, maxp2, dm, dm / 0x1p-23);
    return NODAL_OK;
}
int visit_self_check(nodal_ctx *h, SHierarchy *H) {
    static const bool check = knob::TRACE.now() && knob::SA_VISIT_CHECK.now();
    if (!check) return NODAL_OK;
    for (int l = 1; l + 1 < H->nlev; ++l) {
        const SLevel *L = H->pool[l];
        if (L->visit && l + 1 == H->tail && H->tail_dense && H->nu[l < 2 ? l : 2] == 2) NODAL_TRY(visit_check_level(h, H, l));
    }
    return NODAL_OK;
}

}

__global__ __launch_bounds__(TB) void k_x0(int64_t n, const double *__restrict__ dinv, const double *__restrict__ r,
                                           cyc_t *__restrict__ x0) {
    for (int64_t i = (int64_t)xcd_block() * TB + threadIdx.x; i < n; i += (int64_t)gridDim.x * TB)
        x0[i] = (cyc_t)(OMEGA * dinv[i] * r[i]);
}
bool sagg_ready(nodal_ctx *h, int64_t n) {
    SHierarchy *H = static_cast<SHierarchy *>(h->sagg);
    return H && H->ready && H->pool[0]->n == n;
}
void sagg_invalidate(nodal_ctx *h) {
    if (h->sagg) static_cast<SHierarchy *>(h->sagg)->ready = false;
}
int sagg_levels(nodal_ctx *h) { return h->sagg ? static_cast<SHierarchy *>(h->sagg)->nlev : 0; }

static SHierarchy *debug_hierarchy(nodal_ctx *h, nodal_ctx **owner) {
    for (nodal_ctx *c : {h, h->reduced}) {
        SHierarchy *H = c ? static_cast<SHierarchy *>(c->sagg) : nullptr;
        if (H && H->ready && H->nlev >= 1 && H->nlev <= MAX_LEVELS && (int)H->pool.size() >= H->nlev) {
            *owner = c;
            return H;
        }
    }
    return nullptr;
}

int sagg_debug_info(nodal_ctx *h, int32_t *nlev, int64_t *ints, double *reals) {
    nodal_ctx *c = nullptr;
    SHierarchy *H = debug_hierarchy(h, &c);
    if (!H) return nodal_fail(h, NODAL_E_INVALID, "debug hierarchy: the handle holds no ready hierarchy");
    *nlev = H->nlev;
    memset(ints, 0, sizeof(int64_t) * MAX_LEVELS * 16);
    memset(reals, 0, sizeof(double) * MAX_LEVELS * 2);
    for (int l = 0; l < H->nlev; ++l) {
        const SLevel *L = H->pool[l];
        const bool next = l + 1 < H->nlev;
        int64_t *w = ints + (size_t)l * 16;
        w[0] = L->n; w[1] = L->ld; w[2] = next ? L->nc : 0; w[3] = L->width; w[4] = L->maxlen; w[5] = L->wfix;
        w[6] = L->nnz; w[7] = next ? L->rld : 0; w[8] = next ? rcap_for(L->nc) : 0; w[9] = next ? L->wslots : 0;
        w[10] = next && L->fold_want; w[11] = next && L->fold; w[12] = L->d16; w[13] = H->tail >= 0 && l >= H->tail;
        w[14] = H->refreshed; w[15] = H->dense_coarsest;
        reals[(size_t)l * 2] = omega_p(l);
        reals[(size_t)l * 2 + 1] = OMEGA;
    }
    return NODAL_OK;
}

int sagg_debug_array(nodal_ctx *h, int32_t level, int32_t which, void *dst, int64_t capacity_bytes, int64_t *bytes_out) {
    nodal_ctx *c = nullptr;
    SHierarchy *H = debug_hierarchy(h, &c);
    if (!H) return nodal_fail(h, NODAL_E_INVALID, "debug hierarchy: the handle holds no ready hierarchy");
    const DevBuf *buf = nullptr;
    int64_t bytes = 0;
    if (level == -1) {
        const int64_t nl = H->pool[H->nlev - 1]->n;
        buf = &H->coarse_inv;
        bytes = H->dense_coarsest ? nl * nl * 8 : 0;
    } else {
        if (level < 0 || level >= H->nlev) return nodal_fail(h, NODAL_E_INVALID, "debug hierarchy: no such level");
        const SLevel *L = H->pool[level];
        const bool next = level + 1 < H->nlev;
        const int64_t slots = (int64_t)L->width * L->ld, pslots = next ? (int64_t)PW * L->ld : 0;
        const int64_t rslots = next ? (int64_t)rcap_for(L->nc) * L->rld : 0;
        const int64_t wslots = next && L->fold_want ? (int64_t)L->wslots * L->ld : 0;
        switch (which) {
        case NODAL_HA_ACOL: buf = &L->acol; bytes = slots * 4; break;
        case NODAL_HA_AVAL: buf = &L->aval; bytes = slots * 8; break;
        case NODAL_HA_AVALF: buf = &L->avalf; bytes = slots * 4; break;
        case NODAL_HA_ALEN: buf = &L->alen; bytes = L->n * 4; break;
        case NODAL_HA_DINV: buf = &L->dinv; bytes = L->n * 8; break;
        case NODAL_HA_ADCOL: buf = &L->adcol; bytes = L->d16 ? slots * 2 : 0; break;
        case NODAL_HA_AGG: buf = &L->agg; bytes = next ? L->n * 4 : 0; break;
        case NODAL_HA_PCOL: buf = &L->pcol; bytes = pslots * 4; break;
        case NODAL_HA_PVAL: buf = &L->pval; bytes = pslots * 8; break;
        case NODAL_HA_PVALF: buf = &L->pvalf; bytes = pslots * 4; break;
        case NODAL_HA_RCOL: buf = &L->rcol; bytes = rslots * 4; break;
        case NODAL_HA_RVAL: buf = &L->rval; bytes = rslots * 8; break;
        case NODAL_HA_RVALF: buf = &L->rvalf; bytes = rslots * 4; break;
        case NODAL_HA_RLEN: buf = &L->rlen; bytes = next ? L->nc * 4 : 0; break;
        case NODAL_HA_WCOL: buf = &L->wcol; bytes = wslots * 4; break;
        case NODAL_HA_WVAL: buf = &L->wval; bytes = wslots * 4; break;
        case NODAL_HA_WLEN: buf = &L->wlen; bytes = wslots ? L->n * 4 : 0; break;
        case NODAL_HA_P2COL: buf = &L->p2col; bytes = next && L->visit_want ? (int64_t)P2CAP * L->ld * 4 : 0; break;
        case NODAL_HA_P2VAL: buf = &L->p2val; bytes = next && L->visit_want ? (int64_t)P2CAP * L->ld * 4 : 0; break;
        case NODAL_HA_P2LEN: buf = &L->p2len; bytes = next && L->visit_want ? L->n * 4 : 0; break;
        case NODAL_HA_D2: buf = &L->d2; bytes = next && L->visit_want ? L->nc * L->ld * 4 : 0; break;
        default: return nodal_fail(h, NODAL_E_INVALID, "debug hierarchy: no such array");
        }
    }
    if (bytes < 0 || (bytes > 0 && (!buf->p || (size_t)bytes > buf->cap)))
        return nodal_fail(h, NODAL_E_INVALID, "debug hierarchy: the level's buffer is smaller than its extent");
    *bytes_out = bytes;
    if (!dst || bytes == 0) return NODAL_OK;
    if (capacity_bytes < bytes) return nodal_fail(h, NODAL_E_INVALID, "debug hierarchy: destination too small");
    NODAL_WAIT_STREAM(h, c->stream);
    if (H->aux) NODAL_WAIT_STREAM(h, H->aux);
    NODAL_HIP_TRY(h, hipMemcpyAsync(dst, buf->p, (size_t)bytes, hipMemcpyDeviceToHost, c->stream));
    NODAL_WAIT_STREAM(h, c->stream);
    return NODAL_OK;
}

bool sagg_x0_slot(nodal_ctx *h, const double **dinv, nodal_cyc_t **x0, int64_t *n0, double *omega) {
    SHierarchy *H = static_cast<SHierarchy *>(h->sagg);
    if (!H || !H->ready) return false;
    SLevel *L0 = H->pool[0];
    *dinv = L0->dinv.as<double>();
    *x0 = L0->v<cyc_t>(V_X);
    *n0 = L0->n;
    *omega = OMEGA;
    return true;
}
int sagg_apply(nodal_ctx *h, const double *r, double *z, bool x0_ready, int it) {
    SHierarchy *H = static_cast<SHierarchy *>(h->sagg);
    if (!H || !H->ready) return nodal_fail(h, NODAL_E_INVALID, "sagg_setup_csr not called");
    SLevel *L0 = H->pool[0];
    cyc_t *x0 = L0->v<cyc_t>(V_X);
    if (!x0_ready) k_x0<<<grid_for(L0->n), TB, 0, h->stream>>>(L0->n, L0->dinv.as<double>(), r, x0);
    NODAL_HIP_TRY(h, hipGetLastError());
    kcycle_schedule(H, it);
    const int rc = cycle<double, double>(h, H, 0, r, x0, z, nullptr);
    H->kfrozen = false;
    H->kslot = -1;
    return rc;
}

int sagg_spmv(nodal_ctx *h, const double *x, double *y, hipEvent_t start, hipEvent_t stop) {
    SHierarchy *H = static_cast<SHierarchy *>(h->sagg);
    if (!H || !H->ready) return nodal_fail(h, NODAL_E_INVALID, "sagg_setup_csr not called");
    const SLevel *L0 = H->pool[0];
    const Ell A0 = L0->A();
    const unsigned tb0 = L0->wfix ? TB : TB * LPR_RAGGED;
    if (start && stop) {
        SAGG_DISPATCH_W(L0->wfix, (hipExtLaunchKernelGGL((k_ell_spmv<W>), dim3(grid_for(L0->n)), dim3(tb0), 0, h->stream,
                                                         start, stop, 0, A0, x, y)));
    } else {
        SAGG_DISPATCH_W(L0->wfix, (k_ell_spmv<W><<<grid_for(L0->n), tb0, 0, h->stream>>>(A0, x, y)));
    }
    NODAL_HIP_TRY(h, hipGetLastError());
    return NODAL_OK;
}

int sagg_fcg_solve(nodal_ctx *h, const double *b, bool do_setup, int32_t *info, int32_t *iters, double *resid) {
    static const bool trace = knob::TRACE.now();
    const int64_t n = h->n;
    hipStream_t st = h->stream;
    SHierarchy *H = hierarchy_of(h);
    if (do_setup) {
        bool accepted = false;
        int32_t floating = 0;
        NODAL_TRY(sagg_setup(h, &accepted, &floating));
        if (!accepted) return SAGG_DECLINED;
        if (floating) {
            *info = 1;
            *iters = 0;
            *resid = 0.0;
            return -2;
        }
    }
    if (!H->ready || H->pool[0]->n != n) return SAGG_DECLINED;
    h->amg_levels = H->nlev;
    static const int kc = knob::SA_KCYCLE.now();
    H->kcycle = kc != 0;
    H->klevels = knob::SA_KLEVELS.now();
    apply_nu_knob(H);

    const size_t vec = align_up((size_t)n * 8);
    NODAL_HIP_TRY(h, h->solver.reserve(6 * vec + 4 * MAX_PARTIALS * 8 + F_COUNT * 8 + 256));
    char *base = h->solver.as<char>();
    SolveBufs sb;
    sb.r = reinterpret_cast<double *>(base);
    sb.z = reinterpret_cast<cyc_t *>(base + vec);
    sb.p = reinterpret_cast<double *>(base + 2 * vec);
    sb.Ap = reinterpret_cast<double *>(base + 3 * vec);
    sb.x0 = reinterpret_cast<cyc_t *>(base + 4 * vec);
    sb.p2 = reinterpret_cast<double *>(base + 5 * vec);
    sb.part_rz = reinterpret_cast<double *>(base + 6 * vec);
    sb.part_zap = sb.part_rz + MAX_PARTIALS;
    sb.part_rr = sb.part_zap + MAX_PARTIALS;
    sb.part_pap = sb.part_rr + MAX_PARTIALS;
    sb.sc = sb.part_pap + MAX_PARTIALS;
    sb.g0 = (int)grid_for(n, MAX_PARTIALS);
    double *x = h->x.as<double>();
    const Ell A0 = H->pool[0]->A();

    const double tol = 1e-13;
    f_set_scalars<<<1, 1, 0, st>>>(sb.sc, tol * tol);
    const double *dinv0 = H->pool[0]->dinv.as<double>();
    f_init<<<sb.g0, TB, 0, st>>>(b, x, sb.r, sb.Ap, dinv0, sb.x0, sb.part_rr, n);
    NODAL_HIP_TRY(h, hipGetLastError());

    const int64_t maxit = knob::FCG_MAXIT.now().value_or(2000);
    hipEvent_t e0 = h->ev[2], e1 = h->ev[3];
    h->kern_ms = 0;
    h->kern_launches = 0;
    double hs[F_COUNT];
    int64_t enqueued = 0;
    int batch = 6;
    if (H->last_iters > 6 && (H->refreshed || !do_setup)) batch = H->last_iters + 1 > 32 ? 32 : H->last_iters + 1;
    else if (H->hint_iters > 8 && H->hint_n == n && H->hint_nnz == H->pool[0]->nnz) {
        batch = (3 * H->hint_iters) / 4;
        if (batch > 32) batch = 32;
    }
    int status = 0;
    const bool poll_partials = knob::FCG_HOST_SUM.now();
    double rr_prev = -1.0;
    int64_t it_prev = 0;
    int polls = 0;
    static const bool fuse_dir_env = knob::SA_FUSE_DIR.now();
    const bool fuse_dir = fuse_dir_env && LPR_RAGGED == 1;
    static const bool graphs_env = knob::SA_GRAPH.now();
    auto iteration = [&](int it, bool timed) -> int {
        kcycle_schedule(H, graphs_env ? -1 : it);
        struct KReset {
            SHierarchy *H;
            ~KReset() { H->kfrozen = false; H->kslot = -1; }
        } kreset{H};
        NODAL_TRY((cycle<double, cyc_t>(h, H, 0, sb.r, sb.x0, sb.z, &sb)));
        if (fuse_dir) {
            double *p_new = (it & 1) ? sb.p2 : sb.p;
            const double *p_old = (it & 1) ? sb.p : sb.p2;
            const unsigned tbf = TB;
            if (timed) {
                SAGG_DISPATCH_W(H->pool[0]->wfix, (hipExtLaunchKernelGGL((f_dir_spmv<W>), dim3(sb.g0), dim3(tbf), 0, st, e0, e1, 0,
                                                                         A0, (const cyc_t *)sb.z, p_old, p_new, sb.Ap,
                                                                         (const double *)sb.part_rz, (const double *)sb.part_zap,
                                                                         (const double *)sb.part_rr, sb.g0, sb.part_pap, sb.sc,
                                                                         it & 1)));
            } else {
                SAGG_DISPATCH_W(H->pool[0]->wfix, (f_dir_spmv<W><<<sb.g0, tbf, 0, st>>>(A0, sb.z, p_old, p_new, sb.Ap, sb.part_rz,
                                                                                       sb.part_zap, sb.part_rr, sb.g0,
                                                                                       sb.part_pap, sb.sc, it & 1)));
            }
            f_update<<<sb.g0, TB, 0, st>>>(x, sb.r, p_new, sb.Ap, sb.part_pap, sb.g0, dinv0, sb.x0, sb.part_rr, sb.sc, it & 1, n);
            NODAL_HIP_TRY(h, hipGetLastError());
            return NODAL_OK;
        }
        f_direction<<<sb.g0, TB, 0, st>>>(sb.z, sb.p, sb.part_rz, sb.part_zap, sb.part_rr, sb.g0, sb.sc, it & 1, n);
        const unsigned tb0 = H->pool[0]->wfix ? TB : TB * LPR_RAGGED;
        if (timed) {
// ... 152 lines not shown
```

nodal_amd/csrc/sagg_cycle.h:

```cpp
#pragma once

namespace {

constexpr int LPR_RAGGED = 1;
template <int W> struct RowLanes { static constexpr int value = W == 0 ? LPR_RAGGED : 1; };

template <class VT, class XF>
__device__ __forceinline__ double ell_row_lanes(const Ell &A, const VT *__restrict__ val, int64_t i, int sub, XF xf) {
    constexpr int Q = 8;
    const int32_t len = A.len[i];
    double acc = 0.0;
    for (int32_t s0 = sub; s0 < len; s0 += LPR_RAGGED * Q) {
        int32_t c[Q];
        double v[Q];
        if (A.dcol) {
#pragma unroll
            for (int q = 0; q < Q; ++q) {
                const bool ok = s0 + q * LPR_RAGGED < len;
                const int64_t at = (int64_t)(ok ? s0 + q * LPR_RAGGED : s0) * A.ld + i;
                c[q] = (int32_t)i + (int32_t)A.dcol[at];
                const VT loaded = val[at];
                v[q] = ok ? (double)loaded : 0.0;
            }
        } else {
// ... 749 lines not shown
        for (int c = 0; c < NV; ++c) {
            const double v = wave_sum(s[c]);
            if (lane == 0) out[(int64_t)i * NV + c] = v;
        }
    }
}

static_assert(LPR_RAGGED == 1 && TB == 256, "the visit's launches mix row blocks and dense-row blocks of 256 threads");

__device__ __forceinline__ unsigned xcd_block_sub(unsigned first, unsigned count) {
    const unsigned b = blockIdx.x - first;
    return (count & 7u) ? b : (b & 7u) * (count >> 3) + (b >> 3);
}

template <int W>
__device__ __forceinline__ void visit_sweep_rows(const Ell &A, const double *__restrict__ dinv, const cyc_t *__restrict__ b,
                                                 const cyc_t *__restrict__ xin, cyc_t *__restrict__ xout, unsigned vb,
                                                 unsigned count) {
    for (int64_t i = (int64_t)vb * TB + threadIdx.x; i < A.n; i += (int64_t)count * TB) {
        const double s = ell_row_w<W>(A, A.valf, i, 0, [&](int32_t j) { return (double)xin[j]; });
        xout[i] = (cyc_t)fma(OMEGA * dinv[i], (double)b[i] - s, (double)xin[i]);
    }
}

template <int W>
__global__ __launch_bounds__(TB) void k_visit_first(Ell A, const double *__restrict__ dinv, const cyc_t *__restrict__ b,
                                                    const cyc_t *__restrict__ x0, cyc_t *__restrict__ x1, unsigned grows,
                                                    const float *__restrict__ D2, double *__restrict__ rc) {
    if (blockIdx.x < grows) {
        visit_sweep_rows<W>(A, dinv, b, x0, x1, xcd_block_sub(0, grows), grows);
        return;
    }
    __shared__ double ws[TB / 64];
    const int64_t I = (int64_t)(blockIdx.x - grows);
    const float4 *row = reinterpret_cast<const float4 *>(D2 + I * A.ld);
    const float4 *bv = reinterpret_cast<const float4 *>(b);
    const int pieces = (int)(A.ld >> 2);
    constexpr int U = 10;
    double s0 = 0.0, s1 = 0.0;
    for (int p0 = threadIdx.x; p0 < pieces; p0 += TB * U) {
        float4 d[U], v[U];
#pragma unroll
        for (int u = 0; u < U; ++u) {
            const int p = p0 + TB * u;
            d[u] = row[p < pieces ? p : p0];
            v[u] = bv[p < pieces ? p : p0];
        }
#pragma unroll
        for (int u = 0; u < U; ++u) {
            const int p = p0 + TB * u;
            if (p >= pieces) continue;
            const int64_t j = (int64_t)p * 4;
            if (j + 0 < A.n && d[u].x != 0.0f) s0 = fma((double)d[u].x, (double)v[u].x, s0);
            if (j + 1 < A.n && d[u].y != 0.0f) s1 = fma((double)d[u].y, (double)v[u].y, s1);
            if (j + 2 < A.n && d[u].z != 0.0f) s0 = fma((double)d[u].z, (double)v[u].z, s0);
            if (j + 3 < A.n && d[u].w != 0.0f) s1 = fma((double)d[u].w, (double)v[u].w, s1);
        }
    }
    const double s = wave_sum(s0 + s1);
    if ((threadIdx.x & 63) == 0) ws[threadIdx.x >> 6] = s;
    __syncthreads();
    if (threadIdx.x == 0) {
        double t = 0.0;
#pragma unroll
        for (int w = 0; w < TB / 64; ++w) t += ws[w];
        rc[I] = t;
    }
}

template <int W>
__global__ __launch_bounds__(TB) void k_visit_second(Ell A, const double *__restrict__ dinv, const cyc_t *__restrict__ b,
                                                     const cyc_t *__restrict__ x1, cyc_t *__restrict__ x2, unsigned grows,
                                                     int nt, const double *__restrict__ T, const double *__restrict__ rc,
                                                     double *__restrict__ c) {
    if (blockIdx.x < grows) {
        visit_sweep_rows<W>(A, dinv, b, x1, x2, xcd_block_sub(0, grows), grows);
        return;
    }
    const int i = (int)(blockIdx.x - grows) * 4 + (int)(threadIdx.x >> 6);
    if (i >= nt) return;
    tail_apply_row<TAIL_MAX_N / 64>(nt, T, rc, c, i, (int)(threadIdx.x & 63));
}

constexpr int P2CAP = 64;
constexpr int VL = 4;
template <int W>
__global__ __launch_bounds__(TB) void k_visit_last(Ell A, const double *__restrict__ dinv, const cyc_t *__restrict__ b,
                                                   const cyc_t *__restrict__ x2, cyc_t *__restrict__ out,
                                                   const int32_t *__restrict__ p2col, const float *__restrict__ p2val,
                                                   const int32_t *__restrict__ p2len, const double *__restrict__ c) {
    constexpr int PQ = P2CAP / VL, AQ = W > 0 ? (W + VL - 1) / VL : 8, ROWS = TB / VL;
    static_assert(P2CAP % VL == 0 && TB % VL == 0 && 64 % VL == 0, "whole rows per wavefront");
    const int sub = threadIdx.x & (VL - 1);
    for (int64_t i = (int64_t)xcd_block() * ROWS + threadIdx.x / VL; i < A.n; i += (int64_t)gridDim.x * ROWS) {
        const int32_t len = p2len[i];
        int32_t J[PQ];
        float w[PQ];
#pragma unroll
        for (int j = 0; j < PQ; ++j) {
            J[j] = p2col[(int64_t)(sub + VL * j) * A.ld + i];
            w[j] = p2val[(int64_t)(sub + VL * j) * A.ld + i];
        }
        double s = 0.0;
        if constexpr (W > 0) {
            int32_t ca[AQ];
            float va[AQ];
#pragma unroll
            for (int j = 0; j < AQ; ++j) {
                const int q = sub + VL * j;
                const int64_t at = (int64_t)(q < W ? q : 0) * A.ld + i;
                ca[j] = A.col[at];
                va[j] = A.valf[at];
            }
#pragma unroll
            for (int j = 0; j < AQ; ++j) {
                const double xv = (double)x2[ca[j]];
                if (sub + VL * j < W) s = fma((double)va[j], xv, s);
            }
        } else {
            const int32_t la = A.len[i];
            for (int32_t s0 = sub; s0 < la; s0 += VL * AQ) {
                int32_t ca[AQ];
                float va[AQ];
#pragma unroll
                for (int j = 0; j < AQ; ++j) {
                    const int32_t q = s0 + VL * j;
                    const int64_t at = (int64_t)(q < la ? q : s0) * A.ld + i;
                    ca[j] = A.col[at];
                    va[j] = A.valf[at];
                }
#pragma unroll
                for (int j = 0; j < AQ; ++j) {
                    const double xv = (double)x2[ca[j]];
                    if (s0 + VL * j < la) s = fma((double)va[j], xv, s);
                }
            }
        }
        double acc = 0.0;
#pragma unroll
        for (int j = 0; j < PQ; ++j) {
            const bool ok = sub + VL * j < len;
            const double cv = c[ok ? J[j] : 0];
            if (ok) acc = fma((double)w[j], cv, acc);
        }
#pragma unroll
        for (int off = VL >> 1; off > 0; off >>= 1) {
            s += __shfl_xor(s, off, 64);
            acc += __shfl_xor(acc, off, 64);
        }
        if (sub == 0) out[i] = (cyc_t)(fma(OMEGA * dinv[i], (double)b[i] - s, (double)x2[i]) + acc);
    }
}

enum { F_RZ = 0, F_ALPHA = 2, F_CONV = 4, F_RR = 6, F_BB = 7, F_FLAG = 8, F_ITERS = 9, F_TOL2 = 10,
       F_ITNO = 12,
       F_COUNT = 16 };
constexpr int MAX_PARTIALS = 1024;

__global__ __launch_bounds__(TB) void f_init(const double *__restrict__ b, double *__restrict__ x,
                                             double *__restrict__ r, double *__restrict__ Ap,
                                             const double *__restrict__ dinv, cyc_t *__restrict__ x0,
                                             double *__restrict__ part_rr, int64_t n) {
    double srr = 0.0;
    for (int64_t i = (int64_t)xcd_block() * TB + threadIdx.x; i < n; i += (int64_t)gridDim.x * TB) {
        const double ri = b[i];
        x[i] = 0.0;
        r[i] = ri;
        x0[i] = (cyc_t)(OMEGA * dinv[i] * ri);
        Ap[i] = 0.0;
        srr = fma(ri, ri, srr);
    }
    srr = block_sum(srr);
    if (threadIdx.x == 0) part_rr[blockIdx.x] = srr;
}

__global__ __launch_bounds__(TB) void f_direction(const cyc_t *__restrict__ z, double *__restrict__ p,
                                                  const double *__restrict__ part_rz,
                                                  const double *__restrict__ part_zap,
                                                  const double *__restrict__ part_rr, int nparts,
                                                  double *__restrict__ sc, int parity, int64_t n) {
    const int cur = parity & 1, prev = cur ^ 1;
    constexpr int FD_PRE = 4;
    const int64_t i0 = (int64_t)xcd_block() * TB + threadIdx.x, stride = (int64_t)gridDim.x * TB;
    cyc_t zq[FD_PRE];
    double pq[FD_PRE];
#pragma unroll
    for (int u = 0; u < FD_PRE; ++u) {
        const int64_t i = i0 + u * stride, ii = i < n ? i : n - 1;
        zq[u] = z[ii];
        pq[u] = p[ii];
    }
    const int iter = (int)sc[F_ITNO + prev];
    if (blockIdx.x == 0 && threadIdx.x == 0) sc[F_ITNO + cur] = (double)(iter + 1);
    if (iter > 0 && sc[F_CONV + prev] != 0.0) {
        if (blockIdx.x == 0 && threadIdx.x == 0) sc[F_CONV + cur] = 1.0;
        return;
    }
    double rz_new, zap, rr;
    reduce_partials3(part_rz, part_zap, part_rr, nparts, rz_new, zap, rr);
    const double rz_old = iter > 0 ? sc[F_RZ + prev] : 1.0;
    const double beta = (iter > 0 && rz_old != 0.0) ? -sc[F_ALPHA + prev] * zap / rz_old : 0.0;
    const double bb = iter == 0 ? rr : sc[F_BB];
    const bool bad = !(rz_new >= 0.0) || !(rr == rr);
    const bool converged = bb == 0.0 || rr <= sc[F_TOL2] * bb || bad;
    if (blockIdx.x == 0 && threadIdx.x == 0) {
        sc[F_RZ + cur] = rz_new;
        sc[F_RR] = rr;
        if (iter == 0) sc[F_BB] = rr;
        if (bad) sc[F_FLAG] = 1.0;
        sc[F_CONV + cur] = converged ? 1.0 : 0.0;
        if (converged) sc[F_ITERS] = (double)iter;
    }
    if (converged) return;
#pragma unroll
    for (int u = 0; u < FD_PRE; ++u) {
        const int64_t i = i0 + u * stride;
        if (i < n) p[i] = iter > 0 ? fma(beta, pq[u], (double)zq[u]) : (double)zq[u];
    }
    for (int64_t i = i0 + FD_PRE * stride; i < n; i += stride)
        p[i] = iter > 0 ? fma(beta, p[i], (double)z[i]) : (double)z[i];
}

template <int W>
__global__ __launch_bounds__(TB * RowLanes<W>::value) void k_ell_spmv(Ell A, const double *__restrict__ x,
                                                                      double *__restrict__ y) {
    constexpr int LPR = RowLanes<W>::value, NT = TB * LPR;
    const int sub = threadIdx.x & (LPR - 1);
    for (int64_t t = (int64_t)xcd_block() * NT + threadIdx.x; t / LPR < A.n; t += (int64_t)gridDim.x * NT) {
        const int64_t i = t / LPR;
        const double s = ell_row_w<W>(A, A.val, i, sub, [&](int32_t j) { return x[j]; });
        if (sub == 0) y[i] = s;
    }
}

template <int W>
__global__ __launch_bounds__(TB * RowLanes<W>::value) void f_spmv(Ell A, const double *__restrict__ p, double *__restrict__ Ap,
                                             double *__restrict__ part_pap, const double *__restrict__ sc,
                                             int iter) {
    if (sc[F_CONV + (iter & 1)] != 0.0) return;
    double acc = 0.0;
    constexpr int LPR = RowLanes<W>::value, NT = TB * LPR;
    const int sub = threadIdx.x & (LPR - 1);
    for (int64_t t = (int64_t)xcd_block() * NT + threadIdx.x; t / LPR < A.n; t += (int64_t)gridDim.x * NT) {
        const int64_t i = t / LPR;
        const double s = ell_row_w<W>(A, A.val, i, sub, [&](int32_t j) { return p[j]; });
        if (sub != 0) continue;
        Ap[i] = s;
        acc = fma(p[i], s, acc);
    }
    acc = block_sum<NT>(acc);
    if (threadIdx.x == 0) part_pap[blockIdx.x] = acc;
}

template <int W>
__global__ __launch_bounds__(TB * RowLanes<W>::value) void f_dir_spmv(Ell A, const cyc_t *__restrict__ z,
                                                 const double *__restrict__ p_old, double *__restrict__ p_new,
                                                 double *__restrict__ Ap, const double *__restrict__ part_rz,
                                                 const double *__restrict__ part_zap, const double *__restrict__ part_rr,
                                                 int nparts, double *__restrict__ part_pap, double *__restrict__ sc,
                                                 int parity) {
    static_assert(RowLanes<W>::value == 1, "the reduction of the partials assumes TB threads");
    const int cur = parity & 1, prev = cur ^ 1;
    const int64_t i0 = (int64_t)xcd_block() * TB + threadIdx.x, stride = (int64_t)gridDim.x * TB;
    int32_t c0[W > 0 ? W : 1];
    double v0[W > 0 ? W : 1];
    const int64_t ifirst = i0 < A.n ? i0 : A.n - 1;
    if constexpr (W > 0) ell_row_load<W>(A, A.val, ifirst, c0, v0);
    const cyc_t zfirst = z[ifirst];
    const double pfirst = p_old[ifirst];
    const int iter = (int)sc[F_ITNO + prev];
    if (blockIdx.x == 0 && threadIdx.x == 0) sc[F_ITNO + cur] = (double)(iter + 1);
    if (iter > 0 && sc[F_CONV + prev] != 0.0) {
        if (blockIdx.x == 0 && threadIdx.x == 0) sc[F_CONV + cur] = 1.0;
        return;
    }
    double rz_new, zap, rr;
    reduce_partials3(part_rz, part_zap, part_rr, nparts, rz_new, zap, rr);
    const double rz_old = iter > 0 ? sc[F_RZ + prev] : 1.0;
    const double beta = (iter > 0 && rz_old != 0.0) ? -sc[F_ALPHA + prev] * zap / rz_old : 0.0;
    const double bb = iter == 0 ? rr : sc[F_BB];
    const bool bad = !(rz_new >= 0.0) || !(rr == rr);
    const bool converged = bb == 0.0 || rr <= sc[F_TOL2] * bb || bad;
    if (blockIdx.x == 0 && threadIdx.x == 0) {
        sc[F_RZ + cur] = rz_new;
        sc[F_RR] = rr;
        if (iter == 0) sc[F_BB] = rr;
        if (bad) sc[F_FLAG] = 1.0;
        sc[F_CONV + cur] = converged ? 1.0 : 0.0;
        if (converged) sc[F_ITERS] = (double)iter;
    }
    if (converged) return;
    const bool first = iter == 0;
    auto pn = [&](int32_t j) { return first ? (double)z[j] : fma(beta, p_old[j], (double)z[j]); };
    double acc = 0.0;
    for (int64_t i = i0; i < A.n; i += stride) {
        double s, pi;
        if (W > 0 && i == i0) {
            s = ell_row_sum<W>(i, c0, v0, pn);
            pi = first ? (double)zfirst : fma(beta, pfirst, (double)zfirst);
        } else {
            s = ell_row_w<W>(A, A.val, i, 0, pn);
            pi = pn((int32_t)i);
        }
        p_new[i] = pi;
        Ap[i] = s;
        acc = fma(pi, s, acc);
// ... 58 lines not shown
```

Before: 169.9 circuits/s.

## Compute coarse restriction from b via W^T alongside residual launch

Builds a transposed, sorted CSR form of the W operator (W^T) for each eligible level during setup, on the aux stream. Within the cycle, a single fused launch splits its blocks between computing the fine residual and computing the coarse restricted vector directly from b through W^T. This removes the dependency of the restriction on the residual and saves one launch per level. In exchange it adds setup work and memory (sort, pack and refresh of W^T), applies only when nu==1 and the level folds without visiting, and includes a host-side self-check.

```diff
diff --git a/include/nodal_hip.h b/include/nodal_hip.h
--- a/include/nodal_hip.h
+++ b/include/nodal_hip.h
@@ -187,7 +187,8 @@
     NODAL_HA_ACOL = 0, NODAL_HA_AVAL = 1, NODAL_HA_AVALF = 2, NODAL_HA_ALEN = 3, NODAL_HA_DINV = 4, NODAL_HA_ADCOL = 5,
     NODAL_HA_AGG = 6, NODAL_HA_PCOL = 7, NODAL_HA_PVAL = 8, NODAL_HA_PVALF = 9, NODAL_HA_RCOL = 10, NODAL_HA_RVAL = 11,
     NODAL_HA_RVALF = 12, NODAL_HA_RLEN = 13, NODAL_HA_WCOL = 14, NODAL_HA_WVAL = 15, NODAL_HA_WLEN = 16,
-    NODAL_HA_P2COL = 17, NODAL_HA_P2VAL = 18, NODAL_HA_P2LEN = 19, NODAL_HA_D2 = 20
+    NODAL_HA_P2COL = 17, NODAL_HA_P2VAL = 18, NODAL_HA_P2LEN = 19, NODAL_HA_D2 = 20,
+    NODAL_HA_WTSTART = 21, NODAL_HA_WTCOL = 22, NODAL_HA_WTVAL = 23, NODAL_HA_WTSRC = 24
 };
 int nodal_debug_hierarchy_info(nodal_handle h, int32_t *nlev, int64_t *ints , double *reals );
 int nodal_debug_hierarchy_array(nodal_handle h, int32_t level, int32_t which, void *dst, int64_t capacity_bytes,
diff --git a/nodal_amd/_ffi.py b/nodal_amd/_ffi.py
--- a/nodal_amd/_ffi.py
+++ b/nodal_amd/_ffi.py
@@ -91,7 +91,8 @@
                     ("pval", np.float64), ("pvalf", np.float32), ("rcol", np.int32), ("rval", np.float64),
                     ("rvalf", np.float32), ("rlen", np.int32), ("wcol", np.int32), ("wval", np.float32),
                     ("wlen", np.int32), ("p2col", np.int32), ("p2val", np.float32), ("p2len", np.int32),
-                    ("d2", np.float32))
+                    ("d2", np.float32), ("wtstart", np.uint32), ("wtcol", np.int32), ("wtval", np.float32),
+                    ("wtsrc", np.int32))
 HIERARCHY_INFO = ("n", "ld", "nc", "width", "maxlen", "wfix", "nnz", "rld", "rcap", "wslots", "fold_want", "fold", "d16",
                   "in_tail", "refreshed", "dense_coarsest")
 
diff --git a/nodal_amd/csrc/knobs.h b/nodal_amd/csrc/knobs.h
--- a/nodal_amd/csrc/knobs.h
+++ b/nodal_amd/csrc/knobs.h
@@ -120,6 +120,8 @@
 inline constexpr OnUnless0 SA_FOLD_VISIT{"NODAL_SA_FOLD_VISIT"};
 inline constexpr Int64 SA_VISIT_CAP{"NODAL_SA_VISIT_CAP", 16777216};
 inline constexpr OffUnlessNon0 SA_VISIT_CHECK{"NODAL_SA_VISIT_CHECK"};
+inline constexpr OnUnless0 SA_RESTRICT_B{"NODAL_SA_RESTRICT_B"};
+inline constexpr OffUnlessNon0 SA_RESTRICT_CHECK{"NODAL_SA_RESTRICT_CHECK"};
 inline constexpr OnUnless0 SA_TAIL_DENSE{"NODAL_SA_TAIL_DENSE"};
 inline constexpr OffUnlessNon0 SA_TAIL_CHECK{"NODAL_SA_TAIL_CHECK"};
 inline constexpr Int SA_TAIL_NU{"NODAL_SA_TAIL_NU", 3};
diff --git a/nodal_amd/csrc/sagg.hip b/nodal_amd/csrc/sagg.hip
--- a/nodal_amd/csrc/sagg.hip
+++ b/nodal_amd/csrc/sagg.hip
@@ -63,7 +63,8 @@
        ST_FARCOL = 8 ,
        ST_FOLDMISS = 9 ,
        ST_VISITMISS = 10 ,
-       ST_COUNT = 11 };
+       ST_RESTRICTMISS = 11 ,
+       ST_COUNT = 12 };
 
 struct SLevel {
     int64_t n = 0, ld = 0, nc = 0;
@@ -84,6 +85,9 @@
     bool fold_want = false, fold = false;
     DevBuf p2col, p2val, p2len, d2;
     bool visit_want = false, visit = false;
+    DevBuf wtstart, wtcol, wtval, wtsrc;
+    int64_t wtcap = 0;
+    bool restrict_want = false, restrict_b = false;
     Ell A() const {
         Ell e;
         e.n = n; e.ld = ld; e.width = width;
@@ -137,6 +141,10 @@
     bool aux_tried = false;
     bool want_flags = false;
     int flags_levels = 0;
+    hipEvent_t ev_w = nullptr, ev_wt = nullptr;
+    bool wt_pending = false;
+    bool general = false;
+    DevBuf wt_scratch, wt_keys;
     DevBuf stats, coarse_inv, mis_t, mis_m, mis_flag, mis_id, agg1, keys, rstart, cursor, lists;
     TailDesc td;
     uint64_t *host_stats = nullptr;
@@ -172,11 +180,14 @@
         if (ev_fork) (void)hipEventDestroy(ev_fork);
         if (ev_join) (void)hipEventDestroy(ev_join);
         if (ev_flags) (void)hipEventDestroy(ev_flags);
+        if (ev_w) (void)hipEventDestroy(ev_w);
+        if (ev_wt) (void)hipEventDestroy(ev_wt);
         if (aux) (void)hipStreamDestroy(aux);
         for (SLevel *l : pool) {
             DevBuf *b[] = {&l->acol, &l->aval, &l->alen, &l->dinv, &l->agg, &l->pcol, &l->pval, &l->rcol,
                            &l->rval, &l->rlen, &l->vec, &l->part, &l->gflag, &l->avalf, &l->pvalf, &l->rvalf, &l->adcol,
-                           &l->wcol, &l->wval, &l->wlen, &l->p2col, &l->p2val, &l->p2len, &l->d2};
+                           &l->wcol, &l->wval, &l->wlen, &l->p2col, &l->p2val, &l->p2len, &l->d2,
+                           &l->wtstart, &l->wtcol, &l->wtval, &l->wtsrc};
             for (DevBuf *x : b) x->release();
             delete l;
         }
@@ -188,7 +199,8 @@
         apcol.release();
         apval.release();
         aplen.release();
-        DevBuf *b[] = {&stats, &coarse_inv, &mis_t, &mis_m, &mis_flag, &mis_id, &agg1, &keys, &rstart, &cursor, &lists};
+        DevBuf *b[] = {&stats, &coarse_inv, &mis_t, &mis_m, &mis_flag, &mis_id, &agg1, &keys, &rstart, &cursor, &lists,
+                       &wt_scratch, &wt_keys};
         for (DevBuf *x : b) x->release();
         if (host_stats) (void)hipHostFree(host_stats);
     }
@@ -517,24 +529,46 @@
     }
 }
 
+template <bool LEN>
+struct TKey { static constexpr int SHIFT = LEN ? 6 : 2; };
+template <bool LEN = false>
 __global__ __launch_bounds__(TB) void r_count(int64_t n, int64_t ld, const int32_t *__restrict__ pcol,
-                                              uint32_t *__restrict__ cnt, uint32_t *__restrict__ place) {
+                                              uint32_t *__restrict__ cnt, uint32_t *__restrict__ place,
+                                              const int32_t *__restrict__ len = nullptr) {
     for (int64_t i = (int64_t)xcd_block() * TB + threadIdx.x; i < n; i += (int64_t)gridDim.x * TB) {
-#pragma unroll
-        for (int k = 0; k < PW; ++k) {
-            const int32_t J = pcol[(int64_t)k * ld + i];
-            if (J >= 0) place[(int64_t)k * ld + i] = atomicAdd(&cnt[J], 1u);
-        }
-    }
-}
+        if constexpr (LEN) {
+            const int32_t m = len[i];
+            for (int32_t k = 0; k < m; ++k)
+                place[(int64_t)k * ld + i] = atomicAdd(&cnt[pcol[(int64_t)k * ld + i]], 1u);
+        } else {
+#pragma unroll
+            for (int k = 0; k < PW; ++k) {
+                const int32_t J = pcol[(int64_t)k * ld + i];
+                if (J >= 0) place[(int64_t)k * ld + i] = atomicAdd(&cnt[J], 1u);
+            }
+        }
+    }
+}
+template <bool LEN = false>
 __global__ __launch_bounds__(TB) void r_fill(int64_t n, int64_t ld, const int32_t *__restrict__ pcol,
                                              const uint32_t *__restrict__ rstart, const uint32_t *__restrict__ place,
-                                             uint64_t *__restrict__ keys) {
+                                             uint64_t *__restrict__ keys, const int32_t *__restrict__ len = nullptr,
+                                             uint32_t keycap = 0, int64_t nc = 0) {
+    if constexpr (LEN) {
+        if (rstart[nc] > keycap) return;
+    }
     for (int64_t i = (int64_t)xcd_block() * TB + threadIdx.x; i < n; i += (int64_t)gridDim.x * TB) {
-#pragma unroll
-        for (int k = 0; k < PW; ++k) {
-            const int32_t J = pcol[(int64_t)k * ld + i];
-            if (J >= 0) keys[rstart[J] + place[(int64_t)k * ld + i]] = ((uint64_t)i << 2) | (uint64_t)k;
+        if constexpr (LEN) {
+            const int32_t m = len[i];
+            for (int32_t k = 0; k < m; ++k)
+                keys[rstart[pcol[(int64_t)k * ld + i]] + place[(int64_t)k * ld + i]] =
+                    ((uint64_t)i << TKey<true>::SHIFT) | (uint64_t)k;
+        } else {
+#pragma unroll
+            for (int k = 0; k < PW; ++k) {
+                const int32_t J = pcol[(int64_t)k * ld + i];
+                if (J >= 0) keys[rstart[J] + place[(int64_t)k * ld + i]] = ((uint64_t)i << 2) | (uint64_t)k;
+            }
         }
     }
 }
@@ -612,7 +646,8 @@
 }
 
 __global__ __launch_bounds__(TB) void r_sort_short(const uint32_t *__restrict__ rstart, uint64_t *__restrict__ keys,
-                                                   int64_t nc) {
+                                                   int64_t nc, uint32_t keycap = 0xffffffffu) {
+    if (rstart[nc] > keycap) return;
     for (int64_t I = (int64_t)xcd_block() * TB + threadIdx.x; I < nc; I += (int64_t)gridDim.x * TB) {
         const uint32_t s0 = rstart[I];
         const int len = (int)(rstart[I + 1] - s0);
@@ -624,9 +659,10 @@
     }
 }
 __global__ __launch_bounds__(64) void r_sort_medium(const uint32_t *__restrict__ rstart, uint64_t *__restrict__ keys,
-                                                    int64_t nc) {
+                                                    int64_t nc, uint32_t keycap = 0xffffffffu) {
     __shared__ uint64_t buf[RCAP_SMALL];
     const int lane = threadIdx.x;
+    if (rstart[nc] > keycap) return;
     for (int64_t I = blockIdx.x; I < nc; I += gridDim.x) {
         const uint32_t s0 = rstart[I];
         const int len = (int)(rstart[I + 1] - s0);
@@ -648,6 +684,36 @@
         for (int e = lane; e < len; e += 64) keys[s0 + e] = buf[e];
         __syncthreads();
     }
+}
+
+__global__ __launch_bounds__(TB) void wt_pack(int64_t nc, const uint32_t *__restrict__ wtstart,
+                                              const uint64_t *__restrict__ keys, int64_t ld,
+                                              const float *__restrict__ wval, uint32_t cap, int32_t *__restrict__ wtcol,
+                                              float *__restrict__ wtval, int32_t *__restrict__ wtsrc,
+                                              unsigned long long *__restrict__ stats) {
+    const int lane = threadIdx.x & 63;
+    const bool over = wtstart[nc] > cap;
+    if (over && blockIdx.x == 0 && threadIdx.x == 0) atomicOr(&stats[ST_RESTRICTMISS], 2ull);
+    if (over) return;
+    for (int64_t I = (int64_t)blockIdx.x * (TB / 64) + (threadIdx.x >> 6); I < nc; I += (int64_t)gridDim.x * (TB / 64)) {
+        const uint32_t s0 = wtstart[I], l = wtstart[I + 1] - s0;
+        if (l > (uint32_t)RCAP_SMALL && lane == 0) atomicOr(&stats[ST_RESTRICTMISS], 1ull);
+        for (uint32_t t = lane; t < l; t += 64) {
+            const uint64_t key = keys[s0 + t];
+            const int64_t i = (int64_t)(key >> TKey<true>::SHIFT);
+            const int64_t src = (int64_t)(key & ((1u << TKey<true>::SHIFT) - 1)) * ld + i;
+            wtcol[s0 + t] = (int32_t)i;
+            wtval[s0 + t] = wval[src];
+            wtsrc[s0 + t] = (int32_t)src;
+        }
+    }
+}
+__global__ __launch_bounds__(TB) void wt_refresh(int64_t nc, const uint32_t *__restrict__ wtstart,
+                                                 const int32_t *__restrict__ wtsrc, const float *__restrict__ wval,
+                                                 float *__restrict__ wtval) {
+    const int64_t total = wtstart[nc];
+    for (int64_t e = (int64_t)blockIdx.x * TB + threadIdx.x; e < total; e += (int64_t)gridDim.x * TB)
+        wtval[e] = wval[wtsrc[e]];
 }
 
 __device__ __forceinline__ int wave_excl_scan(int v, int *total) {
@@ -1236,7 +1302,58 @@
         if (trace && L->visit_want)
             fprintf(stderr, "[sagg] level %d (%lld rows): visit %s\n", k, (long long)L->n,
                     L->visit ? "in three launches" : "NOT in three launches: W missing, or a row of P2 beyond its slots");
-    }
+        const unsigned long long over = hs[(size_t)k * ST_COUNT + ST_RESTRICTMISS] |
+                                        (H->sym_valid ? H->sym_stats[(size_t)k * ST_COUNT + ST_RESTRICTMISS] : 0ull);
+        L->restrict_b = L->restrict_want && L->fold && !L->visit && !over;
+        if (trace && L->restrict_want && runs_cycle)
+            fprintf(stderr, "[sagg] level %d (%lld rows): restriction %s\n", k, (long long)L->n,
+                    L->restrict_b ? "from b beside the residual launch"
+                                  : over ? "NOT from b: a row of W^T beyond the per-row sort, or more entries than its arrays hold"
+                                         : "NOT from b: W missing, or the level visits in three launches");
+    }
+}
+
+void apply_nu_knob(SHierarchy *H);
+constexpr int WT_AVG = 16;
+bool restrict_wanted(SHierarchy *H, int l, const SLevel *L) {
+    static const bool on = knob::SA_RESTRICT_B.now();
+    if (!on || l < 1 || H->general || !L->fold_want || (int64_t)L->wslots * L->ld >= (1ll << 31)) return false;
+    apply_nu_knob(H);
+    return H->nu[l < 2 ? l : 2] == 1;
+}
+int reserve_wt(nodal_ctx *h, SHierarchy *H, SLevel *L, int64_t nc) {
+    const int64_t cap = (int64_t)(L->wslots < WT_AVG ? L->wslots : WT_AVG) * L->n;
+    L->wtcap = cap;
+    NODAL_HIP_TRY(h, L->wtstart.reserve(align256((size_t)(nc + 1) * 4) + 256));
+    NODAL_HIP_TRY(h, L->wtcol.reserve((size_t)cap * 4 + 64));
+    NODAL_HIP_TRY(h, L->wtval.reserve((size_t)cap * 4 + 64));
+    NODAL_HIP_TRY(h, L->wtsrc.reserve((size_t)cap * 4 + 64));
+    NODAL_HIP_TRY(h, H->wt_keys.reserve((size_t)cap * 8 + 64));
+    NODAL_HIP_TRY(h, H->wt_scratch.reserve(align256(scan_tmp_bytes(nc + 1)) + (size_t)L->wslots * L->ld * 4 + 64));
+    return NODAL_OK;
+}
+int build_wt(nodal_ctx *h, SHierarchy *H, int l) {
+    hipStream_t st = h->stream;
+    SLevel *L = H->pool[l];
+    const int64_t n = L->n, ld = L->ld, nc = L->nc;
+    const uint32_t cap = (uint32_t)L->wtcap;
+    uint32_t *wtstart = L->wtstart.as<uint32_t>();
+    char *sc = H->wt_scratch.as<char>();
+    uint32_t *place = reinterpret_cast<uint32_t *>(sc + align256(scan_tmp_bytes(nc + 1)));
+    uint64_t *keys = H->wt_keys.as<uint64_t>();
+    const int32_t *wcol = L->wcol.as<int32_t>(), *wlen = L->wlen.as<int32_t>();
+    NODAL_HIP_TRY(h, hipMemsetAsync(wtstart, 0, align256((size_t)(nc + 1) * 4) + 256, st));
+    r_count<true><<<grid_for(n), TB, 0, st>>>(n, ld, wcol, wtstart, place, wlen);
+    NODAL_HIP_TRY(h, hipGetLastError());
+    NODAL_TRY(scan_exclusive_u32(h, wtstart, wtstart, nc + 1, nullptr, sc));
+    r_fill<true><<<grid_for(n), TB, 0, st>>>(n, ld, wcol, wtstart, place, keys, wlen, cap, nc);
+    r_sort_short<<<grid_for(nc), TB, 0, st>>>(wtstart, keys, nc, cap);
+    r_sort_medium<<<(unsigned)(nc < 8192 ? nc : 8192), 64, 0, st>>>(wtstart, keys, nc, cap);
+    wt_pack<<<grid_for(nc * 64), TB, 0, st>>>(nc, wtstart, keys, ld, L->wval.as<float>(), cap, L->wtcol.as<int32_t>(),
+                                             L->wtval.as<float>(), L->wtsrc.as<int32_t>(),
+                                             H->stats.as<unsigned long long>() + (size_t)l * ST_COUNT);
+    NODAL_HIP_TRY(h, hipGetLastError());
+    return NODAL_OK;
 }
 
 int build_level(nodal_ctx *h, SHierarchy *H, int l, unsigned long long *hs, bool *declined, bool *stop) {
@@ -1330,7 +1447,9 @@
         if (hipStreamCreateWithFlags(&H->aux, hipStreamNonBlocking) != hipSuccess) H->aux = nullptr;
         if (H->aux && ((!H->ev_fork && hipEventCreateWithFlags(&H->ev_fork, hipEventDisableTiming) != hipSuccess) ||
                        (!H->ev_join && hipEventCreateWithFlags(&H->ev_join, hipEventDisableTiming) != hipSuccess) ||
-                       (!H->ev_flags && hipEventCreateWithFlags(&H->ev_flags, hipEventDisableTiming) != hipSuccess))) {
+                       (!H->ev_flags && hipEventCreateWithFlags(&H->ev_flags, hipEventDisableTiming) != hipSuccess) ||
+                       (!H->ev_w && hipEventCreateWithFlags(&H->ev_w, hipEventDisableTiming) != hipSuccess) ||
+                       (!H->ev_wt && hipEventCreateWithFlags(&H->ev_wt, hipEventDisableTiming) != hipSuccess))) {
             (void)hipStreamDestroy(H->aux);
             H->aux = nullptr;
         }
@@ -1374,6 +1493,9 @@
             NODAL_HIP_TRY(h, L->wval.reserve((size_t)apw * ld * 4 + 64));
             NODAL_HIP_TRY(h, L->wlen.reserve((size_t)ld * 4 + 64));
         }
+        L->restrict_b = false;
+        L->restrict_want = restrict_wanted(H, l, L);
+        if (L->restrict_want) NODAL_TRY(reserve_wt(h, H, L, nc));
     }
     hipStream_t main_st = h->stream;
     struct StreamGuard {
@@ -1386,6 +1508,7 @@
         NODAL_HIP_TRY(h, hipStreamWaitEvent(H->aux, H->ev_fork, 0));
         H->aux_pending = true;
         NODAL_TRY(galerkin_product<false>(h, H, l, nullptr, 1));
+        if (L->restrict_want) NODAL_HIP_TRY(h, hipEventRecord(H->ev_w, main_st));
         h->stream = H->aux;
         st = H->aux;
     }
@@ -1425,7 +1548,17 @@
         st = main_st;
     }
     NODAL_TRY(galerkin_product<false>(h, H, l, forked ? H->ev_join : nullptr, forked ? 2 : 0));
-    if (forked && H->flags_levels != l + 1) H->aux_pending = false;
+    if (L->restrict_want && forked) {
+        NODAL_HIP_TRY(h, hipStreamWaitEvent(H->aux, H->ev_w, 0));
+        h->stream = H->aux;
+        NODAL_TRY(build_wt(h, H, l));
+        h->stream = main_st;
+        NODAL_HIP_TRY(h, hipEventRecord(H->ev_wt, H->aux));
+        H->wt_pending = true;
+    } else if (L->restrict_want) {
+        NODAL_TRY(build_wt(h, H, l));
+    }
+    if (forked && H->flags_levels != l + 1 && !H->wt_pending) H->aux_pending = false;
     return NODAL_OK;
 }
 
@@ -1735,6 +1868,7 @@
     return NODAL_OK;
 }
 int visit_self_check(nodal_ctx *h, SHierarchy *H);
+int restrict_self_check(nodal_ctx *h, SHierarchy *H);
 int fold_self_check(nodal_ctx *h, SHierarchy *H) {
     static const bool check = knob::TRACE.now() && knob::SA_FOLD_CHECK.now();
     if (!check) return NODAL_OK;
@@ -1856,11 +1990,13 @@
         const bool forked = H->aux != nullptr && nodal_extra_streams_ok(h) &&
                             knob::SA_FORK.now();
         hipStream_t rst = st;
+        const bool wt = L->restrict_want && H->sym_stats[(size_t)l * ST_COUNT + ST_RESTRICTMISS] == 0;
         if (forked) {
             NODAL_HIP_TRY(h, hipEventRecord(H->ev_fork, st));
             NODAL_HIP_TRY(h, hipStreamWaitEvent(H->aux, H->ev_fork, 0));
             H->aux_pending = true;
             NODAL_TRY(galerkin_product<true>(h, H, l, nullptr, 1));
+            if (wt) NODAL_HIP_TRY(h, hipEventRecord(H->ev_w, st));
             rst = H->aux;
         }
         r_refresh<<<grid_for(C->n * 8), TB, 0, rst>>>(C->n, L->rld, L->rlen.as<int32_t>(), L->rcol.as<int32_t>(), L->ld,
@@ -1868,8 +2004,23 @@
                                                      L->rvalf.as<float>());
         NODAL_HIP_TRY(h, hipGetLastError());
         if (forked) NODAL_HIP_TRY(h, hipEventRecord(H->ev_join, H->aux));
+        if (forked && wt) NODAL_HIP_TRY(h, hipStreamWaitEvent(H->aux, H->ev_w, 0));
         NODAL_TRY(galerkin_product<true>(h, H, l, forked ? H->ev_join : nullptr, forked ? 2 : 0));
-        if (forked) H->aux_pending = false;
+        if (wt) {
+            wt_refresh<<<grid_for(L->wtcap), TB, 0, rst>>>(C->n, L->wtstart.as<uint32_t>(), L->wtsrc.as<int32_t>(),
+                                                          L->wval.as<float>(), L->wtval.as<float>());
+            NODAL_HIP_TRY(h, hipGetLastError());
+            if (forked) {
+                NODAL_HIP_TRY(h, hipEventRecord(H->ev_wt, H->aux));
+                H->wt_pending = true;
+            }
+        }
+        if (forked && !H->wt_pending) H->aux_pending = false;
+    }
+    if (H->wt_pending) {
+        NODAL_HIP_TRY(h, hipStreamWaitEvent(st, H->ev_wt, 0));
+        H->wt_pending = false;
+        H->aux_pending = false;
     }
     const int last = H->nlev - 1;
     if (H->dense_coarsest)
@@ -1887,6 +2038,7 @@
     decide_folds(H, hs, false);
     NODAL_TRY(fold_self_check(h, H));
     NODAL_TRY(visit_self_check(h, H));
+    NODAL_TRY(restrict_self_check(h, H));
     *ok = true;
     return NODAL_OK;
 }
@@ -1943,6 +2095,8 @@
     H->sym_valid = false;
     H->refreshed = false;
     H->want_flags = check_floating;
+    H->general = general;
+    H->wt_pending = false;
     H->flags_levels = 0;
     H->last_iters = 0;
     H->drop_graph();
@@ -2025,6 +2179,11 @@
     NODAL_HIP_TRY(h, hipMemcpyAsync(hs, dstats, (size_t)MAX_LEVELS * ST_COUNT * 8, hipMemcpyDeviceToHost, st));
     if (!H->ev_copy) NODAL_HIP_TRY(h, hipEventCreateWithFlags(&H->ev_copy, hipEventDisableTiming));
     NODAL_HIP_TRY(h, hipEventRecord(H->ev_copy, st));
+    if (H->wt_pending) {
+        NODAL_HIP_TRY(h, hipStreamWaitEvent(st, H->ev_wt, 0));
+        H->wt_pending = false;
+        if (!(check_floating && H->flags_levels != 0)) H->aux_pending = false;
+    }
     if (check_floating) {
         if (H->flags_levels == 0) {
             NODAL_HIP_TRY(h, H->level(0)->gflag.reserve((size_t)n0 + 64));
@@ -2100,6 +2259,7 @@
     decide_folds(H, hs, trace);
     NODAL_TRY(fold_self_check(h, H));
     NODAL_TRY(visit_self_check(h, H));
+    NODAL_TRY(restrict_self_check(h, H));
     H->ready = true;
     *accepted = true;
     H->sym_valid = true;
@@ -2204,20 +2364,41 @@
         SAGG_DISPATCH_W(L->wfix, (k_post<W, false, TBV, cyc_t><<<g, tb, 0, st>>>(A, dinv, b, x, x2, nullptr, nullptr, nullptr)));
         x = x2;
     }
-    SAGG_DISPATCH_W(L->wfix, (k_smooth_residual<W, TBV><<<g, tb, 0, st>>>(A, b, x, r)));
     const bool last = l + 1 == H->tail || l + 1 == H->nlev - 1;
+    bool from_b = false;
+    if constexpr (std::is_same_v<TBV, cyc_t>) {
+        from_b = L->restrict_b && fold && nu == 1 && !sb;
+        if (from_b) {
+            const unsigned rblocks = restrict_blocks(nc);
+            const unsigned gw = rblocks + grid_for(n);
+            const uint32_t *ws = L->wtstart.as<uint32_t>();
+            const int32_t *wc = L->wtcol.as<int32_t>();
+            const float *wv = L->wtval.as<float>();
+            if (last) {
+                SAGG_DISPATCH_W(L->wfix, (k_residual_restrict<W, double><<<gw, TB, 0, st>>>(
+                                             A, b, x, r, rblocks, nc, ws, wc, wv, C->v<double>(V_RC), C->dinv.as<double>(), nullptr)));
+            } else {
+                SAGG_DISPATCH_W(L->wfix, (k_residual_restrict<W, cyc_t><<<gw, TB, 0, st>>>(
+                                             A, b, x, r, rblocks, nc, ws, wc, wv, C->v<cyc_t>(V_RC), C->dinv.as<double>(),
+                                             C->v<cyc_t>(V_X))));
+            }
+        }
+    }
+    if (!from_b) SAGG_DISPATCH_W(L->wfix, (k_smooth_residual<W, TBV><<<g, tb, 0, st>>>(A, b, x, r)));
     const double *coef = nullptr;
     if (last) {
         double *rc = C->v<double>(V_RC), *c1 = C->v<double>(V_C1);
-        k_restrict<double><<<grid_for(nc * RL), TB, 0, st>>>(nc, L->rld, L->rcol.as<int32_t>(), L->rvalf.as<float>(),
-                                                            L->rlen.as<int32_t>(), r, rc, C->dinv.as<double>(), nullptr);
+        if (!from_b)
+            k_restrict<double><<<grid_for(nc * RL), TB, 0, st>>>(nc, L->rld, L->rcol.as<int32_t>(), L->rvalf.as<float>(),
+                                                                L->rlen.as<int32_t>(), r, rc, C->dinv.as<double>(), nullptr);
         NODAL_HIP_TRY(h, hipGetLastError());
         NODAL_TRY(last_level(h, H, l + 1, rc, c1));
         hand_up((const double *)c1, (const double *)nullptr, nullptr);
     } else {
         cyc_t *rc = C->v<cyc_t>(V_RC), *c1 = C->v<cyc_t>(V_C1), *c2 = C->v<cyc_t>(V_C2), *x0c = C->v<cyc_t>(V_X);
-        k_restrict<cyc_t><<<grid_for(nc * RL), TB, 0, st>>>(nc, L->rld, L->rcol.as<int32_t>(), L->rvalf.as<float>(),
-                                                           L->rlen.as<int32_t>(), r, rc, C->dinv.as<double>(), x0c);
+        if (!from_b)
+            k_restrict<cyc_t><<<grid_for(nc * RL), TB, 0, st>>>(nc, L->rld, L->rcol.as<int32_t>(), L->rvalf.as<float>(),
+                                                               L->rlen.as<int32_t>(), r, rc, C->dinv.as<double>(), x0c);
         NODAL_HIP_TRY(h, hipGetLastError());
         int nparts = 0;
         const bool kcycle = l < H->klevels && H->kcycle;
@@ -2415,6 +2596,103 @@
                     "d = %.3e (against the bound 2^-23: %.3e)\n", l, (long long)n, (long long)nt, maxp2, dm, dm / 0x1p-23);
     return NODAL_OK;
 }
+template <typename TO>
+int restrict_check_level(nodal_ctx *h, SHierarchy *H, int l) {
+    hipStream_t st = h->stream;
+    SLevel *L = H->pool[l], *C = H->pool[l + 1];
+    const int64_t n = L->n, ld = L->ld, nc = C->n, rld = L->rld;
+    uint64_t seed = 0x9e3779b97f4a7c15ull + 1297ull * (uint64_t)l;
+    auto unit = [&]() {
+        uint64_t z = (seed += 0x9e3779b97f4a7c15ull);
+        z = (z ^ (z >> 30)) * 0xbf58476d1ce4e5b9ull;
+        z = (z ^ (z >> 27)) * 0x94d049bb133111ebull;
+        z ^= z >> 31;
+        return (double)(z >> 11) * (1.0 / 4503599627370496.0) - 1.0;
+    };
+    const int64_t rslots = (int64_t)rcap_for(nc) * rld;
+    std::vector<double> dinv((size_t)n);
+    std::vector<cyc_t> hb((size_t)n), hx0((size_t)n);
+    std::vector<TO> rc_old((size_t)nc), rc_new((size_t)nc);
+    std::vector<int32_t> acol((size_t)L->width * ld), alen((size_t)n), rcol((size_t)rslots), rlen((size_t)nc),
+        wcol((size_t)L->wslots * ld), wlen((size_t)n);
+    std::vector<float> aval((size_t)L->width * ld), rval((size_t)rslots), wval((size_t)L->wslots * ld);
+    auto down = [&](void *dst, const void *src, size_t bytes) { return hipMemcpy(dst, src, bytes, hipMemcpyDeviceToHost); };
+    hipError_t e = hipStreamSynchronize(st);
+    if (e == hipSuccess) e = down(dinv.data(), L->dinv.p, (size_t)n * 8);
+    for (int64_t i = 0; i < n; ++i) {
+        hb[i] = (cyc_t)unit();
+        hx0[i] = (cyc_t)(OMEGA * dinv[i] * (double)hb[i]);
+    }
+    const size_t vb = align256((size_t)n * sizeof(cyc_t)), cb = align256((size_t)nc * sizeof(TO));
+    DevBuf buf;
+    if (e == hipSuccess) e = buf.reserve(3 * vb + 2 * cb);
+    char *p = buf.as<char>();
+    cyc_t *b = reinterpret_cast<cyc_t *>(p), *x0 = reinterpret_cast<cyc_t *>(p + vb), *r = reinterpret_cast<cyc_t *>(p + 2 * vb);
+    TO *ro = reinterpret_cast<TO *>(p + 3 * vb), *rn = reinterpret_cast<TO *>(p + 3 * vb + cb);
+    if (e == hipSuccess) e = hipMemcpyAsync(b, hb.data(), (size_t)n * sizeof(cyc_t), hipMemcpyHostToDevice, st);
+    if (e == hipSuccess) e = hipMemcpyAsync(x0, hx0.data(), (size_t)n * sizeof(cyc_t), hipMemcpyHostToDevice, st);
+    if (e == hipSuccess) {
+        const Ell A = L->A();
+        const unsigned g = grid_for(n);
+        const unsigned rblocks = restrict_blocks(nc);
+        SAGG_DISPATCH_W(L->wfix, (k_smooth_residual<W, cyc_t><<<g, TB, 0, st>>>(A, b, x0, r)));
+        k_restrict<TO><<<grid_for(nc * RL), TB, 0, st>>>(nc, rld, L->rcol.as<int32_t>(), L->rvalf.as<float>(),
+                                                        L->rlen.as<int32_t>(), r, ro, C->dinv.as<double>(), nullptr);
+        SAGG_DISPATCH_W(L->wfix, (k_residual_restrict<W, TO><<<rblocks + g, TB, 0, st>>>(
+                                     A, b, x0, r, rblocks, nc, L->wtstart.as<uint32_t>(), L->wtcol.as<int32_t>(),
+                                     L->wtval.as<float>(), rn, C->dinv.as<double>(), nullptr)));
+        e = hipGetLastError();
+    }
+    if (e == hipSuccess) e = hipStreamSynchronize(st);
+    if (e == hipSuccess) e = down(rc_old.data(), ro, (size_t)nc * sizeof(TO));
+    if (e == hipSuccess) e = down(rc_new.data(), rn, (size_t)nc * sizeof(TO));
+    if (e == hipSuccess) e = down(acol.data(), L->acol.p, acol.size() * 4);
+    if (e == hipSuccess) e = down(aval.data(), L->avalf.p, aval.size() * 4);
+    if (e == hipSuccess) e = down(alen.data(), L->alen.p, (size_t)n * 4);
+    if (e == hipSuccess) e = down(rcol.data(), L->rcol.p, rcol.size() * 4);
+    if (e == hipSuccess) e = down(rval.data(), L->rvalf.p, rval.size() * 4);
+    if (e == hipSuccess) e = down(rlen.data(), L->rlen.p, (size_t)nc * 4);
+    if (e == hipSuccess) e = down(wcol.data(), L->wcol.p, wcol.size() * 4);
+    if (e == hipSuccess) e = down(wval.data(), L->wval.p, wval.size() * 4);
+    if (e == hipSuccess) e = down(wlen.data(), L->wlen.p, (size_t)n * 4);
+    buf.release();
+    NODAL_HIP_TRY(h, e);
+    std::vector<double> t((size_t)n), den((size_t)nc, 0.0);
+    for (int64_t i = 0; i < n; ++i) {
+        double s = fabs((double)hb[i]);
+        for (int32_t q = 0; q < alen[i]; ++q)
+            s += fabs((double)aval[(size_t)q * ld + i]) * fabs((double)hx0[acol[(size_t)q * ld + i]]);
+        t[i] = s;
+    }
+    for (int64_t I = 0; I < nc; ++I)
+        for (int32_t q = 0; q < rlen[I]; ++q) {
+            const size_t at = ((size_t)(q >> 3) * rld + I) * 8 + (q & 7);
+            den[I] += fabs((double)rval[at]) * t[rcol[at]];
+        }
+    for (int64_t i = 0; i < n; ++i)
+        for (int32_t q = 0; q < wlen[i]; ++q)
+            den[wcol[(size_t)q * ld + i]] += fabs((double)wval[(size_t)q * ld + i]) * fabs((double)hb[i]);
+    double dm = 0.0;
+    for (int64_t I = 0; I < nc; ++I) {
+        const double di = fabs((double)rc_new[I] - (double)rc_old[I]) / den[I];
+        dm = !(di <= dm) ? di : dm;
+    }
+    fprintf(stderr, "[sagg] restrict check: level %d, rows %lld, coarse rows %lld, rc from b against the two launches "
+                    "d = %.3e (against the bound 2^-23: %.3e)\n", l, (long long)n, (long long)nc, dm, dm / 0x1p-23);
+    return NODAL_OK;
+}
+int restrict_self_check(nodal_ctx *h, SHierarchy *H) {
+    static const bool check = knob::TRACE.now() && knob::SA_RESTRICT_CHECK.now();
+    if (!check) return NODAL_OK;
+    for (int l = 1; l + 1 < H->nlev; ++l) {
+        if (!H->pool[l]->restrict_b) continue;
+        const bool last = l + 1 == H->tail || l + 1 == H->nlev - 1;
+        if (last) NODAL_TRY(restrict_check_level<double>(h, H, l));
+        else NODAL_TRY(restrict_check_level<cyc_t>(h, H, l));
+    }
+    return NODAL_OK;
+}
+
 int visit_self_check(nodal_ctx *h, SHierarchy *H) {
     static const bool check = knob::TRACE.now() && knob::SA_VISIT_CHECK.now();
     if (!check) return NODAL_OK;
@@ -2512,6 +2790,10 @@
         case NODAL_HA_P2VAL: buf = &L->p2val; bytes = next && L->visit_want ? (int64_t)P2CAP * L->ld * 4 : 0; break;
         case NODAL_HA_P2LEN: buf = &L->p2len; bytes = next && L->visit_want ? L->n * 4 : 0; break;
         case NODAL_HA_D2: buf = &L->d2; bytes = next && L->visit_want ? L->nc * L->ld * 4 : 0; break;
+        case NODAL_HA_WTSTART: buf = &L->wtstart; bytes = next && L->restrict_b ? (L->nc + 1) * 4 : 0; break;
+        case NODAL_HA_WTCOL: buf = &L->wtcol; bytes = next && L->restrict_b ? L->wtcap * 4 : 0; break;
+        case NODAL_HA_WTVAL: buf = &L->wtval; bytes = next && L->restrict_b ? L->wtcap * 4 : 0; break;
+        case NODAL_HA_WTSRC: buf = &L->wtsrc; bytes = next && L->restrict_b ? L->wtcap * 4 : 0; break;
         default: return nodal_fail(h, NODAL_E_INVALID, "debug hierarchy: no such array");
         }
     }
diff --git a/nodal_amd/csrc/sagg_cycle.h b/nodal_amd/csrc/sagg_cycle.h
--- a/nodal_amd/csrc/sagg_cycle.h
+++ b/nodal_amd/csrc/sagg_cycle.h
@@ -925,6 +925,55 @@
     }
 }
 
+constexpr int WT_LANES = 16, WT_U = 8;
+static_assert(64 % WT_LANES == 0 && TB % WT_LANES == 0, "whole rows per wavefront");
+inline unsigned restrict_blocks(int64_t nc) {
+    const int64_t g = (nc + TB / WT_LANES - 1) / (TB / WT_LANES);
+    return (unsigned)((g + 7) & ~(int64_t)7);
+}
+template <int W, typename TO>
+__global__ __launch_bounds__(TB) void k_residual_restrict(Ell A, const cyc_t *__restrict__ b, const cyc_t *__restrict__ x0,
+                                                          cyc_t *__restrict__ r, unsigned rblocks, int64_t nc,
+                                                          const uint32_t *__restrict__ wtstart,
+                                                          const int32_t *__restrict__ wtcol, const float *__restrict__ wtval,
+                                                          TO *__restrict__ rc, const double *__restrict__ cdinv,
+                                                          cyc_t *__restrict__ x0c) {
+    if (blockIdx.x >= rblocks) {
+        const unsigned count = gridDim.x - rblocks;
+        for (int64_t i = (int64_t)xcd_block_sub(rblocks, count) * TB + threadIdx.x; i < A.n; i += (int64_t)count * TB) {
+            const double s = ell_row_w<W>(A, A.valf, i, 0, [&](int32_t j) { return (double)x0[j]; });
+            r[i] = (cyc_t)((double)b[i] - s);
+        }
+        return;
+    }
+    const uint32_t sub = threadIdx.x & (WT_LANES - 1);
+    const int64_t I = (int64_t)xcd_block_sub(0, rblocks) * (TB / WT_LANES) + threadIdx.x / WT_LANES;
+    const bool live = I < nc;
+    const uint32_t s0 = live ? wtstart[I] : 0u, len = live ? wtstart[I + 1] - s0 : 0u;
+    double s = 0.0;
+    for (uint32_t t0 = sub; t0 < len; t0 += WT_LANES * WT_U) {
+        int32_t c[WT_U];
+        double v[WT_U];
+#pragma unroll
+        for (int u = 0; u < WT_U; ++u) {
+            const bool ok = t0 + WT_LANES * u < len;
+            const uint32_t at = s0 + (ok ? t0 + WT_LANES * u : t0);
+            c[u] = wtcol[at];
+            const float loaded = wtval[at];
+            v[u] = ok ? (double)loaded : 0.0;
+        }
+#pragma unroll
+        for (int u = 0; u < WT_U; ++u) s = fma(v[u], (double)b[c[u]], s);
+    }
+#pragma unroll
+    for (int off = WT_LANES >> 1; off > 0; off >>= 1) s += __shfl_xor(s, off, 64);
+    if (live && sub == 0) {
+        const TO stored = (TO)s;
+        rc[I] = stored;
+        if (x0c) x0c[I] = (cyc_t)(OMEGA * cdinv[I] * (double)stored);
+    }
+}
+
 enum { F_RZ = 0, F_ALPHA = 2, F_CONV = 4, F_RR = 6, F_BB = 7, F_FLAG = 8, F_ITERS = 9, F_TOL2 = 10,
        F_ITNO = 12,
        F_COUNT = 16 };
```

Measured after the change: 172.6 circuits/s (median of 6 runs). 1.6% higher.
